# arangesh/TrackMPNN

Measured on AMD Instinct MI355X. Metric: graph_edges_per_sec_fwd_bwd, higher is better.
Workload: dtype f32; 1 GPU; C2 KITTI Car/RRC-shaped rolling windows: 7 frames, D_t~clip(Poisson(6),1,20), F=8 (2d), H=64, K=0, diff; 1 fwd per frame + 1 bwd per window; 16384 windows/GPU batched block-diagonally (64 distinct seeds tiled); windows_per_gpu=16384, rows_final=6762496, parallelism=sequence-dp1

## Files before the change

include/tmpnn.h:

```cpp
#ifndef TMPNN_H
#define TMPNN_H

#include <stddef.h>
#include <stdint.h>

#ifdef __cplusplus
extern "C" {
#endif

#define TMPNN_ABI_VERSION 13

#define TMPNN_OK 0
#define TMPNN_EINVAL (-1)
#define TMPNN_ELAUNCH (-2)
#define TMPNN_EWORKSPACE (-3)

typedef void* tmpnn_stream;
typedef void* tmpnn_event;

typedef struct tmpnn_seg_plan {
    int32_t T;
    int32_t I;
    int32_t nsplit;
    const int32_t* t_row;
// ... 37 lines not shown
    const int32_t* t_loc;
    const int32_t* t_dptr;
    const int32_t* t_dets;
} tmpnn_edge_tiles;

int tmpnn_abi_version(void);
const char* tmpnn_last_error(void);

int tmpnn_gather_diff_fwd(const tmpnn_graph* g, const float* in, int ld_in, float* out, int ld_out,
                          int H, int accumulate, tmpnn_stream stream);
int tmpnn_gather_concat_fwd(const tmpnn_graph* g, const float* in, int ld_in, float* out, int ld_out,
                            int H, int accumulate, tmpnn_stream stream);
int tmpnn_gather_diff_bwd(const tmpnn_graph* g, const float* d_out, int ld_dout, float* d_in, int ld_din,
                          int H, int accumulate, tmpnn_stream stream);
int tmpnn_gather_concat_bwd(const tmpnn_graph* g, const float* d_out, int ld_dout, float* d_in, int ld_din,
                            int H, int accumulate, tmpnn_stream stream);

int tmpnn_segsum_fwd(const tmpnn_graph* g, const float* in, int ld_in, float* out, int ld_out,
                     int H, int accumulate, int compact_out ,
                     tmpnn_stream stream);
int tmpnn_segsum_fwd_live(const tmpnn_graph* g, const float* in, int ld_in, float* out, int ld_out,
                          int H, int compact_out, int row_limit, tmpnn_stream stream);
int tmpnn_segsum_bwd(const tmpnn_graph* g, const float* d_out, int ld_dout, float* d_in, int ld_din,
                     int H, int accumulate, tmpnn_stream stream);

int tmpnn_att_fwd(const tmpnn_graph* g, const int32_t* erec, const float* h, int ld_h, int H, int K,
                  const float* W_cat, const float* a, const uint8_t* keep, float p_drop,
                  float* ha, float* score, float* stats, float* esk, float* alpha, float* out, int ld_out,
                  tmpnn_stream stream);
size_t tmpnn_att_bwd_ws(int E, int Dn, int H, int K);
int tmpnn_att_index(const tmpnn_graph* g, const int32_t* pos, const int32_t* src_pos, const int32_t* dst_pos,
                    int32_t* erec, int32_t* inc_other, tmpnn_stream stream);
int tmpnn_att_bwd(const tmpnn_graph* g, const int32_t* erec, const int32_t* inc_other,
                  const float* h, int ld_h, int H, int K,
                  const float* W_cat, const float* a, const uint8_t* keep, float p_drop,
                  const float* ha, const float* score, const float* stats, const float* esk,
                  const float* d_out, int ld_dout, float* ws, size_t ws_floats,
                  float* d_h, int ld_dh, float* dW_att, float* da, tmpnn_stream stream);
int tmpnn_att_bwd_heads(const tmpnn_graph* g, const int32_t* erec, const int32_t* inc_other,
                        const float* h, int ld_h, int H, int K,
                        const float* W_cat, const float* a, const uint8_t* keep, float p_drop,
                        const float* ha, const float* score, const float* stats, const float* esk,
                        const float* d_out, int ld_dout, float* ws, size_t ws_floats,
                        float* d_h, int ld_dh, float* const* dW_heads, float* const* da_heads, tmpnn_stream stream);

int tmpnn_gru_fwd_head_parts(int H, int IN, int xmode);
int tmpnn_gru_fwd(const int32_t* rows, int R, int xmode, const int32_t* src, const int32_t* dst,
                  const float* msg, int ld_msg, int msg_compact, int IN, const float* h, int ld_h, int H,
                  const float* wih_t, const float* whh_t, const float* b_ih, const float* b_hh,
                  float* h_out, int ld_out, float* gates, size_t gate_plane,
                  const float* w_head, float* logit_part, size_t part_stride, tmpnn_stream stream);
int tmpnn_gru_bwd_data(const int32_t* rows, int R, int IN, const float* h, int ld_h, int H,
                       const float* w_ih, const float* w_hh,
                       const float* gates, size_t gate_plane, const float* d_hout, int ld_dhout,
                       const float* dy, const float* w_head,
                       float* d_msg, int ld_dmsg, float* d_h, int ld_dh,
                       const int32_t* add_src, const int32_t* add_dst, const float* add_msg, int ld_add,
                       tmpnn_stream stream);
size_t tmpnn_gru_bwd_weights_ws(int R, int IN, int H);
int tmpnn_gru_bwd_weights(const int32_t* rows, int R, int xmode, const int32_t* src, const int32_t* dst,
                          const float* msg, int ld_msg, int msg_compact, int IN,
                          const float* h, int ld_h, int H,
                          const float* gates, size_t gate_plane, const float* d_hout, int ld_dhout,
                          const float* dy, const float* w_head,
                          float* dW_ih, float* dW_hh, float* db_ih, float* db_hh,
                          void* ws, size_t ws_bytes, tmpnn_stream stream);

int tmpnn_gru_bwd_fused_available(int H, int IN, int xmode);
size_t tmpnn_gru_bwd_fused_ws(int R, int IN, int H);
int tmpnn_gru_bwd_fused(const int32_t* rows, int R, int xmode, const int32_t* src, const int32_t* dst,
                        const float* msg, int ld_msg, int msg_compact, int IN,
                        const float* h, int ld_h, int H, const float* w_ih, const float* w_hh,
                        const float* gates, size_t gate_plane, const float* d_hout, int ld_dhout,
                        const float* dy, const float* w_head,
                        float* d_msg, int ld_dmsg, float* d_h, int ld_dh,
                        const int32_t* add_src, const int32_t* add_dst, const float* add_msg, int ld_add,
                        float* dW_ih, float* dW_hh, float* db_ih, float* db_hh,
                        void* ws, size_t ws_bytes, tmpnn_stream stream);
typedef struct tmpnn_zs_gate_src {
    const float* proj;
    int32_t ld_proj;
    const int32_t* src_pos;
    const int32_t* dst_pos;
    const float* b_ih;
    const float* b_hh;
} tmpnn_zs_gate_src;
int tmpnn_gru_bwd_fused_zero_state_available(int H, int IN, int xmode);
int tmpnn_gru_bwd_fused_zero_state(const int32_t* rows, int R, const int32_t* src, const int32_t* dst, int IN,
                                   const float* h, int ld_h, int H, const float* w_ih, const float* b_hn,
                                   const float* gates, size_t gate_plane, const float* d_hout, int ld_dhout,
                                   const float* dy, const float* w_head, float* d_msg, int ld_dmsg,
                                   float* dW_ih, float* db_ih, float* db_hh,
                                   void* ws, size_t ws_bytes, tmpnn_stream stream);

int tmpnn_gru_fwd_tiles(const tmpnn_edge_tiles* tiles, int R, const float* proj, int ld_proj, const float* h, int ld_h, int H,
                        const float* whh_t, const float* b_ih, const float* b_hh, float* h_out, int ld_out, float* gates,
                        size_t gate_plane, const float* w_head, float* logit_part, size_t part_stride, tmpnn_stream stream);
int tmpnn_gru_fwd_tiles_zero_state_available(int H, int xmode);
int tmpnn_gru_fwd_tiles_zero_state(const tmpnn_edge_tiles* tiles, int R, const float* proj, int ld_proj, int H,
                                   const float* b_ih, const float* b_hh, float* h_out, int ld_out, float* gates,
                                   size_t gate_plane, int write_hn, const float* w_head, float* logit_part, size_t part_stride,
                                   tmpnn_stream stream);

int tmpnn_rows_linear(const int32_t* rows, int R, const float* in, int ld_in, int H, const float* wt, int NOUT,
                      float* out, int ld_out, tmpnn_stream stream);

int tmpnn_transpose(const float* in, int rows, int cols, float* out, tmpnn_stream stream);

int tmpnn_input_bn_fwd(const float* xdet, int ld_x, int F, int nd, const int32_t* seg_ptr,
                       const int32_t* seg_cnt, const int32_t* seg_of_det ,
                       int S, int H, int training,
                       const float* w1, const float* b1, const float* gamma, const float* beta,
                       float* running_mean, float* running_var,
                       const float* w2, const float* b2,
                       float* y_save, float* mean, float* rstd, float* ws_a ,
                       const int32_t* out_row, float* h_new, int ld_h, tmpnn_stream stream);
size_t tmpnn_input_bn_bwd_ws(int nd, int S, int H, int F);
int tmpnn_input_bn_bwd(const float* xdet, int ld_x, int F, int nd, const int32_t* seg_ptr,
                       const int32_t* seg_cnt, const int32_t* seg_of_det, int S, int H, int training,
                       const float* w1, const float* b1, const float* gamma, const float* beta,
                       const float* w2,
                       const float* y_save, const float* mean, const float* rstd,
                       const int32_t* out_row, const float* d_h, int ld_dh,
                       float* d_xdet, int ld_dx, float* d_xzero,
                       float* dw1, float* db1, float* dgamma, float* dbeta, float* dw2, float* db2,
                       float* ws, size_t ws_floats, tmpnn_stream stream);

int tmpnn_input_tf_supported(int H, int F, int max_seg_rows);
int tmpnn_input_tf_fwd(const float* xdet, const int64_t* x_rows, int ld_x, int F, int nd, const int32_t* seg_ptr, const int32_t* seg_cnt,
                       const int32_t* seg_of_det, int S, int max_seg_rows, int H, int training, const float* w1, const float* b1,
                       const float* gamma, const float* beta, float* running_mean, float* running_var, const float* w2,
                       const float* b2, float* y_save, float* mean, float* rstd, const int32_t* out_row, float* h_new,
                       int ld_h, tmpnn_stream stream);
size_t tmpnn_input_tf_bwd_ws(int nd, int S, int H, int F, int training);
int tmpnn_input_tf_bwd(const float* xdet, const int64_t* x_rows, int ld_x, int F, int nd, const int32_t* seg_ptr, const int32_t* seg_cnt,
                       const int32_t* seg_of_det, int S, int max_seg_rows, int H, int training, const float* w1, const float* b1,
                       const float* gamma, const float* beta, const float* w2, const float* y_save, const float* mean,
                       const float* rstd, const int32_t* out_row, const float* d_h, int ld_dh, float* d_xdet, int ld_dx,
                       float* d_xzero, float* dw1, float* db1, float* dgamma, float* dbeta, float* dw2, float* db2, void* ws,
                       size_t ws_bytes, tmpnn_stream stream);

int tmpnn_heads_fwd(const float* h, int ld_h, int C, int N, const uint8_t* is_edge,
                    const float* w_node, const float* b_node, const float* w_edge, const float* b_edge,
                    float* logits, float* scores, tmpnn_stream stream);
int tmpnn_heads_finish(const float* parts, size_t part_stride, int nparts, int N, const uint8_t* is_edge,
                       const float* b_node, const float* b_edge, float* logits, float* scores, tmpnn_stream stream);
size_t tmpnn_heads_bwd_ws(int N, int C);
int tmpnn_heads_bwd(const float* h, int ld_h, int C, int N, const uint8_t* is_edge,
                    const float* w_node, const float* w_edge, const float* scores,
                    const float* d_logits, const float* d_scores, float* dy_out,
                    float* d_h, int ld_dh, int accumulate,
                    float* dw_node, float* db_node, float* dw_edge, float* db_edge,
                    void* ws, size_t ws_bytes, tmpnn_stream stream);

int tmpnn_targets(const tmpnn_graph* g, const uint8_t* labels, uint8_t* targets, tmpnn_stream stream);
size_t tmpnn_ce_loss_ws(int Dn);
int tmpnn_ce_loss_fwd(const tmpnn_graph* g, const float* logits, const uint8_t* targets, float* stats, float* loss,
                      float* ws, size_t ws_floats, tmpnn_stream stream);
int tmpnn_ce_loss_bwd(const tmpnn_graph* g, const int32_t* src_pos, const int32_t* dst_pos, const float* logits,
                      const float* stats, const float* d_loss, float* d_logits, tmpnn_stream stream);
size_t tmpnn_focal_loss_ws(int R);
int tmpnn_focal_loss_fwd(const int32_t* rows, int R, const float* scores, const uint8_t* targets, float gamma,
                         int use_alpha, float alpha0, float alpha1, float* loss_sum, float* ws, size_t ws_floats,
                         tmpnn_stream stream);
int tmpnn_focal_loss_bwd(const int32_t* rows, int R, const float* scores, const uint8_t* targets, float gamma,
                         int use_alpha, float alpha0, float alpha1, const float* d_loss, float scale, float* d_scores,
                         tmpnn_stream stream);
size_t tmpnn_bce_logits_ws(long n);
int tmpnn_bce_logits_sum_fwd(const float* logits, const float* targets, long n, float* loss_sum, float* ws, size_t ws_floats,
                             tmpnn_stream stream);
int tmpnn_bce_logits_sum_bwd(const float* logits, const float* targets, long n, const float* d_loss, float* d_logits,
                             tmpnn_stream stream);
int tmpnn_train_losses_supported(int E, int Dn);
size_t tmpnn_train_losses_ws(int E, int Dn);
int tmpnn_train_losses_fwd(const tmpnn_graph* g, const float* logits, const float* scores, const uint8_t* labels,
                           int tp_classifier, uint8_t* targets, float* stats, float* out, float* ws, size_t ws_floats,
                           tmpnn_stream stream);
int tmpnn_train_losses_bwd(const tmpnn_graph* g, const int32_t* src_pos, const int32_t* dst_pos, const float* logits,
                           const float* scores, const uint8_t* targets, const float* stats, const float* d_c, const float* d_f,
                           int tp_classifier, float* d_logits, float* d_scores, tmpnn_stream stream);
typedef struct tmpnn_loss_windows {
    int32_t W;
    int32_t n_det;
    int32_t n_edge;
    const int32_t* det_ptr;
    const int32_t* det_idx;
    const int32_t* edge_ptr;
    const int32_t* edge_idx;
    const int32_t* det_win;
    const int32_t* edge_win;
} tmpnn_loss_windows;
size_t tmpnn_train_losses_win_ws(const tmpnn_loss_windows* w);
int tmpnn_train_losses_win_fwd(const tmpnn_graph* g, const tmpnn_loss_windows* w, const float* logits, const float* scores,
                               const uint8_t* labels, int tp_classifier, uint8_t* targets, float* stats, float* out, float* ws,
                               size_t ws_floats, tmpnn_stream stream);
int tmpnn_train_losses_win_bwd(const tmpnn_graph* g, const tmpnn_loss_windows* w, const int32_t* src_pos, const int32_t* dst_pos,
                               const float* logits, const float* scores, const uint8_t* targets, const float* stats,
                               const float* d_c, const float* d_f, int tp_classifier, float* d_logits, float* d_scores,
                               tmpnn_stream stream);

typedef struct tmpnn_train_record {
    double sum_f1;
    int64_t forwards;
    double sum_loss_c;
    double sum_loss_f;
    double sum_loss;
    int64_t chunks;
} tmpnn_train_record;
int tmpnn_cls_counts(const tmpnn_graph* g, const float* scores, const uint8_t* targets, int tp_classifier, int32_t* counts,
                     tmpnn_stream stream);
int tmpnn_cls_counts_win(const tmpnn_graph* g, const tmpnn_loss_windows* w, const float* scores, const uint8_t* targets,
                         int tp_classifier, int32_t* counts, tmpnn_stream stream);
int tmpnn_train_record_fold(const int32_t* counts, int C, int W, const float* loss_c, const float* loss_f, int B,
                            tmpnn_train_record* rec, tmpnn_stream stream);

typedef struct tmpnn_optim_seg {
    float* p;
    int64_t start;
    int64_t count;
} tmpnn_optim_seg;
typedef struct tmpnn_adam_state {
    double lr;
    float step;
    int32_t ticket;
} tmpnn_adam_state;
int tmpnn_optim_chunk(void);
int tmpnn_adam_step(const tmpnn_optim_seg* segs, int P, const int32_t* work, int nwork, float* grad, float* exp_avg,
                    float* exp_avg_sq, int64_t n_flat, tmpnn_adam_state* state, double beta1, double beta2, double eps,
                    double weight_decay, float grad_scale, int zero_grads, tmpnn_stream stream);
int tmpnn_grad_flow(const tmpnn_optim_seg* segs, int P, const float* grad, int64_t n_flat, double* stats, tmpnn_stream stream);

#define TMPNN_TB_MAX_DETS 4096
#define TMPNN_TB_MAX_CALLS 1024
#define TMPNN_TB_NONINT INT64_MIN
#define TMPNN_TB_ST_NONINT 1
#define TMPNN_TB_ST_NEGTS 2
#define TMPNN_TB_ST_RANGE 4
#define TMPNN_TB_ST_DETS 8
#define TMPNN_TB_ST_CALLS 16
#define TMPNN_TB_ST_OFFSETS 32
#define TMPNN_TB_ST_LDS 64
typedef struct tmpnn_train_build {
    int32_t n;
    int32_t B;
    int32_t C;
    int32_t max_dets;
    int32_t max_slots;
    int64_t n_feat;
    const int64_t* y;
    const int64_t* offsets;
    int64_t* info;
    const int32_t* kept;
    const int32_t* cptr;
    int32_t* counts;
    const int32_t* blk;
    const int64_t* call_tab;
    const int32_t* cb_tab;
    int32_t* src; int32_t* dst; int32_t* edge_row; int32_t* src_pos; int32_t* dst_pos;
    int32_t* det_row; int32_t* seg_of_det; int64_t* new_det_local; int64_t* det_group;
    uint8_t* is_edge; int32_t* pos; uint8_t* labels; int64_t* feat_src; int64_t* seg_of_new;
    int32_t* rowptr; int32_t* inc; int32_t* det_order; int32_t* det_win; int32_t* edge_win; int32_t* det_idx; int32_t* edge_idx;
} tmpnn_train_build;
int tmpnn_train_build_count(const tmpnn_train_build* d, tmpnn_stream stream);
int tmpnn_train_build_calls(const tmpnn_train_build* d, tmpnn_stream stream);
int tmpnn_train_build_fill(const tmpnn_train_build* d, int phase, tmpnn_stream stream);

#define TMPNN_CD_MAX_FRAMES 256
#define TMPNN_CD_FLAG_REVERSED 1
#define TMPNN_CD_FLAG_FLIPPED 2
#define TMPNN_CD_FLAG_BAD 128
typedef struct tmpnn_chunk_draw {
    int32_t B;
    int32_t nchunks;
    int32_t L;
    int32_t nseq;
    int32_t F;
    int32_t Fs;
    int32_t fr_range;
    int32_t transforms;
    int64_t ndets;
    int64_t nframes;
    int64_t n_max;
    uint64_t seed;
    uint64_t step;
    float p_drop;
    float p_reverse;
    float p_flip;
    float reserved;
    const int32_t* indices;
    const int32_t* chunks;
    const int32_t* seq_base;
    const int32_t* first;
    const int32_t* track;
    const float* stat;
    const float* table;
    int32_t* count;
    uint8_t* flags;
    int64_t* offsets;
    float* X;
    int64_t* y;
} tmpnn_chunk_draw;
int tmpnn_chunk_draw_count(const tmpnn_chunk_draw* d, tmpnn_stream stream);
int tmpnn_chunk_draw_fill(const tmpnn_chunk_draw* d, tmpnn_stream stream);

#define TMPNN_DG_MAX_ROWS 4096
#define TMPNN_DG_BIG_ROWS 65535
// ... 320 lines not shown
```

trackmpnn_amd/_lib.py:

```python
from __future__ import annotations

import ctypes as C

import torch
import os
import re
from typing import Dict, List, Optional

_HERE = os.path.dirname(os.path.abspath(__file__))
LIB_PATH = os.environ.get('TMPNN_LIB_PATH') or os.path.join(_HERE, 'lib', 'libtmpnn.so')
HEADER_PATH = os.path.join(os.path.dirname(_HERE), 'include', 'tmpnn.h')

ABI_VERSION = 13

c_int = C.c_int
c_void_p = C.c_void_p
c_size_t = C.c_size_t
c_float = C.c_float


class CSegPlan(C.Structure):
    _fields_ = [('T', C.c_int32), ('I', C.c_int32), ('nsplit', C.c_int32), ('t_row', c_void_p), ('items', c_void_p),
                ('rowptr2', c_void_p), ('inc2', c_void_p), ('ws', c_void_p), ('ws_floats', c_size_t)]

# ... 45 lines not shown


class CTrackRows(C.Structure):
    _fields_ = [('ts', c_void_p), ('det_id', c_void_p), ('assoc', c_void_p), ('is_edge', c_void_p), ('src', c_void_p),
                ('dst', c_void_p), ('labels', c_void_p)]


class CLossWindows(C.Structure):
    _fields_ = [('W', C.c_int32), ('n_det', C.c_int32), ('n_edge', C.c_int32), ('det_ptr', c_void_p), ('det_idx', c_void_p),
                ('edge_ptr', c_void_p), ('edge_idx', c_void_p), ('det_win', c_void_p), ('edge_win', c_void_p)]


class CTrainBuild(C.Structure):
    _fields_ = [('n', C.c_int32), ('B', C.c_int32), ('C', C.c_int32), ('max_dets', C.c_int32), ('max_slots', C.c_int32),
                ('n_feat', C.c_int64)] + [(f, c_void_p) for f in (
                    'y', 'offsets', 'info', 'kept', 'cptr', 'counts', 'blk', 'call_tab', 'cb_tab',
                    'src', 'dst', 'edge_row', 'src_pos', 'dst_pos', 'det_row', 'seg_of_det', 'new_det_local', 'det_group',
                    'is_edge', 'pos', 'labels', 'feat_src', 'seg_of_new',
                    'rowptr', 'inc', 'det_order', 'det_win', 'edge_win', 'det_idx', 'edge_idx')]


class CChunkDraw(C.Structure):
    _fields_ = ([(f, C.c_int32) for f in ('B', 'nchunks', 'L', 'nseq', 'F', 'Fs', 'fr_range', 'transforms')]
                + [(f, C.c_int64) for f in ('ndets', 'nframes', 'n_max')] + [('seed', C.c_uint64), ('step', C.c_uint64)]
                + [(f, c_float) for f in ('p_drop', 'p_reverse', 'p_flip', 'reserved')]
                + [(f, c_void_p) for f in ('indices', 'chunks', 'seq_base', 'first', 'track', 'stat', 'table',
                                           'count', 'flags', 'offsets', 'X', 'y')])


class CMotStore(C.Structure):
    _fields_ = ([('S', C.c_int32), ('reserved', C.c_int32)] + [(f, C.c_int64) for f in ('n_gt', 'n_det', 'n_off', 'n_obj')]
                + [(f, c_void_p) for f in ('seq', 'gt_off', 'det_off', 'gt_id', 'gt_box', 'det_box', 'det_perm')])


class CMapStore(C.Structure):
    _fields_ = ([('S', C.c_int32), ('C', C.c_int32)] + [(f, C.c_int64) for f in ('n_gt', 'n_det', 'n_grp', 'n_live', 'n_claim')]
                + [(f, c_void_p) for f in ('gt_box', 'gt_seq', 'cls_gt_off', 'grp_off', 'det_box', 'det_grp', 'det_best', 'cls_off',
                                           'order', 'claim_off', 'claim_det')])


class CLabelStore(C.Structure):
    _fields_ = ([('S', C.c_int32), ('reserved', C.c_int32)] + [(f, C.c_int64) for f in ('n_frames', 'n_det', 'n_gt')]
                + [('iom_ignore_cat', C.c_int32), ('iou_ignore_cat', C.c_int32), ('iou_thresh', c_float), ('iom_thresh', c_float)]
                + [(f, C.c_int64) for f in ('n_small', 'n_big')]
                + [(f, c_void_p) for f in ('seq_base', 'det_first', 'gt_first', 'small_frames', 'big_frames', 'det_frame', 'det_cat',
                                           'det_box', 'det_score', 'gt_frame', 'gt_track', 'gt_cat', 'gt_box')])


class CLabelOut(C.Structure):
    _fields_ = [(f, c_void_p) for f in ('record', 'track', 'keep', 'gt_keep', 'det_cnt', 'gt_cnt', 'fflag', 'det_off', 'gt_off',
                                        'seq_det_off', 'seq_gt_off', 'o_det_frame', 'o_det_track', 'o_det_cat', 'o_det_box',
                                        'o_det_score', 'o_gt_frame', 'o_gt_track', 'o_gt_cat', 'o_gt_box')]


class CVisHead(C.Structure):
    _fields_ = ([(f, C.c_int32) for f in ('T', 'Hm', 'Wm', 'B')] + [('D', C.c_int64)]
                + [(f, c_float) for f in ('input_h', 'input_w', 'down_ratio', 'im_h', 'im_w')]
                + [(f, C.c_int32) for f in ('ld_rows', 'col', 'reserved')]
                + [(f, c_void_p) for f in ('maps', 'box', 'map_of', 'im_hw', 'track', 'offsets', 'mean', 'std', 'rows', 'logits',
                                           'stat', 'nll', 'pix', 'flag', 'chunk_of', 'key', 'loss', 'count')])


_DGP = C.POINTER(CDGraph)
_MPP = C.POINTER(CMpParams)
_TRP = C.POINTER(CTrackRows)
_LWP = C.POINTER(CLossWindows)
_TBP = C.POINTER(CTrainBuild)
_CDP = C.POINTER(CChunkDraw)
_MSP = C.POINTER(CMotStore)
_MAP = C.POINTER(CMapStore)
_LSP = C.POINTER(CLabelStore)
_LOP = C.POINTER(CLabelOut)
_VHP = C.POINTER(CVisHead)

_SIGNATURES = {
    'tmpnn_abi_version': (c_int, []),
    'tmpnn_last_error': (C.c_char_p, []),
    'tmpnn_gather_diff_fwd': (c_int, [_GP, c_void_p, c_int, c_void_p, c_int, c_int, c_int, c_void_p]),
    'tmpnn_gather_concat_fwd': (c_int, [_GP, c_void_p, c_int, c_void_p, c_int, c_int, c_int, c_void_p]),
    'tmpnn_gather_diff_bwd': (c_int, [_GP, c_void_p, c_int, c_void_p, c_int, c_int, c_int, c_void_p]),
    'tmpnn_gather_concat_bwd': (c_int, [_GP, c_void_p, c_int, c_void_p, c_int, c_int, c_int, c_void_p]),
    'tmpnn_segsum_fwd': (c_int, [_GP, c_void_p, c_int, c_void_p, c_int, c_int, c_int, c_int, c_void_p]),
    'tmpnn_segsum_fwd_live': (c_int, [_GP, c_void_p, c_int, c_void_p, c_int, c_int, c_int, c_int, c_void_p]),
    'tmpnn_segsum_bwd': (c_int, [_GP, c_void_p, c_int, c_void_p, c_int, c_int, c_int, c_void_p]),
    'tmpnn_att_fwd': (c_int, [_GP, c_void_p, c_void_p, c_int, c_int, c_int, c_void_p, c_void_p, c_void_p, c_float,
                              c_void_p, c_void_p, c_void_p, c_void_p, c_void_p, c_void_p, c_int, c_void_p]),
    'tmpnn_att_bwd_ws': (c_size_t, [c_int, c_int, c_int, c_int]),
    'tmpnn_att_index': (c_int, [_GP, c_void_p, c_void_p, c_void_p, c_void_p, c_void_p, c_void_p]),
    'tmpnn_att_bwd': (c_int, [_GP, c_void_p, c_void_p, c_void_p, c_int, c_int, c_int, c_void_p, c_void_p, c_void_p,
                              c_float, c_void_p, c_void_p, c_void_p, c_void_p, c_void_p, c_int, c_void_p, c_size_t,
                              c_void_p, c_int, c_void_p, c_void_p, c_void_p]),
    'tmpnn_att_bwd_heads': (c_int, [_GP, c_void_p, c_void_p, c_void_p, c_int, c_int, c_int, c_void_p, c_void_p,
                                    c_void_p, c_float, c_void_p, c_void_p, c_void_p, c_void_p, c_void_p, c_int, c_void_p,
                                    c_size_t, c_void_p, c_int, c_void_p, c_void_p, c_void_p]),
    'tmpnn_gru_fwd': (c_int, [c_void_p, c_int, c_int, c_void_p, c_void_p, c_void_p, c_int, c_int, c_int,
                              c_void_p, c_int, c_int, c_void_p, c_void_p, c_void_p, c_void_p,
                              c_void_p, c_int, c_void_p, c_size_t, c_void_p, c_void_p, c_size_t, c_void_p]),
    'tmpnn_gru_fwd_head_parts': (c_int, [c_int, c_int, c_int]),
    'tmpnn_gru_fwd_tiles': (c_int, [_TP, c_int, c_void_p, c_int, c_void_p, c_int, c_int, c_void_p, c_void_p, c_void_p,
                                    c_void_p, c_int, c_void_p, c_size_t, c_void_p, c_void_p, c_size_t, c_void_p]),
    'tmpnn_gru_fwd_tiles_zero_state_available': (c_int, [c_int, c_int]),
    'tmpnn_gru_fwd_tiles_zero_state': (c_int, [_TP, c_int, c_void_p, c_int, c_int, c_void_p, c_void_p, c_void_p, c_int,
                                               c_void_p, c_size_t, c_int, c_void_p, c_void_p, c_size_t, c_void_p]),
    'tmpnn_heads_finish': (c_int, [c_void_p, c_size_t, c_int, c_int, c_void_p, c_void_p, c_void_p, c_void_p, c_void_p, c_void_p]),
    'tmpnn_gru_bwd_data': (c_int, [c_void_p, c_int, c_int, c_void_p, c_int, c_int, c_void_p, c_void_p,
                                   c_void_p, c_size_t, c_void_p, c_int, c_void_p, c_void_p,
                                   c_void_p, c_int, c_void_p, c_int,
                                   c_void_p, c_void_p, c_void_p, c_int, c_void_p]),
    'tmpnn_gru_bwd_weights_ws': (c_size_t, [c_int, c_int, c_int]),
    'tmpnn_gru_bwd_weights': (c_int, [c_void_p, c_int, c_int, c_void_p, c_void_p, c_void_p, c_int, c_int, c_int,
                                      c_void_p, c_int, c_int, c_void_p, c_size_t, c_void_p, c_int, c_void_p, c_void_p,
                                      c_void_p, c_void_p, c_void_p, c_void_p, c_void_p, c_size_t, c_void_p]),
    'tmpnn_gru_bwd_fused_available': (c_int, [c_int, c_int, c_int]),
    'tmpnn_gru_bwd_fused_ws': (c_size_t, [c_int, c_int, c_int]),
    'tmpnn_gru_bwd_fused': (c_int, [c_void_p, c_int, c_int, c_void_p, c_void_p, c_void_p, c_int, c_int, c_int,
                                    c_void_p, c_int, c_int, c_void_p, c_void_p, c_void_p, c_size_t, c_void_p, c_int,
                                    c_void_p, c_void_p, c_void_p, c_int, c_void_p, c_int,
                                    c_void_p, c_void_p, c_void_p, c_int, c_void_p, c_void_p, c_void_p, c_void_p,
                                    c_void_p, c_size_t, c_void_p]),
    'tmpnn_gru_bwd_fused_zero_state_available': (c_int, [c_int, c_int, c_int]),
    'tmpnn_gru_bwd_fused_zero_state': (c_int, [c_void_p, c_int, c_void_p, c_void_p, c_int, c_void_p, c_int, c_int,
                                               c_void_p, c_void_p, c_void_p, c_size_t, c_void_p, c_int, c_void_p,
                                               c_void_p, c_void_p, c_int, c_void_p, c_void_p, c_void_p, c_void_p,
                                               c_size_t, c_void_p]),
    'tmpnn_rows_linear': (c_int, [c_void_p, c_int, c_void_p, c_int, c_int, c_void_p, c_int, c_void_p, c_int, c_void_p]),
    'tmpnn_transpose': (c_int, [c_void_p, c_int, c_int, c_void_p, c_void_p]),
    'tmpnn_input_bn_fwd': (c_int, [c_void_p, c_int, c_int, c_int, c_void_p, c_void_p, c_void_p, c_int, c_int, c_int,
                                   c_void_p, c_void_p, c_void_p, c_void_p, c_void_p, c_void_p, c_void_p, c_void_p,
                                   c_void_p, c_void_p, c_void_p, c_void_p, c_void_p, c_void_p, c_int, c_void_p]),
    'tmpnn_input_bn_bwd_ws': (c_size_t, [c_int, c_int, c_int, c_int]),
    'tmpnn_input_bn_bwd': (c_int, [c_void_p, c_int, c_int, c_int, c_void_p, c_void_p, c_void_p, c_int, c_int, c_int,
                                   c_void_p, c_void_p, c_void_p, c_void_p, c_void_p,
                                   c_void_p, c_void_p, c_void_p, c_void_p, c_void_p, c_int,
                                   c_void_p, c_int, c_void_p,
                                   c_void_p, c_void_p, c_void_p, c_void_p, c_void_p, c_void_p,
                                   c_void_p, c_size_t, c_void_p]),
    'tmpnn_input_tf_supported': (c_int, [c_int, c_int, c_int]),
    'tmpnn_input_tf_fwd': (c_int, [c_void_p, c_void_p, c_int, c_int, c_int, c_void_p, c_void_p, c_void_p, c_int, c_int, c_int, c_int,
                                   c_void_p, c_void_p, c_void_p, c_void_p, c_void_p, c_void_p, c_void_p, c_void_p,
                                   c_void_p, c_void_p, c_void_p, c_void_p, c_void_p, c_int, c_void_p]),
    'tmpnn_input_tf_bwd_ws': (c_size_t, [c_int, c_int, c_int, c_int, c_int]),
    'tmpnn_input_tf_bwd': (c_int, [c_void_p, c_void_p, c_int, c_int, c_int, c_void_p, c_void_p, c_void_p, c_int, c_int, c_int, c_int,
                                   c_void_p, c_void_p, c_void_p, c_void_p, c_void_p,
                                   c_void_p, c_void_p, c_void_p, c_void_p, c_void_p, c_int,
                                   c_void_p, c_int, c_void_p,
                                   c_void_p, c_void_p, c_void_p, c_void_p, c_void_p, c_void_p,
                                   c_void_p, c_size_t, c_void_p]),
    'tmpnn_heads_fwd': (c_int, [c_void_p, c_int, c_int, c_int, c_void_p, c_void_p, c_void_p, c_void_p, c_void_p,
                                c_void_p, c_void_p, c_void_p]),
    'tmpnn_heads_bwd_ws': (c_size_t, [c_int, c_int]),
    'tmpnn_heads_bwd': (c_int, [c_void_p, c_int, c_int, c_int, c_void_p, c_void_p, c_void_p, c_void_p, c_void_p,
                                c_void_p, c_void_p, c_void_p, c_int, c_int, c_void_p, c_void_p, c_void_p, c_void_p,
                                c_void_p, c_size_t, c_void_p]),
    'tmpnn_targets': (c_int, [_GP, c_void_p, c_void_p, c_void_p]),
    'tmpnn_ce_loss_ws': (c_size_t, [c_int]),
    'tmpnn_ce_loss_fwd': (c_int, [_GP, c_void_p, c_void_p, c_void_p, c_void_p, c_void_p, c_size_t, c_void_p]),
    'tmpnn_ce_loss_bwd': (c_int, [_GP, c_void_p, c_void_p, c_void_p, c_void_p, c_void_p, c_void_p, c_void_p]),
    'tmpnn_focal_loss_ws': (c_size_t, [c_int]),
    'tmpnn_focal_loss_fwd': (c_int, [c_void_p, c_int, c_void_p, c_void_p, c_float, c_int, c_float, c_float, c_void_p,
                                     c_void_p, c_size_t, c_void_p]),
    'tmpnn_focal_loss_bwd': (c_int, [c_void_p, c_int, c_void_p, c_void_p, c_float, c_int, c_float, c_float, c_void_p,
                                     c_float, c_void_p, c_void_p]),
    'tmpnn_bce_logits_ws': (c_size_t, [C.c_long]),
    'tmpnn_bce_logits_sum_fwd': (c_int, [c_void_p, c_void_p, C.c_long, c_void_p, c_void_p, c_size_t, c_void_p]),
    'tmpnn_bce_logits_sum_bwd': (c_int, [c_void_p, c_void_p, C.c_long, c_void_p, c_void_p, c_void_p]),
    'tmpnn_train_losses_supported': (c_int, [c_int, c_int]),
    'tmpnn_train_losses_ws': (c_size_t, [c_int, c_int]),
    'tmpnn_train_losses_fwd': (c_int, [_GP, c_void_p, c_void_p, c_void_p, c_int, c_void_p, c_void_p, c_void_p, c_void_p,
                                       c_size_t, c_void_p]),
    'tmpnn_train_losses_bwd': (c_int, [_GP, c_void_p, c_void_p, c_void_p, c_void_p, c_void_p, c_void_p, c_void_p, c_void_p,
                                       c_int, c_void_p, c_void_p, c_void_p]),
    'tmpnn_train_losses_win_ws': (c_size_t, [_LWP]),
    'tmpnn_train_losses_win_fwd': (c_int, [_GP, _LWP, c_void_p, c_void_p, c_void_p, c_int, c_void_p, c_void_p, c_void_p,
                                           c_void_p, c_size_t, c_void_p]),
    'tmpnn_train_losses_win_bwd': (c_int, [_GP, _LWP, c_void_p, c_void_p, c_void_p, c_void_p, c_void_p, c_void_p, c_void_p,
                                           c_void_p, c_int, c_void_p, c_void_p, c_void_p]),
    'tmpnn_cls_counts': (c_int, [_GP, c_void_p, c_void_p, c_int, c_void_p, c_void_p]),
    'tmpnn_cls_counts_win': (c_int, [_GP, _LWP, c_void_p, c_void_p, c_int, c_void_p, c_void_p]),
    'tmpnn_train_record_fold': (c_int, [c_void_p, c_int, c_int, c_void_p, c_void_p, c_int, c_void_p, c_void_p]),
    'tmpnn_optim_chunk': (c_int, []),
    'tmpnn_adam_step': (c_int, [c_void_p, c_int, c_void_p, c_int, c_void_p, c_void_p, c_void_p, C.c_int64, c_void_p,
                                C.c_double, C.c_double, C.c_double, C.c_double, c_float, c_int, c_void_p]),
    'tmpnn_grad_flow': (c_int, [c_void_p, c_int, c_void_p, C.c_int64, c_void_p, c_void_p]),
    'tmpnn_train_build_count': (c_int, [_TBP, c_void_p]),
    'tmpnn_train_build_calls': (c_int, [_TBP, c_void_p]),
    'tmpnn_train_build_fill': (c_int, [_TBP, c_int, c_void_p]),
    'tmpnn_chunk_draw_count': (c_int, [_CDP, c_void_p]),
    'tmpnn_chunk_draw_fill': (c_int, [_CDP, c_void_p]),
    'tmpnn_online_features': (c_int, [c_int] * 8 + [c_void_p, c_void_p, c_int, c_void_p, c_void_p, c_void_p, c_void_p, c_int,
                                      c_void_p, c_void_p, c_void_p]),
    'tmpnn_mot_max_per_frame': (c_int, []),
    'tmpnn_mot_events_ws': (c_size_t, [c_int, C.c_int64, C.c_int64]),
    'tmpnn_mot_events': (c_int, [_MSP, c_void_p, c_void_p, c_void_p, c_size_t, c_void_p, c_void_p]),
    'tmpnn_mot_dist': (c_int, [c_void_p, c_int, c_void_p, c_int, c_void_p, c_void_p]),
    'tmpnn_mot_summary_limit': (c_int, [c_int]),
    'tmpnn_mot_summary_ws': (c_size_t, [c_int, C.c_int64, C.c_int64, C.c_int64]),
    'tmpnn_mot_summary': (c_int, [_MSP, c_void_p, c_void_p, c_void_p, c_size_t, c_void_p, c_void_p]),
    'tmpnn_map_tile': (c_int, []),
    'tmpnn_map_best': (c_int, [_MAP, c_void_p, c_void_p]),
    'tmpnn_map_eval_ws': (c_size_t, [C.c_int64, C.c_int64, C.c_int64]),
    'tmpnn_map_eval': (c_int, [_MAP, c_void_p, c_void_p, c_void_p, c_size_t, c_void_p, c_void_p]),
    'tmpnn_label_max_per_frame': (c_int, []),
    'tmpnn_label_wave_frame': (c_int, []),
    'tmpnn_label_dets': (c_int, [_LSP, _LOP, c_void_p]),
    'tmpnn_label_compact': (c_int, [_LSP, _LOP, c_void_p]),
    'tmpnn_vis_head_fwd': (c_int, [_VHP, c_void_p]),
    'tmpnn_vis_head_bwd': (c_int, [_VHP, c_void_p, c_void_p, c_void_p]),
    'tmpnn_dgraph_ints': (c_size_t, [c_int]),
    'tmpnn_dgraph_bind': (c_int, [c_void_p, c_int, c_int, _DGP]),
    'tmpnn_graph_from_coo': (c_int, [c_int, c_void_p, c_void_p, C.c_int64, c_void_p, c_void_p, C.c_int64, _DGP, c_void_p]),
    'tmpnn_graph_from_coo_arena': (c_int, [c_int, c_void_p, c_void_p, C.c_int64, c_void_p, c_void_p, C.c_int64, c_void_p, c_int, c_void_p]),
    'tmpnn_graph_from_coo_arena_ws': (c_int, [c_int, c_void_p, c_void_p, C.c_int64, c_void_p, c_void_p, C.c_int64, c_void_p, c_int,
                                              c_void_p, c_size_t, c_void_p]),
    'tmpnn_graph_from_rows_ws': (c_int, [c_int, c_void_p, c_void_p, c_void_p, _DGP, c_void_p, c_size_t, c_void_p]),
    'tmpnn_track_finalize_ws': (c_size_t, [c_int]),
    'tmpnn_track_load': (c_int, [c_int, c_int, c_void_p, _TRP, c_void_p, c_int, c_int, c_void_p, c_int, c_void_p, _DGP, c_void_p,
                                 c_size_t, c_void_p]),
    'tmpnn_track_select': (c_int, [_DGP, _TRP, c_void_p, c_int, c_int, c_int, c_void_p, c_void_p, c_void_p]),
    'tmpnn_track_select_ws': (c_int, [_DGP, _TRP, c_void_p, c_int, c_int, c_int, c_void_p, c_void_p, c_void_p, c_size_t, c_void_p]),
    'tmpnn_track_hungarian_max_dets': (c_int, []),
    'tmpnn_track_extend': (c_int, [c_int, c_int, c_int, c_void_p, c_void_p, c_int, c_void_p, _TRP, c_void_p, c_int, c_int,
                                   c_void_p, c_int, _DGP, c_void_p, c_size_t, c_void_p]),
    'tmpnn_track_extend_tf': (c_int, [c_int, c_int, c_int, c_void_p, c_void_p, c_int, c_void_p, _TRP, c_void_p, c_int, c_void_p,
                                      c_void_p, c_void_p, c_size_t, _DGP, c_void_p, c_void_p, c_int, c_void_p, c_void_p]),
    'tmpnn_track_retire': (c_int, [_DGP, _TRP, c_void_p, c_int, c_int, c_int, c_void_p, c_int, c_void_p, c_void_p, c_size_t,
                                   c_void_p, c_void_p, _TRP, c_void_p, c_int, c_int, c_void_p, c_int, c_void_p, c_int,
                                   c_void_p, c_void_p, c_void_p]),
    'tmpnn_val_f1_count': (c_int, [_DGP, c_void_p, c_void_p, c_int, c_void_p, c_void_p, c_int, c_void_p]),
    'tmpnn_wide_supported': (c_int, [c_int, c_int]),
    'tmpnn_wide_prep_bytes': (c_size_t, [c_int, c_int]),
    'tmpnn_wide_prepare': (c_int, [c_void_p, c_void_p, c_int, c_int, c_void_p, c_void_p]),
    'tmpnn_wide_gru_fwd': (c_int, [c_void_p, c_void_p, c_int, c_void_p, c_int, c_void_p, c_void_p, c_void_p, c_int, c_int,
                                   c_void_p, c_void_p, c_void_p, c_void_p, c_int, c_void_p, c_size_t, c_void_p]),
    'tmpnn_wide_gru_fwd_tiled': (c_int, [c_void_p, c_void_p, c_int, _TP, c_int, c_void_p, c_int, c_int, c_void_p, c_void_p,
                                         c_void_p, c_void_p, c_int, c_void_p, c_size_t, c_void_p]),
    'tmpnn_wide_gru_bwd_diff_ws': (c_size_t, [c_int, c_int, c_int, c_int]),
    'tmpnn_wide_gru_bwd_diff': (c_int, [c_void_p, _GP, c_void_p, c_int, c_int, c_void_p, c_size_t, c_void_p, c_int,
                                        c_void_p, c_void_p, c_void_p, c_int, c_void_p, c_void_p, c_void_p, c_void_p,
                                        c_void_p, c_size_t, c_void_p]),
    'tmpnn_wide_gru_bwd_diff_fused': (c_int, [c_void_p, _GP, c_void_p, c_int, c_int, c_void_p, c_size_t, c_void_p, c_int,
                                              c_void_p, c_void_p, c_void_p, c_int, c_void_p, c_void_p, c_void_p, c_void_p,
                                              c_void_p, c_size_t, c_void_p, c_int, c_void_p, c_void_p, c_void_p, c_void_p]),
    'tmpnn_mp_iter_prep_floats': (c_size_t, [c_int, c_int, c_int]),
    'tmpnn_mp_iter_prepare': (c_int, [_MPP, c_void_p, c_void_p]),
    'tmpnn_mp_iter_save_floats': (c_size_t, [c_int, c_int, c_int, c_int]),
    'tmpnn_mp_iter_fwd': (c_int, [_MPP, c_void_p, _DGP, c_int, c_void_p, c_int, c_void_p, c_int,
                                  c_void_p, c_void_p, c_void_p, c_void_p, c_size_t, c_void_p]),
    'tmpnn_mp_iter_save_es_offset': (c_size_t, [c_int, c_int, c_int, c_int]),
    'tmpnn_mp_iter_fwd_parts': (c_int, [_MPP, c_void_p, _DGP, c_int, c_void_p, c_int, c_void_p, c_int,
                                        c_void_p, c_void_p, c_void_p, c_void_p, c_size_t, c_int, c_void_p]),
    'tmpnn_mp_iter_bwd_parts': (c_int, [_MPP, c_void_p, _DGP, c_int, c_void_p, c_int, c_void_p, c_void_p, c_void_p, c_void_p,
                                        c_int, c_void_p, c_int, c_void_p, c_int, c_void_p, c_void_p, c_void_p, _MPP, c_void_p,
                                        c_size_t, c_int, c_void_p]),
    'tmpnn_mp_iter_bwd_ws': (c_size_t, [c_int, c_int, c_int, c_int, c_int]),
    'tmpnn_mp_iter_bwd': (c_int, [_MPP, c_void_p, _DGP, c_int, c_void_p, c_int, c_void_p, c_void_p, c_void_p, c_void_p,
                                  c_int, c_void_p, c_int, c_void_p, c_int, c_void_p, c_void_p, c_void_p, _MPP, c_void_p,
                                  c_size_t, c_void_p]),
}

_lib: Optional[C.CDLL] = None


_VARIANT_SIGNATURES = {
    'tmpnn_track_append': (c_int, [c_int, c_int, c_int, c_void_p, c_void_p, c_int, c_void_p, c_void_p, c_void_p, c_void_p,
                                   c_void_p, c_void_p, c_void_p, c_void_p, c_void_p]),
    'tmpnn_gru_bwd_weights_variant': (c_int, [c_void_p, c_int, c_int, c_void_p, c_void_p, c_void_p, c_int, c_int, c_int,
                                              c_void_p, c_int, c_int, c_void_p, c_size_t, c_void_p, c_int, c_void_p, c_void_p,
                                              c_void_p, c_void_p, c_void_p, c_void_p, c_void_p, c_size_t, c_int, c_void_p]),
    'tmpnn_gru_bwd_weights_choice': (c_int, []),
    'tmpnn_wide_gru_bwd_diff_aux': (c_int, [c_void_p, _GP, c_void_p, c_int, c_int, c_void_p, c_size_t, c_void_p, c_int,
                                            c_void_p, c_void_p, c_void_p, c_int, c_void_p, c_void_p, c_void_p, c_void_p,
                                            c_void_p, c_size_t, c_void_p, c_void_p, c_void_p, c_void_p]),
    'tmpnn_wide_gru_bwd_data_ws': (c_size_t, [c_int, c_int]),
    'tmpnn_wide_gru_bwd_data': (c_int, [c_void_p, c_void_p, c_int, c_void_p, c_int, c_int, c_void_p, c_size_t, c_void_p, c_int,
                                        c_void_p, c_void_p, c_void_p, c_int, c_void_p, c_int, c_void_p, c_size_t, c_void_p]),
    'tmpnn_wide_gru_bwd_weights_ws': (c_size_t, [c_int, c_int]),
    'tmpnn_wide_gru_bwd_weights': (c_int, [c_void_p, c_void_p, c_int, c_void_p, c_void_p, c_void_p, c_int, c_int, c_void_p,
                                           c_void_p, c_void_p, c_void_p, c_void_p, c_size_t, c_void_p]),
}


def header_symbols(variants: bool = False) -> List[str]:
    with open(HEADER_PATH) as f:
        txt = f.read()
    if not variants:
        txt = re.sub(r'#ifdef TMPNN_KEEP_VARIANTS.*?#endif', '', txt, flags=re.S)
    txt = re.sub(r'/\*.*?\*/', '', txt, flags=re.S)
    return sorted(set(re.findall(r'\b(tmpnn_[a-z0-9_]+)\s*\(', txt)))


def load() -> C.CDLL:
    global _lib
    if _lib is not None:
        return _lib
    if not os.path.exists(LIB_PATH):
        raise RuntimeError(
            f'{LIB_PATH} is missing: build it with `python -c "import __graft_entry__ as g; g.build()"` '
            '(hipcc --offload-arch=gfx950).  trackmpnn_amd has no CPU or torch fallback.')
    lib = C.CDLL(LIB_PATH)
    for name, (res, args) in _SIGNATURES.items():
        try:
            fn = getattr(lib, name)
        except AttributeError as e:
            raise RuntimeError(f'libtmpnn.so does not export {name}; rebuild it') from e
        fn.restype = res
        fn.argtypes = args
# ... 37 lines not shown
```

trackmpnn_amd/csrc/agg.hip:

```cpp
#include "common.h"
#include <stdlib.h>

namespace tmpnn {

static thread_local char g_err[512] = "";

int set_error(int code, const char* fmt, ...) {
    va_list ap;
    va_start(ap, fmt);
    vsnprintf(g_err, sizeof(g_err), fmt, ap);
    va_end(ap);
    return code;
}

#ifdef TMPNN_KEEP_VARIANTS
template <bool CONCAT, bool ACC>
__global__ __launch_bounds__(256) void k_gather(int E, const int32_t* __restrict__ src,
                                                const int32_t* __restrict__ dst,
                                                const int32_t* __restrict__ edge_row,
                                                const float* __restrict__ in, int ld_in,
                                                float* __restrict__ out, int ld_out, int H) {
    const int lpr = H >> 2;
    const int rpb = 256 / lpr;
    const int c4 = (threadIdx.x % lpr) * 4;
    const int slot = threadIdx.x / lpr;
    constexpr int U = 4;
    const long stride = (long)gridDim.x * rpb;
    for (long e0 = (long)blockIdx.x * rpb + slot; e0 < E; e0 += stride * U) {
        int s[U], d[U], r[U];
        bool ok[U];
#pragma unroll
        for (int u = 0; u < U; ++u) {
            const long e = e0 + u * stride;
            ok[u] = e < E;
            const long ec = ok[u] ? e : e0;
            s[u] = src[ec]; d[u] = dst[ec]; r[u] = edge_row[ec];
        }
        float4 a[U], b[U];
#pragma unroll
        for (int u = 0; u < U; ++u) {
            a[u] = *reinterpret_cast<const float4*>(in + (size_t)s[u] * ld_in + c4);
            b[u] = *reinterpret_cast<const float4*>(in + (size_t)d[u] * ld_in + c4);
        }
#pragma unroll
        for (int u = 0; u < U; ++u) {
            if (!ok[u]) continue;
            float* o = out + (size_t)r[u] * ld_out + c4;
            if (!CONCAT) {
                float4 v = make_float4(a[u].x - b[u].x, a[u].y - b[u].y, a[u].z - b[u].z, a[u].w - b[u].w);
                if (ACC) {
                    const float4 p = *reinterpret_cast<const float4*>(o);
                    v.x += p.x; v.y += p.y; v.z += p.z; v.w += p.w;
                }
                *reinterpret_cast<float4*>(o) = v;
            } else {
                float4 va = a[u], vb = b[u];
                if (ACC) {
                    const float4 p = *reinterpret_cast<const float4*>(o);
                    const float4 q = *reinterpret_cast<const float4*>(o + H);
                    va.x += p.x; va.y += p.y; va.z += p.z; va.w += p.w;
                    vb.x += q.x; vb.y += q.y; vb.z += q.z; vb.w += q.w;
                }
                *reinterpret_cast<float4*>(o) = va;
                *reinterpret_cast<float4*>(o + H) = vb;
            }
        }
    }
}

template <bool ACC>
__global__ __launch_bounds__(256) void k_segsum(int Dn, const int32_t* __restrict__ det_row,
                                                const int32_t* __restrict__ rowptr,
                                                const int32_t* __restrict__ inc,
                                                const int32_t* __restrict__ det_order,
                                                const float* __restrict__ in, int ld_in,
                                                float* __restrict__ out, int ld_out, int H,
                                                float wneg, int cneg, int compact_out) {
    const int lane = threadIdx.x & 63;
    const int lpr = H >> 2;
    const int ngrp = 64 / lpr;
    const int grp = lane / lpr;
    const int c4 = (lane % lpr) * 4;
    constexpr int U = 4;
    constexpr int SEG_CHUNK = 64;
    const int wv = threadIdx.x >> 6;
    for (long base = (long)blockIdx.x * SEG_CHUNK; base < Dn; base += (long)gridDim.x * SEG_CHUNK) {
        const long hi = base + SEG_CHUNK < Dn ? base + SEG_CHUNK : Dn;
        for (long i = base + wv; i < hi; i += 4) {
            const int d = det_order ? det_order[i] : (int)i;
            const int p0 = rowptr[d], p1 = rowptr[d + 1];
            float4 acc = make_float4(0.f, 0.f, 0.f, 0.f);
            for (int pb = p0 + grp; pb < p1; pb += ngrp * U) {
                int v[U];
#pragma unroll
                for (int u = 0; u < U; ++u) {
                    const int p = pb + u * ngrp;
                    v[u] = p < p1 ? inc[p] : 0x7fffffff;
                }
                float4 x[U];
#pragma unroll
                for (int u = 0; u < U; ++u) {
                    const bool live = v[u] != 0x7fffffff;
                    const int row = live ? (v[u] & 0x7fffffff) : 0;
                    x[u] = *reinterpret_cast<const float4*>(in + (size_t)row * ld_in + (v[u] < 0 ? cneg : 0) + c4);
                    const float w = v[u] < 0 ? wneg : 1.0f;
                    if (live) { x[u].x *= w; x[u].y *= w; x[u].z *= w; x[u].w *= w; }
                    else x[u] = make_float4(0.f, 0.f, 0.f, 0.f);
                }
#pragma unroll
                for (int u = 0; u < U; ++u) { acc.x += x[u].x; acc.y += x[u].y; acc.z += x[u].z; acc.w += x[u].w; }
            }
            for (int off = lpr; off < 64; off <<= 1) {
                acc.x += __shfl_xor(acc.x, off);
                acc.y += __shfl_xor(acc.y, off);
                acc.z += __shfl_xor(acc.z, off);
                acc.w += __shfl_xor(acc.w, off);
            }
            if (grp == 0) {
                float* o = out + (size_t)(compact_out ? d : det_row[d]) * ld_out + c4;
                if (ACC) {
                    const float4 p = *reinterpret_cast<const float4*>(o);
                    acc.x += p.x; acc.y += p.y; acc.z += p.z; acc.w += p.w;
                }
                *reinterpret_cast<float4*>(o) = acc;
            }
        }
    }
}


#endif

template <bool CONCAT, bool ACC, int U = 4>
__global__ __launch_bounds__(256) void k_gather_pipe(int E, const int32_t* __restrict__ src,
                                                     const int32_t* __restrict__ dst,
                                                     const int32_t* __restrict__ edge_row,
                                                     const float* __restrict__ in, int ld_in,
                                                     float* __restrict__ out, int ld_out, int H) {
    const int lpr = H >> 2;
    const int rpb = 256 / lpr;
    const int c4 = (threadIdx.x % lpr) * 4;
    const int slot = threadIdx.x / lpr;
    const long chunk = (long)rpb * U;
    long e0 = (long)blockIdx.x * chunk + slot;
    const long step = (long)gridDim.x * chunk;
    int s[U], d[U], r[U];
    auto load_ids = [&](long base) {
#pragma unroll
        for (int u = 0; u < U; ++u) {
            const long e = base + (long)u * rpb;
            const long ec = e < E ? e : (E - 1);
            s[u] = src[ec]; d[u] = dst[ec]; r[u] = edge_row[ec];
        }
    };
    if (e0 < E) load_ids(e0);
    for (; e0 < E; e0 += step) {
        float4 a[U], b[U];
        int rr[U];
        bool ok[U];
#pragma unroll
        for (int u = 0; u < U; ++u) {
            ok[u] = e0 + (long)u * rpb < E;
            rr[u] = r[u];
            a[u] = *reinterpret_cast<const float4*>(in + (size_t)s[u] * ld_in + c4);
            b[u] = *reinterpret_cast<const float4*>(in + (size_t)d[u] * ld_in + c4);
        }
        if (e0 + step < E) load_ids(e0 + step);
#pragma unroll
        for (int u = 0; u < U; ++u) {
            if (!ok[u]) continue;
            float* o = out + (size_t)rr[u] * ld_out + c4;
            if (!CONCAT) {
                float4 v = make_float4(a[u].x - b[u].x, a[u].y - b[u].y, a[u].z - b[u].z, a[u].w - b[u].w);
                if (ACC) {
                    const float4 p = *reinterpret_cast<const float4*>(o);
                    v.x += p.x; v.y += p.y; v.z += p.z; v.w += p.w;
                }
                *reinterpret_cast<float4*>(o) = v;
            } else {
                float4 va = a[u], vb = b[u];
                if (ACC) {
                    const float4 p = *reinterpret_cast<const float4*>(o);
                    const float4 q = *reinterpret_cast<const float4*>(o + H);
                    va.x += p.x; va.y += p.y; va.z += p.z; va.w += p.w;
                    vb.x += q.x; vb.y += q.y; vb.z += q.z; vb.w += q.w;
                }
                *reinterpret_cast<float4*>(o) = va;
                *reinterpret_cast<float4*>(o + H) = vb;
            }
        }
    }
}

template <bool ACC, int U = 4, int SEG_CHUNK = 32, bool DUAL = false, bool LIM = false>
__global__ __launch_bounds__(256) void k_segsum_pipe(int Dn, const int32_t* __restrict__ det_row,
                                                     const int32_t* __restrict__ rowptr,
                                                     const int32_t* __restrict__ inc,
                                                     const int32_t* __restrict__ det_order,
                                                     const float* __restrict__ in, int ld_in,
                                                     float* __restrict__ out, int ld_out, int H,
                                                     float wneg, int cneg, int compact_out,
                                                     const float* __restrict__ part = nullptr, int nsplit = 0,
                                                     int row_limit = 0x7fffffff) {
    const int lane = threadIdx.x & 63;
    const int lpr = H >> 2;
    const int ngrp = 64 / lpr;
    const int grp = lane / lpr;
    const int c4 = (lane % lpr) * 4;
    const int wv = threadIdx.x >> 6;
    const long nchunk = (Dn + SEG_CHUNK - 1) / SEG_CHUNK;
    auto item_pos = [&](long k) -> long {
        const long per = SEG_CHUNK / 4;
        const long ch = (long)blockIdx.x + (k / per) * gridDim.x;
        if (ch >= nchunk) return -1;
        const long i = ch * SEG_CHUNK + wv + (k % per) * 4;
        return i < Dn ? i : -2;
    };
    long kA = 0;
    int dA = -1, dB = -1, p0B = 0, p1B = 0, dC = -1, p0C = 0, p1C = 0, vC[U];
    auto fetchA = [&]() {
        long pos;
        do { pos = item_pos(kA++); } while (pos == -2);
        dA = pos < 0 ? -1 : (det_order ? det_order[pos] : (int)pos);
    };
    auto advanceB = [&]() {
        dB = dA;
        if (dB >= 0) { p0B = rowptr[dB]; p1B = rowptr[dB + 1]; }
    };
    auto advanceC = [&]() {
        dC = dB; p0C = p0B; p1C = p1B;
        if (dC >= 0) {
#pragma unroll
            for (int u = 0; u < U; ++u) {
                const int p = p0C + grp + u * ngrp;
                vC[u] = p < p1C ? inc[p] : 0x7fffffff;
            }
        }
    };
    fetchA(); advanceB(); fetchA(); advanceC(); advanceB(); fetchA();
    int pbC = p0C + grp;
    float4 acc = make_float4(0.f, 0.f, 0.f, 0.f);
    while (dC >= 0) {
        const int d = dC;
        float4 x[U];
        bool live[U];
        float w[U];
#pragma unroll
        for (int u = 0; u < U; ++u) {
            live[u] = vC[u] != 0x7fffffff;
            const int row = live[u] ? (vC[u] & 0x7fffffff) : 0;
            w[u] = vC[u] < 0 ? wneg : 1.0f;
            if (LIM) {
                live[u] = live[u] && row < row_limit;
                x[u] = make_float4(0.f, 0.f, 0.f, 0.f);
                if (live[u]) x[u] = *reinterpret_cast<const float4*>(in + (size_t)row * ld_in + (vC[u] < 0 ? cneg : 0) + c4);
            } else if (DUAL && row >= nsplit)
                x[u] = *reinterpret_cast<const float4*>(part + (size_t)(row - nsplit) * H + c4);
            else
                x[u] = *reinterpret_cast<const float4*>(in + (size_t)row * ld_in + (vC[u] < 0 ? cneg : 0) + c4);
        }
        const bool last = (pbC - grp) + ngrp * U >= p1C;
        if (!last) {
            pbC += ngrp * U;
#pragma unroll
            for (int u = 0; u < U; ++u) {
                const int p = pbC + u * ngrp;
                vC[u] = p < p1C ? inc[p] : 0x7fffffff;
            }
        } else {
            advanceC(); advanceB(); fetchA();
            pbC = p0C + grp;
        }
#pragma unroll
        for (int u = 0; u < U; ++u) {
            if (live[u]) { x[u].x *= w[u]; x[u].y *= w[u]; x[u].z *= w[u]; x[u].w *= w[u]; }
            else x[u] = make_float4(0.f, 0.f, 0.f, 0.f);
        }
#pragma unroll
        for (int u = 0; u < U; ++u) { acc.x += x[u].x; acc.y += x[u].y; acc.z += x[u].z; acc.w += x[u].w; }
        if (!last) continue;
        for (int off = lpr; off < 64; off <<= 1) {
            acc.x += __shfl_xor(acc.x, off);
            acc.y += __shfl_xor(acc.y, off);
            acc.z += __shfl_xor(acc.z, off);
            acc.w += __shfl_xor(acc.w, off);
        }
        if (grp == 0) {
            float* o = out + (size_t)(compact_out ? d : det_row[d]) * ld_out + c4;
            if (ACC) {
                const float4 p = *reinterpret_cast<const float4*>(o);
                acc.x += p.x; acc.y += p.y; acc.z += p.z; acc.w += p.w;
            }
            *reinterpret_cast<float4*>(o) = acc;
        }
        acc = make_float4(0.f, 0.f, 0.f, 0.f);
    }
}

#ifdef TMPNN_KEEP_VARIANTS
static int agg_variant() {
    static const int v = [] { const char* e = getenv("TMPNN_AGG"); return (e && e[0] == '0') ? 0 : 1; }();
    return v;
}
#else
static constexpr int agg_variant() { return 1; }
#endif

__global__ void k_transpose(const float* __restrict__ in, int rows, int cols, float* __restrict__ out) {
    __shared__ float tile[32][33];
    const int bx = blockIdx.x * 32, by = blockIdx.y * 32;
    for (int j = threadIdx.y; j < 32; j += blockDim.y) {
        const int r = by + j, c = bx + threadIdx.x;
        if (r < rows && c < cols) tile[j][threadIdx.x] = in[(size_t)r * cols + c];
    }
    __syncthreads();
    for (int j = threadIdx.y; j < 32; j += blockDim.y) {
        const int c = bx + j, r = by + threadIdx.x;
        if (r < rows && c < cols) out[(size_t)c * rows + r] = tile[threadIdx.x][j];
    }
}

__global__ void k_reduce_slabs(const float* __restrict__ slabs, size_t stride, int nslab,
                               float* __restrict__ dst, size_t n, int accumulate) {
    const size_t i = (size_t)blockIdx.x * blockDim.x + threadIdx.x;
    if (i >= n) return;
    float s = 0.f;
#pragma unroll 8
    for (int k = 0; k < nslab; ++k) s += slabs[(size_t)k * stride + i];
    dst[i] = accumulate ? dst[i] + s : s;
}

__global__ void k_fold_slabs(const float* __restrict__ slabs, size_t stride, int nslab, float* __restrict__ out,
                             size_t n) {
    const size_t i = (size_t)blockIdx.x * blockDim.x + threadIdx.x;
    if (i >= n) return;
    const int k0 = blockIdx.y * 32, k1 = min(nslab, k0 + 32);
    float s = 0.f;
#pragma unroll 8
    for (int k = k0; k < k1; ++k) s += slabs[(size_t)k * stride + i];
    out[(size_t)blockIdx.y * n + i] = s;
}

size_t reduce_slabs_ws_floats(int nslab, size_t n) { return nslab > 64 ? (size_t)ceil_div(nslab, 32) * n : 0; }

int launch_reduce_slabs(const float* slabs, size_t stride, int nslab, float* dst, size_t n, int accumulate,
                        hipStream_t st, float* ws2) {
    if (n == 0) return TMPNN_OK;
    if (nslab > 64 && ws2 != nullptr) {
        const int ng = ceil_div(nslab, 32);
        hipLaunchKernelGGL(k_fold_slabs, dim3(ceil_div((long)n, 256), ng), dim3(256), 0, st, slabs, stride, nslab, ws2, n);
        int rc = check_launch("fold_slabs");
        if (rc) return rc;
        slabs = ws2;
        stride = n;
        nslab = ng;
    }
    hipLaunchKernelGGL(k_reduce_slabs, dim3(ceil_div((long)n, 256)), dim3(256), 0, st, slabs, stride, nslab, dst,
                       n, accumulate);
    return check_launch("reduce_slabs");
}

static int check_graph(const tmpnn_graph* g) {
    TM_REQUIRE(g != nullptr, "graph is null");
    TM_REQUIRE(g->N >= 0 && g->E >= 0 && g->Dn >= 0 && (long)g->E + g->Dn == g->N,
               "graph sizes inconsistent: N=%d E=%d Dn=%d", g->N, g->E, g->Dn);
    if (g->E > 0)
        TM_REQUIRE(g->src && g->dst && g->edge_row && g->inc, "graph edge arrays are null (E=%d)", g->E);
    if (g->Dn > 0) TM_REQUIRE(g->det_row && g->rowptr, "graph det arrays are null (Dn=%d)", g->Dn);
    return TMPNN_OK;
}

static int check_rows(const float* in, int ld_in, const float* out, int ld_out, int H, int w_in, int w_out) {
    TM_REQUIRE(supported_H(H), "unsupported hidden width H=%d (need 32/64/128/256)", H);
    TM_REQUIRE(in && out, "null feature pointer");
    TM_REQUIRE(ld_in >= w_in && ld_out >= w_out, "leading dimension too small (ld_in=%d ld_out=%d)", ld_in, ld_out);
    TM_REQUIRE((ld_in & 3) == 0 && (ld_out & 3) == 0 && aligned16(in) && aligned16(out),
               "feature rows must be 16-byte aligned (ld multiple of 4 floats)");
    return TMPNN_OK;
}

static int grid_for(long items, int per_block) {
    long b = (items + per_block - 1) / per_block;
    if (b > 256L * 64) b = 256L * 64;
    if (b < 1) b = 1;
    return (int)b;
}

static int gather(const tmpnn_graph* g, const float* in, int ld_in, float* out, int ld_out, int H, int accumulate,
                  bool concat, tmpnn_stream stream) {
    int rc = check_graph(g);
    if (rc) return rc;
    rc = check_rows(in, ld_in, out, ld_out, H, H, concat ? 2 * H : H);
    if (rc) return rc;
    if (g->E == 0) return TMPNN_OK;
    const int rpb = 256 / (H >> 2);
    dim3 grid(grid_for(g->E, rpb)), block(256);
    hipStream_t st = as_stream(stream);
#define L(K, C, A) hipLaunchKernelGGL((K<C, A>), grid, block, 0, st, g->E, g->src, g->dst, g->edge_row, in, ld_in, out, ld_out, H)
    if (agg_variant() && !concat) {
        grid = dim3(grid_for(g->E, rpb * 8));
        if (accumulate) hipLaunchKernelGGL((k_gather_pipe<false, true, 8>), grid, block, 0, st, g->E, g->src, g->dst, g->edge_row, in, ld_in, out, ld_out, H);
        else hipLaunchKernelGGL((k_gather_pipe<false, false, 8>), grid, block, 0, st, g->E, g->src, g->dst, g->edge_row, in, ld_in, out, ld_out, H);
    } else
    if (agg_variant()) {
        grid = dim3(grid_for(g->E, rpb * 4));
        if (concat) { if (accumulate) L(k_gather_pipe, true, true); else L(k_gather_pipe, true, false); }
        else        { if (accumulate) L(k_gather_pipe, false, true); else L(k_gather_pipe, false, false); }
    }
#ifdef TMPNN_KEEP_VARIANTS
    else {
        if (concat) { if (accumulate) L(k_gather, true, true); else L(k_gather, true, false); }
        else        { if (accumulate) L(k_gather, false, true); else L(k_gather, false, false); }
    }
#endif
#undef L
    return check_launch("gather");
}


__global__ __launch_bounds__(256) void k_segsum_tiles(int I, int T, const int32_t* __restrict__ items,
                                                      const int32_t* __restrict__ t_row, const float* __restrict__ in,
                                                      int ld_in, float* __restrict__ part) {
    __shared__ float4 S[4][8][64];
    const int tid = threadIdx.x, lane = tid & 63;
    const int w = __builtin_amdgcn_readfirstlane(tid >> 6);
    auto add4 = [](float4 a, const float4& b) { a.x += b.x; a.y += b.y; a.z += b.z; a.w += b.w; return a; };
    for (int k = blockIdx.x; k < I; k += gridDim.x) {
        const int t0 = items[2 * k], nt = items[2 * k + 1];
        float4 ad[4];
#pragma unroll
        for (int j = 0; j < 4; ++j) ad[j] = make_float4(0.f, 0.f, 0.f, 0.f);
        for (int t = t0; t < t0 + nt; ++t) {
            const int32_t* tr = t_row + (size_t)t * 128 + 4 * w;
            float4 ps[8];
#pragma unroll
            for (int half = 0; half < 2; ++half) {
                float4 x[4][4];
#pragma unroll
                for (int i = 0; i < 4; ++i)
#pragma unroll
                    for (int j = 0; j < 4; ++j) {
                        const int row = tr[(half * 4 + i) * 16 + j];
                        x[i][j] = *reinterpret_cast<const float4*>(in + (size_t)(row < 0 ? 0 : row) * ld_in + 4 * lane);
                        if (row < 0) x[i][j] = make_float4(0.f, 0.f, 0.f, 0.f);
                    }
#pragma unroll
                for (int i = 0; i < 4; ++i) {
                    ps[half * 4 + i] = add4(add4(add4(x[i][0], x[i][1]), x[i][2]), x[i][3]);
#pragma unroll
                    for (int j = 0; j < 4; ++j) ad[j] = add4(ad[j], x[i][j]);
                }
            }
#pragma unroll
            for (int i = 0; i < 8; ++i) S[w][i][lane] = ps[i];
            __syncthreads();
#pragma unroll
            for (int r = 0; r < 2; ++r) {
                const int i = w + 4 * r;
                const float4 v = add4(add4(add4(S[0][i][lane], S[1][i][lane]), S[2][i][lane]), S[3][i][lane]);
                *reinterpret_cast<float4*>(part + ((size_t)t * 8 + i) * 256 + 4 * lane) = v;
            }
            __syncthreads();
        }
#pragma unroll
        for (int j = 0; j < 4; ++j)
            *reinterpret_cast<float4*>(part + ((size_t)8 * T + (size_t)16 * k + 4 * w + j) * 256 + 4 * lane) = ad[j];
    }
}

static int segsum_dense(const tmpnn_graph* g, const tmpnn_seg_plan* pl, const float* in, int ld_in, float* out, int ld_out,
                        int accumulate, int compact_out, hipStream_t st) {
    TM_REQUIRE(pl->T >= 0 && pl->I >= 0 && pl->nsplit == g->N && pl->rowptr2 && pl->inc2 && (pl->T == 0 || (pl->t_row && pl->items)),
               "segsum (dense form): inconsistent plan (T=%d I=%d nsplit=%d N=%d)", pl->T, pl->I, pl->nsplit, g->N);
    const size_t need = ((size_t)8 * pl->T + (size_t)16 * pl->I) * 256;
    if (need > 0 && (pl->ws == nullptr || pl->ws_floats < need))
        return set_error(TMPNN_EWORKSPACE, "segsum (dense form): the plan's partial buffer holds %zu floats, %zu needed", pl->ws_floats, need);
    if (pl->I > 0) {
        const int grid = pl->I < 256 * 4 ? pl->I : 256 * 4;
        hipLaunchKernelGGL(k_segsum_tiles, dim3(grid), dim3(256), 0, st, pl->I, pl->T, pl->items, pl->t_row, in, ld_in, pl->ws);
        int rc = check_launch("segsum_tiles");
        if (rc) return rc;
    }
    dim3 grid(grid_for(g->Dn, 16)), block(256);
    if (accumulate)
        hipLaunchKernelGGL((k_segsum_pipe<true, 8, 16, true>), grid, block, 0, st, g->Dn, g->det_row, pl->rowptr2, pl->inc2,
                           (const int32_t*)nullptr, in, ld_in, out, ld_out, 256, -1.0f, 0, compact_out, pl->ws, pl->nsplit);
    else
        hipLaunchKernelGGL((k_segsum_pipe<false, 8, 16, true>), grid, block, 0, st, g->Dn, g->det_row, pl->rowptr2, pl->inc2,
                           (const int32_t*)nullptr, in, ld_in, out, ld_out, 256, -1.0f, 0, compact_out, pl->ws, pl->nsplit);
    return check_launch("segsum (dense form, second pass)");
}

#ifdef TMPNN_KEEP_VARIANTS
static constexpr int SW_CH = 160;
static constexpr int SW_MAXCH = 24, SW_MAXD = 160, SW_LCAP = 15;
static constexpr int SW_NW = 8, SW_NHG = 128;
static constexpr int SW_ROWS = SW_CH * 128, SW_RECS = 4096, SW_ACCS = 4 * SW_MAXD * 128, SW_IDS = 768, SW_OROW = 768;
static constexpr int SW_OFF_RECS = 3 * SW_ROWS, SW_OFF_ACCS = SW_OFF_RECS + 3 * SW_RECS, SW_OFF_IDS = SW_OFF_ACCS + SW_ACCS,
                     SW_OFF_OROW = SW_OFF_IDS + 3 * SW_IDS;
static constexpr size_t SW_SHM = SW_OFF_OROW + 2 * SW_OROW;
static_assert(SW_SHM <= 160 * 1024, "k_segsum_win: three chunks and a window's streams must fit the LDS");
static_assert(SW_MAXD <= SW_CH && SW_LCAP * 2 * SW_NHG <= SW_RECS && 4 * SW_CH <= SW_IDS && 4 * SW_MAXD <= SW_OROW &&
                  4 * SW_MAXD <= 5 * SW_NHG && SW_CH / 8 <= 3 * SW_NW && SW_MAXD <= 3 * 8 * SW_NW, "k_segsum_win: capacities");

__device__ __forceinline__ uint32_t sw_lds_addr(const void* p) {
    return (uint32_t)(uintptr_t)(const __attribute__((address_space(3))) char*)(const char*)p;
}
template <int DW>
__device__ __forceinline__ void sw_glds(const void* gsrc, uint32_t lds_wave_base) {
    unsigned keep;
    lds_wave_base = __builtin_amdgcn_readfirstlane(lds_wave_base);
    if constexpr (DW == 4)
        asm volatile("s_mov_b32 %0, m0\n\ts_mov_b32 m0, %2\n\ts_nop 0\n\tglobal_load_lds_dwordx4 %1, off\n\ts_mov_b32 m0, %0"
                     : "=&s"(keep) : "v"(gsrc), "s"(lds_wave_base) : "memory");
    else
        asm volatile("s_mov_b32 %0, m0\n\ts_mov_b32 m0, %2\n\ts_nop 0\n\tglobal_load_lds_dword %1, off\n\ts_mov_b32 m0, %0"
                     : "=&s"(keep) : "v"(gsrc), "s"(lds_wave_base) : "memory");
}
__device__ __forceinline__ void sw_wait(int n) {
    if (n == 0) asm volatile("s_waitcnt vmcnt(0)" ::: "memory");
    else if (n == 1) asm volatile("s_waitcnt vmcnt(1)" ::: "memory");
    else if (n == 2) asm volatile("s_waitcnt vmcnt(2)" ::: "memory");
    else if (n == 3) asm volatile("s_waitcnt vmcnt(3)" ::: "memory");
    else if (n == 4) asm volatile("s_waitcnt vmcnt(4)" ::: "memory");
    else if (n == 5) asm volatile("s_waitcnt vmcnt(5)" ::: "memory");
    else if (n == 6) asm volatile("s_waitcnt vmcnt(6)" ::: "memory");
    else if (n == 7) asm volatile("s_waitcnt vmcnt(7)" ::: "memory");
    else if (n == 8) asm volatile("s_waitcnt vmcnt(8)" ::: "memory");
    else asm volatile("s_waitcnt vmcnt(0)" ::: "memory");
}

struct SwJob {
    int j, e0, ne, q0, nd, r0, lm2, mb, nit;
    unsigned long long lm01;
    __device__ __forceinline__ int hf() const { return j & 1; }
    __device__ __forceinline__ int nch() const { return (ne + SW_CH - 1) / SW_CH; }
};
struct SwItem { SwJob jb; int c, L, roff; };
__device__ __forceinline__ void sw_copy(SwItem& d, const SwItem& s) {
// ... 106 lines not shown
    sw_copy(B, A);
    next_item(B);
    sw_copy(Cn, B);
    next_item(Cn);
    sw_copy(D, Cn);
    next_item(D);
    sw_copy(En, D);
    next_item(En);
    for (int x = tid; x < SW_ACCS / 16; x += 512) reinterpret_cast<float4*>(accs)[x] = make_float4(0.f, 0.f, 0.f, 0.f);
    stage_ids(A, 0);
    stage_ids(B, 1);
    stage_ids(Cn, 2);
    sw_wait(0);
    __syncthreads();
    stage_rows(A, 0);
    sw_wait(0);
    __syncthreads();
    fly = 0;
    stage_rows(B, 1);
    stage_ids(D, 0);
    int fly_prev = fly;
    int W_nd = 0, W_hf = 0, W_mb = 0;
    bool wr = false;
    int rb = 0;
    for (;;) {
        sw_wait(fly_prev);
        __syncthreads();
        fly = 0;
        if (wr) {
            const int* orow = orow_of(W_mb);
            const float* prevr = rows_of(rb == 0 ? 2 : rb - 1);
#pragma unroll
            for (int p = 0; p < 3; ++p) {
                if (64 * p + 8 * wv >= W_nd) continue;
                const int q = 64 * p + hgl, qc = min(q, W_nd - 1);
                float* as = accs + qc * 4 * 32 + c4;
                const float4 a0 = *reinterpret_cast<const float4*>(as), a1 = *reinterpret_cast<const float4*>(as + 32);
                const float4 a2 = *reinterpret_cast<const float4*>(as + 64), a3 = *reinterpret_cast<const float4*>(as + 96);
                const int orw = orow[qc];
                float4 t;
                t.x = (a0.x + a1.x) + (a2.x + a3.x);
                t.y = (a0.y + a1.y) + (a2.y + a3.y);
                t.z = (a0.z + a1.z) + (a2.z + a3.z);
                t.w = (a0.w + a1.w) + (a2.w + a3.w);
                if (ACC) {
                    const float4 pv = *reinterpret_cast<const float4*>(prevr + qc * 32 + c4);
                    t.x += pv.x; t.y += pv.y; t.z += pv.z; t.w += pv.w;
                }
                if (q < W_nd) {
                    *reinterpret_cast<float4*>(out + (size_t)orw * ld_out + 32 * W_hf + c4) = t;
                    const float4 z = make_float4(0.f, 0.f, 0.f, 0.f);
                    *reinterpret_cast<float4*>(as) = z;
                    *reinterpret_cast<float4*>(as + 32) = z;
                    *reinterpret_cast<float4*>(as + 64) = z;
                    *reinterpret_cast<float4*>(as + 96) = z;
                }
                ++fly;
            }
            __syncthreads();
            wr = false;
        }
        if (A.jb.nit == 0) break;
        stage_rows(Cn, rb == 0 ? 2 : rb - 1);
        stage_ids(En, rb == 2 ? 0 : rb + 1);
        if (A.L > 0) {
            const uint16_t* rc = recs_of(rb) + hgl;
            const float* rows = rows_of(rb) + c4;
            float* ab = accs + hgl * 32 + c4;
            unsigned r0 = rc[0], r1 = rc[64];
            for (int s = 0; s < A.L; ++s) {
                const int sn = min(s + 1, A.L - 1) * SW_NHG;
                const unsigned n0 = rc[sn], n1 = rc[sn + 64];
                const float4 x0 = *reinterpret_cast<const float4*>(rows + (r0 & 255u) * 32);
                const float4 x1 = *reinterpret_cast<const float4*>(rows + (r1 & 255u) * 32);
                float* ap0 = ab + ((r0 >> 9) & 7u) * (SW_NHG * 32);
                float* ap1 = ab + ((r1 >> 9) & 7u) * (SW_NHG * 32) + 64 * 32;
                float4 a0 = *reinterpret_cast<const float4*>(ap0), a1 = *reinterpret_cast<const float4*>(ap1);
                const float w0 = (r0 & 0x100u) ? -1.0f : 1.0f, w1 = (r1 & 0x100u) ? -1.0f : 1.0f;
                a0.x += x0.x * w0; a0.y += x0.y * w0; a0.z += x0.z * w0; a0.w += x0.w * w0;
                a1.x += x1.x * w1; a1.y += x1.y * w1; a1.z += x1.z * w1; a1.w += x1.w * w1;
                if (!(r0 & 0x8000u)) *reinterpret_cast<float4*>(ap0) = a0;
                if (!(r1 & 0x8000u)) *reinterpret_cast<float4*>(ap1) = a1;
                r0 = n0; r1 = n1;
            }
        }
        if (A.c == A.jb.nit - 1) { wr = true; W_nd = A.jb.nd; W_hf = A.jb.hf(); W_mb = A.jb.mb; }
        sw_copy(A, B); sw_copy(B, Cn); sw_copy(Cn, D); sw_copy(D, En);
        next_item(En);
        rb = rb == 2 ? 0 : rb + 1;
        fly_prev = fly;
    }
    sw_wait(0);
}

static int cu_count() {
    static const int v = [] {
        int dev = 0, cus = 256;
        if (hipGetDevice(&dev) == hipSuccess) (void)hipDeviceGetAttribute(&cus, hipDeviceAttributeMultiprocessorCount, dev);
        return cus > 0 ? cus : 256;
    }();
    return v;
}

static int segsum_win(const tmpnn_graph* g, const tmpnn_win_plan* pl, const float* in, int ld_in, float* out, int ld_out,
                      int accumulate, int compact_out, hipStream_t st) {
    TM_REQUIRE(pl->W > 0 && pl->wrec && pl->erow && pl->recs && pl->det && pl->drow &&
                   (pl->nbig == 0 || pl->big_order), "segsum: incomplete window plan");
    const int njob = 2 * pl->W, cus = cu_count();
    dim3 grid(njob < cus ? njob : cus), block(512);
    if (accumulate) {
        TM_SHM_ONCE((k_segsum_win<true>), SW_SHM);
        hipLaunchKernelGGL((k_segsum_win<true>), grid, block, SW_SHM, st, *pl, in, ld_in, out, ld_out, compact_out);
    } else {
        TM_SHM_ONCE((k_segsum_win<false>), SW_SHM);
        hipLaunchKernelGGL((k_segsum_win<false>), grid, block, SW_SHM, st, *pl, in, ld_in, out, ld_out, compact_out);
    }
    int rc = check_launch("segsum (window-owned form)");
    if (rc || pl->nbig == 0) return rc;
    dim3 g2(grid_for(pl->nbig, 32));
    if (accumulate)
        hipLaunchKernelGGL((k_segsum_pipe<true, 4, 32>), g2, dim3(256), 0, st, pl->nbig, g->det_row, g->rowptr, g->inc, pl->big_order,
                           in, ld_in, out, ld_out, 64, -1.0f, 0, compact_out);
    else
        hipLaunchKernelGGL((k_segsum_pipe<false, 4, 32>), g2, dim3(256), 0, st, pl->nbig, g->det_row, g->rowptr, g->inc, pl->big_order,
                           in, ld_in, out, ld_out, 64, -1.0f, 0, compact_out);
    return check_launch("segsum (windows beyond the LDS capacity)");
}

#endif

static int segsum(const tmpnn_graph* g, const float* in, int ld_in, float* out, int ld_out, int H, int accumulate,
                  float wneg, int cneg, int compact_out, tmpnn_stream stream, int row_limit = 0x7fffffff) {
    int rc = check_graph(g);
    if (rc) return rc;
    rc = check_rows(in, ld_in, out, ld_out, H, H + cneg, H);
    if (rc) return rc;
    if (g->Dn == 0) return TMPNN_OK;
    hipStream_t st = as_stream(stream);
    if (g->seg_plan && H == 256 && wneg == -1.0f && cneg == 0)
        return segsum_dense(g, g->seg_plan, in, ld_in, out, ld_out, accumulate, compact_out, st);
#ifdef TMPNN_KEEP_VARIANTS
    if (g->win_plan && H == 64 && wneg == -1.0f && cneg == 0 && 2 * g->win_plan->W >= cu_count() &&
        ld_in % 4 == 0 && ld_out % 4 == 0 && (((uintptr_t)in | (uintptr_t)out) & 15) == 0)
        return segsum_win(g, g->win_plan, in, ld_in, out, ld_out, accumulate, compact_out, st);
#endif
    dim3 grid(grid_for(g->Dn, 64)), block(256);
#define LS(K, A) hipLaunchKernelGGL((K<A>), grid, block, 0, st, g->Dn, g->det_row, g->rowptr, g->inc, g->det_order, in, ld_in, out, ld_out, H, wneg, cneg, compact_out)
#define LSP(A, UU, CH)                                                                                       \
    do {                                                                                                     \
        grid = dim3(grid_for(g->Dn, CH));                                                                    \
        hipLaunchKernelGGL((k_segsum_pipe<A, UU, CH>), grid, block, 0, st, g->Dn, g->det_row, g->rowptr, g->inc, \
                           g->det_order, in, ld_in, out, ld_out, H, wneg, cneg, compact_out);                \
    } while (0)
    const bool deep = (long)2 * g->E > (long)24 * g->Dn;
    if (row_limit < g->N && !accumulate) {
        grid = dim3(grid_for(g->Dn, deep ? 16 : 32));
        if (deep)
            hipLaunchKernelGGL((k_segsum_pipe<false, 8, 16, false, true>), grid, block, 0, st, g->Dn, g->det_row, g->rowptr, g->inc,
                               g->det_order, in, ld_in, out, ld_out, H, wneg, cneg, compact_out, (const float*)nullptr, 0, row_limit);
        else
            hipLaunchKernelGGL((k_segsum_pipe<false, 4, 32, false, true>), grid, block, 0, st, g->Dn, g->det_row, g->rowptr, g->inc,
                               g->det_order, in, ld_in, out, ld_out, H, wneg, cneg, compact_out, (const float*)nullptr, 0, row_limit);
        return check_launch("segsum (live rows)");
    }
    if (agg_variant()) {
        if (deep) { if (accumulate) LSP(true, 8, 16); else LSP(false, 8, 16); }
        else      { if (accumulate) LSP(true, 4, 32); else LSP(false, 4, 32); }
    }
#ifdef TMPNN_KEEP_VARIANTS
    else               { if (accumulate) LS(k_segsum, true); else LS(k_segsum, false); }
#endif
#undef LSP
#undef LS
    return check_launch("segsum");
}

}

using namespace tmpnn;

extern "C" {

int tmpnn_abi_version(void) { return TMPNN_ABI_VERSION; }
const char* tmpnn_last_error(void) { return tmpnn::g_err; }

#define TM_SLICED(H_, call_)                                                              \
    do {                                                                                  \
        if (supported_H_big(H_)) {                                                        \
            for (int c0 = 0; c0 < (H_); c0 += 256) {                                      \
                const int w = (H_) - c0 < 256 ? (H_) - c0 : 256;                          \
                const int rc_ = call_;                                                    \
                if (rc_) return rc_;                                                      \
            }                                                                             \
            return TMPNN_OK;                                                              \
        }                                                                                 \
    } while (0)

int tmpnn_gather_diff_fwd(const tmpnn_graph* g, const float* in, int ld_in, float* out, int ld_out, int H,
                          int accumulate, tmpnn_stream stream) {
    TM_SLICED(H, gather(g, in + c0, ld_in, out + c0, ld_out, w, accumulate, false, stream));
    return gather(g, in, ld_in, out, ld_out, H, accumulate, false, stream);
}
int tmpnn_gather_concat_fwd(const tmpnn_graph* g, const float* in, int ld_in, float* out, int ld_out, int H,
                            int accumulate, tmpnn_stream stream) {
    return gather(g, in, ld_in, out, ld_out, H, accumulate, true, stream);
}
int tmpnn_gather_diff_bwd(const tmpnn_graph* g, const float* d_out, int ld_dout, float* d_in, int ld_din, int H,
                          int accumulate, tmpnn_stream stream) {
    TM_SLICED(H, segsum(g, d_out + c0, ld_dout, d_in + c0, ld_din, w, accumulate, -1.0f, 0, 0, stream));
    return segsum(g, d_out, ld_dout, d_in, ld_din, H, accumulate, -1.0f, 0, 0, stream);
}
int tmpnn_gather_concat_bwd(const tmpnn_graph* g, const float* d_out, int ld_dout, float* d_in, int ld_din, int H,
                            int accumulate, tmpnn_stream stream) {
    TM_SLICED(H, segsum(g, d_out + c0, ld_dout, d_in + c0, ld_din, w, accumulate, 1.0f, H, 0, stream));
    return segsum(g, d_out, ld_dout, d_in, ld_din, H, accumulate, 1.0f, H, 0, stream);
}
int tmpnn_segsum_fwd(const tmpnn_graph* g, const float* in, int ld_in, float* out, int ld_out, int H, int accumulate,
                     int compact_out, tmpnn_stream stream) {
    TM_SLICED(H, segsum(g, in + c0, ld_in, out + c0, ld_out, w, accumulate, -1.0f, 0, compact_out, stream));
    return segsum(g, in, ld_in, out, ld_out, H, accumulate, -1.0f, 0, compact_out, stream);
}
int tmpnn_segsum_fwd_live(const tmpnn_graph* g, const float* in, int ld_in, float* out, int ld_out, int H, int compact_out,
                          int row_limit, tmpnn_stream stream) {
    TM_REQUIRE(row_limit >= 0, "segsum_fwd_live: row_limit %d", row_limit);
    TM_SLICED(H, segsum(g, in + c0, ld_in, out + c0, ld_out, w, 0, -1.0f, 0, compact_out, stream, row_limit));
    return segsum(g, in, ld_in, out, ld_out, H, 0, -1.0f, 0, compact_out, stream, row_limit);
}
int tmpnn_segsum_bwd(const tmpnn_graph* g, const float* d_out, int ld_dout, float* d_in, int ld_din, int H,
                     int accumulate, tmpnn_stream stream) {
    TM_SLICED(H, gather(g, d_out + c0, ld_dout, d_in + c0, ld_din, w, accumulate, false, stream));
    return gather(g, d_out, ld_dout, d_in, ld_din, H, accumulate, false, stream);
}

int tmpnn_transpose(const float* in, int rows, int cols, float* out, tmpnn_stream stream) {
    TM_REQUIRE(in && out && rows > 0 && cols > 0, "transpose: bad arguments");
    dim3 grid(ceil_div(cols, 32), ceil_div(rows, 32)), block(32, 8);
    hipLaunchKernelGGL(k_transpose, grid, block, 0, as_stream(stream), in, rows, cols, out);
    return check_launch("transpose");
}

}
```

trackmpnn_amd/csrc/dense.hip:

```cpp
#include "common.h"

namespace tmpnn {

static constexpr float BN_EPS = 1e-5f;
static constexpr float BN_MOMENTUM = 0.1f;

__global__ __launch_bounds__(256) void k_gemm(GemmArgs g, int kper, float* slab) {
    __shared__ float As[16][68];
    __shared__ float Bs[16][68];
    const int tid = threadIdx.x;
    const int tx = tid & 15, ty = tid >> 4;
    const int m0 = blockIdx.y * 64, n0 = blockIdx.x * 64;
    const int kbeg = blockIdx.z * kper;
    const int kend = min(g.K, kbeg + kper);
    float acc[4][4] = {};
    const bool va = (reinterpret_cast<uintptr_t>(g.A) & 15) == 0 && ((g.sak == 1 ? g.sam : g.sak) & 3) == 0;
    const bool vb = (reinterpret_cast<uintptr_t>(g.B) & 15) == 0 && ((g.sbn == 1 ? g.sbk : g.sbn) & 3) == 0;
    for (int k0 = kbeg; k0 < kend; k0 += 16) {
        const bool fullk = k0 + 16 <= kend;
        if (fullk && m0 + 64 <= g.M && !g.a_krows && g.sak == 1 && va) {
            const int m = tid >> 2, kq = (tid & 3) * 4;
            const long ar = g.a_rows ? g.a_rows[m0 + m] : (m0 + m);
            const float4 v = *reinterpret_cast<const float4*>(g.A + ar * g.sam + k0 + kq);
            As[kq][m] = v.x; As[kq + 1][m] = v.y; As[kq + 2][m] = v.z; As[kq + 3][m] = v.w;
        } else if (fullk && m0 + 64 <= g.M && !g.a_rows && g.sam == 1 && va) {
            const int k = tid >> 4, mq = (tid & 15) * 4;
            const long ak = g.a_krows ? g.a_krows[k0 + k] : (k0 + k);
            *reinterpret_cast<float4*>(&As[k][mq]) = *reinterpret_cast<const float4*>(g.A + ak * g.sak + m0 + mq);
        } else {
#pragma unroll
            for (int i = 0; i < 4; ++i) {
                const int idx = tid + i * 256;
                int m, k;
                if (g.sak == 1) { k = idx & 15; m = idx >> 4; } else { m = idx & 63; k = idx >> 6; }
                float v = 0.f;
                if (m0 + m < g.M && k0 + k < kend) {
                    const long ar = g.a_rows ? g.a_rows[m0 + m] : (m0 + m);
                    const long ak = g.a_krows ? g.a_krows[k0 + k] : (k0 + k);
                    v = g.A[ar * g.sam + ak * g.sak];
                }
                As[k][m] = v;
            }
        }
        if (fullk && n0 + 64 <= g.N && g.sbn == 1 && vb) {
            const int k = tid >> 4, nq = (tid & 15) * 4;
            *reinterpret_cast<float4*>(&Bs[k][nq]) = *reinterpret_cast<const float4*>(g.B + (long)(k0 + k) * g.sbk + n0 + nq);
        } else if (fullk && n0 + 64 <= g.N && g.sbk == 1 && vb) {
            const int n = tid >> 2, kq = (tid & 3) * 4;
            const float4 v = *reinterpret_cast<const float4*>(g.B + (long)(n0 + n) * g.sbn + k0 + kq);
            Bs[kq][n] = v.x; Bs[kq + 1][n] = v.y; Bs[kq + 2][n] = v.z; Bs[kq + 3][n] = v.w;
        } else {
#pragma unroll
            for (int i = 0; i < 4; ++i) {
                const int idx = tid + i * 256;
                int n, k;
                if (g.sbn == 1) { n = idx & 63; k = idx >> 6; } else { k = idx & 15; n = idx >> 4; }
                float v = 0.f;
                if (n0 + n < g.N && k0 + k < kend) v = g.B[(long)(k0 + k) * g.sbk + (long)(n0 + n) * g.sbn];
                Bs[k][n] = v;
            }
        }
        __syncthreads();
#pragma unroll
        for (int k = 0; k < 16; ++k) {
            float a[4], b[4];
#pragma unroll
            for (int i = 0; i < 4; ++i) { a[i] = As[k][ty * 4 + i]; b[i] = Bs[k][tx * 4 + i]; }
#pragma unroll
            for (int i = 0; i < 4; ++i)
#pragma unroll
                for (int j = 0; j < 4; ++j) acc[i][j] += a[i] * b[j];
        }
        __syncthreads();
    }
    const bool vc = n0 + tx * 4 + 3 < g.N &&
                    (slab ? (g.N & 3) == 0 && (reinterpret_cast<uintptr_t>(slab) & 15) == 0
                          : (g.ldc & 3) == 0 && (reinterpret_cast<uintptr_t>(g.C) & 15) == 0 &&
                                (!g.bias || (reinterpret_cast<uintptr_t>(g.bias) & 15) == 0));
#pragma unroll
    for (int i = 0; i < 4; ++i) {
        const int m = m0 + ty * 4 + i;
        if (m >= g.M) continue;
        if (vc) {
            const int n = n0 + tx * 4;
            float4 v = make_float4(acc[i][0], acc[i][1], acc[i][2], acc[i][3]);
            if (slab) {
                *reinterpret_cast<float4*>(slab + (size_t)blockIdx.z * g.M * g.N + (size_t)m * g.N + n) = v;
            } else {
                if (g.bias) {
                    const float4 b = *reinterpret_cast<const float4*>(g.bias + n);
                    v.x += b.x; v.y += b.y; v.z += b.z; v.w += b.w;
                }
                const long cr = g.c_rows ? g.c_rows[m] : m;
                float4* p = reinterpret_cast<float4*>(g.C + cr * g.ldc + n);
                if (g.accumulate) { const float4 o = *p; v.x = o.x + v.x; v.y = o.y + v.y; v.z = o.z + v.z; v.w = o.w + v.w; }
                *p = v;
            }
            continue;
        }
#pragma unroll
        for (int j = 0; j < 4; ++j) {
            const int n = n0 + tx * 4 + j;
            if (n >= g.N) continue;
            if (slab) {
                slab[(size_t)blockIdx.z * g.M * g.N + (size_t)m * g.N + n] = acc[i][j];
            } else {
                const long cr = g.c_rows ? g.c_rows[m] : m;
                float v = acc[i][j] + (g.bias ? g.bias[n] : 0.f);
                float* p = g.C + cr * g.ldc + n;
                *p = g.accumulate ? *p + v : v;
            }
        }
    }
}

int launch_gemm(const GemmArgs& g, hipStream_t st) {
    if (g.M <= 0 || g.N <= 0) return TMPNN_OK;
    dim3 grid(ceil_div(g.N, 64), ceil_div(g.M, 64), 1), block(256);
    hipLaunchKernelGGL(k_gemm, grid, block, 0, st, g, g.K > 0 ? g.K : 1, (float*)nullptr);
    return check_launch("gemm");
}

static int splitk_plan(int K, int* kper) {
    int nsplit = (K + 127) / 128;
    if (nsplit > 1024) nsplit = 1024;
    if (nsplit < 1) nsplit = 1;
    int kp = (K + nsplit - 1) / nsplit;
    kp = (kp + 15) & ~15;
    if (kp < 16) kp = 16;
    nsplit = (K + kp - 1) / kp;
    if (nsplit < 1) nsplit = 1;
    *kper = kp;
    return nsplit;
}

size_t gemm_splitk_ws_floats(int M, int N, int K) {
    int kper;
    const int ns = splitk_plan(K, &kper);
    return (size_t)ns * M * N + reduce_slabs_ws_floats(ns, (size_t)M * N);
}

int launch_gemm_splitk(const GemmArgs& g, float* ws, size_t ws_floats, hipStream_t st) {
    if (g.M <= 0 || g.N <= 0) return TMPNN_OK;
    if (g.K <= 0) return TMPNN_OK;
    int kper;
    const int ns = splitk_plan(g.K, &kper);
    if (ws_floats < gemm_splitk_ws_floats(g.M, g.N, g.K))
        return set_error(TMPNN_EWORKSPACE, "gemm_splitk: workspace too small");
    if (ns == 1) return launch_gemm(g, st);
    float* ws2 = ws + (size_t)ns * g.M * g.N;
    dim3 grid(ceil_div(g.N, 64), ceil_div(g.M, 64), ns), block(256);
    hipLaunchKernelGGL(k_gemm, grid, block, 0, st, g, kper, ws);
    int rc = check_launch("gemm_splitk");
// ... 292 lines not shown
        const float4 g = *reinterpret_cast<const float4*>(gamma + j), b = *reinterpret_cast<const float4*>(beta + j);
        *reinterpret_cast<float4*>(a_out + idx) = make_float4(fmaxf(yh.x * g.x + b.x, 0.f), fmaxf(yh.y * g.y + b.y, 0.f),
                                                              fmaxf(yh.z * g.z + b.z, 0.f), fmaxf(yh.w * g.w + b.w, 0.f));
    }
}

__global__ void k_running_to_stats(const float* __restrict__ rm, const float* __restrict__ rv, int H,
                                   float* __restrict__ mean, float* __restrict__ rstd) {
    const int j = blockIdx.x * blockDim.x + threadIdx.x;
    if (j >= H) return;
    mean[j] = rm[j];
    rstd[j] = rsqrtf(rv[j] + BN_EPS);
}

__global__ void k_bn_bwd_act(float* __restrict__ da, const float* __restrict__ yhat, int nd, int H,
                             const float* __restrict__ gamma, const float* __restrict__ beta,
                             float* __restrict__ dz_out) {
    const size_t idx = ((size_t)blockIdx.x * blockDim.x + threadIdx.x) * 4;
    if (idx >= (size_t)nd * H) return;
    const int j = (int)(idx % H);
    const float4 yh = *reinterpret_cast<const float4*>(yhat + idx), d = *reinterpret_cast<const float4*>(da + idx);
    const float4 g = *reinterpret_cast<const float4*>(gamma + j), b = *reinterpret_cast<const float4*>(beta + j);
    const float4 dz = make_float4(yh.x * g.x + b.x > 0.f ? d.x : 0.f, yh.y * g.y + b.y > 0.f ? d.y : 0.f,
                                  yh.z * g.z + b.z > 0.f ? d.z : 0.f, yh.w * g.w + b.w > 0.f ? d.w : 0.f);
    *reinterpret_cast<float4*>(dz_out + idx) = dz;
    *reinterpret_cast<float4*>(da + idx) = make_float4(dz.x * g.x, dz.y * g.y, dz.z * g.z, dz.w * g.w);
}

__global__ void k_bn_bwd_seg(const float* __restrict__ dyhat, const float* __restrict__ yhat,
                             const int32_t* __restrict__ seg_ptr, const int32_t* __restrict__ seg_cnt, int H,
                             const float* __restrict__ b1, const float* __restrict__ mean,
                             const float* __restrict__ rstd, float* __restrict__ s1, float* __restrict__ s2) {
    __shared__ float red[2048];
    const int s = blockIdx.x, j = threadIdx.x, g = threadIdx.y, G = blockDim.y;
    const int p0 = seg_ptr[s], p1 = seg_ptr[s + 1];
    float a = 0.f, b = 0.f;
#pragma unroll 4
    for (int i = p0 + g; i < p1; i += G) {
        const float d = dyhat[(size_t)i * H + j];
        a += d;
        b += d * yhat[(size_t)i * H + j];
    }
    if (G > 1) {
        red[g * H + j] = a;
        red[1024 + g * H + j] = b;
        __syncthreads();
        a = 0.f; b = 0.f;
        for (int k = 0; k < G; ++k) { a += red[k * H + j]; b += red[1024 + k * H + j]; }
    }
    if (g == 0) {
        s1[(size_t)s * H + j] = a;
        s2[(size_t)s * H + j] = b;
    }
}

__global__ void k_bn_bwd_dy(float* __restrict__ dyhat, const float* __restrict__ yhat, int nd, int H,
                            const int32_t* __restrict__ seg_ptr, const int32_t* __restrict__ seg_cnt, int S,
                            const int32_t* __restrict__ seg_of_det,
                            const float* __restrict__ rstd, const float* __restrict__ s1,
                            const float* __restrict__ s2, int training) {
    const size_t idx = ((size_t)blockIdx.x * blockDim.x + threadIdx.x) * 4;
    if (idx >= (size_t)nd * H) return;
    const int i = (int)(idx / H), j = (int)(idx % H);
    float4 d = *reinterpret_cast<const float4*>(dyhat + idx);
    if (!training) {
        const float4 r = *reinterpret_cast<const float4*>(rstd + j);
        *reinterpret_cast<float4*>(dyhat + idx) = make_float4(d.x * r.x, d.y * r.y, d.z * r.z, d.w * r.w);
        return;
    }
    const int s = seg_of_det ? seg_of_det[i] : seg_of(seg_ptr, S, i);
    const float cnt = (float)seg_cnt[s];
    const size_t sj = (size_t)s * H + j;
    const float4 r = *reinterpret_cast<const float4*>(rstd + sj), a1 = *reinterpret_cast<const float4*>(s1 + sj);
    const float4 a2 = *reinterpret_cast<const float4*>(s2 + sj), yh = *reinterpret_cast<const float4*>(yhat + idx);
    d.x = r.x / cnt * (cnt * d.x - a1.x - yh.x * a2.x);
    d.y = r.y / cnt * (cnt * d.y - a1.y - yh.y * a2.y);
    d.z = r.z / cnt * (cnt * d.z - a1.z - yh.z * a2.z);
    d.w = r.w / cnt * (cnt * d.w - a1.w - yh.w * a2.w);
    *reinterpret_cast<float4*>(dyhat + idx) = d;
}

__global__ void k_bn_bwd_dy0(float* __restrict__ s1, float* __restrict__ s2, const int32_t* __restrict__ seg_ptr,
                             const int32_t* __restrict__ seg_cnt, int S, int H, const float* __restrict__ b1,
                             const float* __restrict__ mean, const float* __restrict__ rstd) {
    const size_t idx = (size_t)blockIdx.x * blockDim.x + threadIdx.x;
    if (idx >= (size_t)S * H) return;
    const int s = (int)(idx / H), j = (int)(idx % H);
    const float cnt = (float)seg_cnt[s];
    const float nz = cnt - (float)(seg_ptr[s + 1] - seg_ptr[s]);
    const float yh0 = (b1[j] - mean[idx]) * rstd[idx];
    const float dy0 = rstd[idx] / cnt * (-s1[idx] - yh0 * s2[idx]);
    s1[idx] = dy0;
    s2[idx] = nz * dy0;
}

__global__ void k_gather_rows(const float* __restrict__ src, long ld, const int32_t* __restrict__ rows, int n, int H,
                              float* __restrict__ dst) {
    const size_t idx = ((size_t)blockIdx.x * blockDim.x + threadIdx.x) * 4;
    if (idx >= (size_t)n * H) return;
    const int i = (int)(idx / H), j = (int)(idx % H);
    *reinterpret_cast<float4*>(dst + idx) = *reinterpret_cast<const float4*>(src + (size_t)rows[i] * ld + j);
}

__global__ __launch_bounds__(256) void k_heads_fwd(const float* __restrict__ h, int ld_h, int C, int N,
                                                   const uint8_t* __restrict__ is_edge,
                                                   const float* __restrict__ w_node, const float* __restrict__ b_node,
                                                   const float* __restrict__ w_edge, const float* __restrict__ b_edge,
                                                   float* __restrict__ logits, float* __restrict__ scores) {
    const int sub = threadIdx.x & 15;
    const long rows_per_pass = (long)gridDim.x * 16;
    for (long i = (long)blockIdx.x * 16 + (threadIdx.x >> 4); i < N; i += rows_per_pass) {
        const bool e = is_edge[i] != 0;
        const float* w = e ? w_edge : w_node;
        const float* hr = h + (size_t)i * ld_h;
        float s = 0.f;
        for (int c4 = sub * 4; c4 < C; c4 += 64) {
            const float4 x = *reinterpret_cast<const float4*>(hr + c4);
            const float4 ww = *reinterpret_cast<const float4*>(w + c4);
            s += x.x * ww.x + x.y * ww.y + x.z * ww.z + x.w * ww.w;
        }
        s += __shfl_xor(s, 8);
        s += __shfl_xor(s, 4);
        s += __shfl_xor(s, 2);
        s += __shfl_xor(s, 1);
        if (sub == 0) {
            const float y = s + (e ? b_edge[0] : b_node[0]);
            logits[i] = y;
            scores[i] = 1.0f / (1.0f + expf(-y));
        }
    }
}

__global__ void k_heads_finish(const float* __restrict__ parts, size_t stride, int nparts, int N,
                               const uint8_t* __restrict__ is_edge, const float* __restrict__ b_node,
                               const float* __restrict__ b_edge, float* __restrict__ logits,
                               float* __restrict__ scores) {
    const int i = blockIdx.x * blockDim.x + threadIdx.x;
    if (i >= N) return;
    float y = is_edge[i] ? b_edge[0] : b_node[0];
    for (int p = 0; p < nparts; ++p) y += parts[(size_t)p * stride + i];
    logits[i] = y;
    scores[i] = 1.0f / (1.0f + expf(-y));
}

__global__ __launch_bounds__(256) void k_heads_bwd(const float* __restrict__ h, int ld_h, int C, int N,
                                                   const uint8_t* __restrict__ is_edge,
                                                   const float* __restrict__ w_node, const float* __restrict__ w_edge,
                                                   const float* __restrict__ scores, const float* __restrict__ d_logits,
                                                   const float* __restrict__ d_scores, float* __restrict__ dy_out,
                                                   float* __restrict__ d_h,
                                                   int ld_dh, int accumulate, int rows_per_block,
                                                   float* __restrict__ part) {
    extern __shared__ float sm[];
    const int cpt = C >> 2;
    const int slots = 256 / cpt;
    const int slot = threadIdx.x / cpt;
    const int c4 = (threadIdx.x % cpt) * 4;
    const bool active = slot < slots;
    float4 an = make_float4(0.f, 0.f, 0.f, 0.f), ae = an;
    float bn = 0.f, be = 0.f;
    const long r0 = (long)blockIdx.x * rows_per_block;
    const long r1 = min((long)N, r0 + rows_per_block);
    if (active) {
        constexpr int UR = 4;
        for (long i0 = r0 + slot; i0 < r1; i0 += (long)slots * UR) {
            float dyv[UR];
            bool ev[UR], live[UR];
            float4 xv[UR];
#pragma unroll
            for (int u = 0; u < UR; ++u) {
                const long i = i0 + (long)u * slots;
                live[u] = i < r1;
                const long ic = live[u] ? i : r1 - 1;
                float dy = d_logits ? d_logits[ic] : 0.f;
                if (d_scores) {
                    const float sc = scores[ic];
                    dy += d_scores[ic] * sc * (1.0f - sc);
                }
                dyv[u] = live[u] ? dy : 0.f;
                ev[u] = is_edge[ic] != 0;
                xv[u] = *reinterpret_cast<const float4*>(h + (size_t)ic * ld_h + c4);
            }
#pragma unroll
            for (int u = 0; u < UR; ++u) {
                if (!live[u]) continue;
                const long i = i0 + (long)u * slots;
                const float dy = dyv[u];
                const bool e = ev[u];
                const float4 x = xv[u];
                if (dy_out && c4 == 0) dy_out[i] = dy;
                if (d_h) {
                    const float4 w = *reinterpret_cast<const float4*>((e ? w_edge : w_node) + c4);
                    float* dp = d_h + (size_t)i * ld_dh + c4;
                    float4 o = make_float4(dy * w.x, dy * w.y, dy * w.z, dy * w.w);
                    if (accumulate) {
                        const float4 p = *reinterpret_cast<const float4*>(dp);
                        o.x += p.x; o.y += p.y; o.z += p.z; o.w += p.w;
                    }
                    *reinterpret_cast<float4*>(dp) = o;
                }
                if (e) { ae.x += dy * x.x; ae.y += dy * x.y; ae.z += dy * x.z; ae.w += dy * x.w; if (c4 == 0) be += dy; }
                else   { an.x += dy * x.x; an.y += dy * x.y; an.z += dy * x.z; an.w += dy * x.w; if (c4 == 0) bn += dy; }
            }
        }
        float* my = sm + (size_t)slot * 2 * C;
        *reinterpret_cast<float4*>(my + c4) = an;
        *reinterpret_cast<float4*>(my + C + c4) = ae;
        if (c4 == 0) {
            sm[(size_t)slots * 2 * C + slot * 2 + 0] = bn;
            sm[(size_t)slots * 2 * C + slot * 2 + 1] = be;
        }
    }
    __syncthreads();
    float* out = part + (size_t)blockIdx.x * (2 * C + 2);
    for (int j = threadIdx.x; j < 2 * C + 2; j += 256) {
        float s = 0.f;
        if (j < 2 * C) for (int k = 0; k < slots; ++k) s += sm[(size_t)k * 2 * C + j];
        else for (int k = 0; k < slots; ++k) s += sm[(size_t)slots * 2 * C + k * 2 + (j - 2 * C)];
        out[j] = s;
    }
}

__global__ void k_heads_bwd_final(const float* __restrict__ red, int C, float* __restrict__ dw_node,
                                  float* __restrict__ db_node, float* __restrict__ dw_edge,
                                  float* __restrict__ db_edge) {
    const int j = blockIdx.x * blockDim.x + threadIdx.x;
    if (j >= 2 * C + 2) return;
    const float s = red[j];
    if (j < C) dw_node[j] += s;
    else if (j < 2 * C) dw_edge[j - C] += s;
    else if (j == 2 * C) db_node[0] += s;
    else db_edge[0] += s;
}

static int heads_rows_per_block(int N) {
    long rpb = ((long)N + 2047) / 2048;
    if (rpb < 64) rpb = 64;
    return (int)rpb;
}

}

using namespace tmpnn;

extern "C" {

int tmpnn_input_bn_fwd(const float* xdet, int ld_x, int F, int nd, const int32_t* seg_ptr, const int32_t* seg_cnt,
                       const int32_t* seg_of_det, int S, int H, int training, const float* w1, const float* b1, const float* gamma,
                       const float* beta, float* running_mean, float* running_var, const float* w2, const float* b2,
                       float* y_save, float* mean, float* rstd, float* ws_a, const int32_t* out_row, float* h_new,
                       int ld_h, tmpnn_stream stream) {
    TM_REQUIRE(supported_H_cell(H), "input_bn_fwd: unsupported H=%d", H);
    TM_REQUIRE(F > 0 && nd >= 0 && S >= 0, "input_bn_fwd: F=%d nd=%d S=%d", F, nd, S);
    TM_REQUIRE(w1 && b1 && gamma && beta && running_mean && running_var && w2 && b2 && mean && rstd,
               "input_bn_fwd: null parameter pointer");
    TM_REQUIRE(!training || (seg_ptr && seg_cnt && S > 0), "input_bn_fwd: training needs segments");
    hipStream_t st = as_stream(stream);
    int rc;
    if (nd > 0) {
        TM_REQUIRE(xdet && y_save && ws_a && out_row && h_new && ld_x >= F && ld_h >= H, "input_bn_fwd: null/short buffers");
        TM_REQUIRE(aligned16(y_save) && aligned16(ws_a) && aligned16(mean) && aligned16(rstd) && aligned16(gamma) && aligned16(beta),
                   "input_bn_fwd: y_save / ws_a / mean / rstd / gamma / beta must be 16-byte aligned");
        GemmArgs g{xdet, ld_x, 1, nullptr, nullptr, w1, 1, F, b1, y_save, H, nullptr, nd, H, F, 0};
        if ((rc = launch_gemm(g, st))) return rc;
    }
    if (training) {
        hipLaunchKernelGGL(k_bn_stats, dim3(S), dim3(H, bn_row_groups(nd, S, H)), 0, st, y_save, seg_ptr, seg_cnt, H, b1, mean, rstd);
        if ((rc = check_launch("bn_stats"))) return rc;
        hipLaunchKernelGGL(k_bn_running, dim3(H), dim3(64), 0, st, mean, rstd, seg_cnt, S, H, running_mean,
                           running_var);
        if ((rc = check_launch("bn_running"))) return rc;
    } else {
        hipLaunchKernelGGL(k_running_to_stats, dim3(ceil_div(H, 64)), dim3(64), 0, st, running_mean, running_var, H,
                           mean, rstd);
        if ((rc = check_launch("running_to_stats"))) return rc;
    }
    if (nd == 0) return TMPNN_OK;
    hipLaunchKernelGGL(k_bn_apply, dim3(ceil_div((long)nd * H / 4, 256)), dim3(256), 0, st, y_save, nd, H,
                       training ? seg_ptr : nullptr, S, seg_of_det, mean, rstd, gamma, beta, (float*)nullptr, ws_a);
    if ((rc = check_launch("bn_apply"))) return rc;
    GemmArgs g2{ws_a, H, 1, nullptr, nullptr, w2, 1, H, b2, h_new, ld_h, out_row, nd, H, H, 0};
    return launch_gemm(g2, st);
}

int tmpnn_input_bn_bwd(const float* xdet, int ld_x, int F, int nd, const int32_t* seg_ptr, const int32_t* seg_cnt,
                       const int32_t* seg_of_det, int S, int H, int training, const float* w1, const float* b1, const float* gamma,
                       const float* beta, const float* w2, const float* y_save, const float* mean, const float* rstd,
                       const int32_t* out_row, const float* d_h, int ld_dh, float* d_xdet, int ld_dx, float* d_xzero,
                       float* dw1, float* db1, float* dgamma, float* dbeta, float* dw2, float* db2, float* ws,
                       size_t ws_floats, tmpnn_stream stream) {
    TM_REQUIRE(supported_H_cell(H), "input_bn_bwd: unsupported H=%d", H);
    TM_REQUIRE(F > 0 && nd >= 0 && S >= 0, "input_bn_bwd: F=%d nd=%d S=%d", F, nd, S);
    TM_REQUIRE(w1 && b1 && gamma && beta && w2 && mean && rstd && dw1 && db1 && dgamma && dbeta && dw2 && db2,
               "input_bn_bwd: null parameter pointer");
    hipStream_t st = as_stream(stream);
    if (nd == 0) {
        if (d_xzero && S > 0) (void)hipMemsetAsync(d_xzero, 0, sizeof(float) * (size_t)S * F, st);
        return TMPNN_OK;
    }
    TM_REQUIRE(xdet && y_save && out_row && d_h && ws, "input_bn_bwd: null buffers");
    const size_t ndH = (size_t)nd * H, SH = (size_t)(S > 0 ? S : 1) * H;
    const size_t need = tmpnn_input_bn_bwd_ws(nd, S, H, F);
    if (ws_floats < need) return set_error(TMPNN_EWORKSPACE, "input_bn_bwd: workspace %zu < %zu floats", ws_floats, need);
    TM_REQUIRE(aligned16(y_save) && aligned16(mean) && aligned16(rstd) && aligned16(gamma) && aligned16(beta) && aligned16(ws) &&
                   aligned16(d_h) && (ld_dh & 3) == 0,
               "input_bn_bwd: y_save / mean / rstd / gamma / beta / ws / d_h must be 16-byte aligned (ld_dh a multiple of 4)");
    float* B0 = ws;
    float* B1 = B0 + ndH;
    float* B2 = B1 + ndH;
    float* s1 = B2 + ndH;
    float* s2 = s1 + SH;
    float* scratch = s2 + SH;
    const size_t scratch_n = ws_floats - (3 * ndH + 2 * SH);
    const int gridE = ceil_div((long)ndH / 4, 256);
    int rc;
    hipLaunchKernelGGL(k_gather_rows, dim3(gridE), dim3(256), 0, st, d_h, (long)ld_dh, out_row, nd, H, B0);
    if ((rc = check_launch("gather_rows"))) return rc;
    hipLaunchKernelGGL(k_bn_apply, dim3(gridE), dim3(256), 0, st, y_save, nd, H, training ? seg_ptr : nullptr, S,
                       seg_of_det, mean, rstd, gamma, beta, B1, B2);
    if ((rc = check_launch("bn_apply"))) return rc;
    {
        GemmArgs g{B0, 1, H, nullptr, nullptr, B2, H, 1, nullptr, dw2, H, nullptr, H, H, nd, 1};
        if ((rc = launch_gemm_splitk(g, scratch, scratch_n, st))) return rc;
        if ((rc = launch_colsum(B0, H, nullptr, 0, nd, H, db2, 1, scratch, scratch_n, st))) return rc;
    }
    {
        GemmArgs g{B0, H, 1, nullptr, nullptr, w2, H, 1, nullptr, B2, H, nullptr, nd, H, H, 0};
        if ((rc = launch_gemm(g, st))) return rc;
    }
    hipLaunchKernelGGL(k_bn_bwd_act, dim3(gridE), dim3(256), 0, st, B2, B1, nd, H, gamma, beta, B0);
    if ((rc = check_launch("bn_bwd_act"))) return rc;
    if ((rc = launch_colsum(B0, H, B1, H, nd, H, dgamma, 1, scratch, scratch_n, st))) return rc;
    if ((rc = launch_colsum(B0, H, nullptr, 0, nd, H, dbeta, 1, scratch, scratch_n, st))) return rc;
    if (training) {
        hipLaunchKernelGGL(k_bn_bwd_seg, dim3(S), dim3(H, bn_row_groups(nd, S, H)), 0, st, B2, B1, seg_ptr, seg_cnt, H, b1, mean, rstd, s1, s2);
        if ((rc = check_launch("bn_bwd_seg"))) return rc;
    }
    hipLaunchKernelGGL(k_bn_bwd_dy, dim3(gridE), dim3(256), 0, st, B2, B1, nd, H, seg_ptr, seg_cnt, S, seg_of_det, rstd,
                       s1, s2, training);
    if ((rc = check_launch("bn_bwd_dy"))) return rc;
    {
        GemmArgs g{B2, 1, H, nullptr, nullptr, xdet, ld_x, 1, nullptr, dw1, F, nullptr, H, F, nd, 1};
        if ((rc = launch_gemm_splitk(g, scratch, scratch_n, st))) return rc;
        if ((rc = launch_colsum(B2, H, nullptr, 0, nd, H, db1, 1, scratch, scratch_n, st))) return rc;
        if (d_xdet) {
            GemmArgs gx{B2, H, 1, nullptr, nullptr, w1, F, 1, nullptr, d_xdet, ld_dx, nullptr, nd, F, H, 0};
            if ((rc = launch_gemm(gx, st))) return rc;
        }
    }
    if (training) {
        hipLaunchKernelGGL(k_bn_bwd_dy0, dim3(ceil_div((long)S * H, 256)), dim3(256), 0, st, s1, s2, seg_ptr, seg_cnt,
                           S, H, b1, mean, rstd);
        if ((rc = check_launch("bn_bwd_dy0"))) return rc;
        const size_t cs2 = colsum_ws_floats(S, H);
        if (scratch_n < cs2) return set_error(TMPNN_EWORKSPACE, "input_bn_bwd: workspace too small for segments");
        if ((rc = launch_colsum(s2, H, nullptr, 0, S, H, db1, 1, scratch, scratch_n, st))) return rc;
        if (d_xzero) {
            GemmArgs gz{s1, H, 1, nullptr, nullptr, w1, F, 1, nullptr, d_xzero, F, nullptr, S, F, H, 0};
            if ((rc = launch_gemm(gz, st))) return rc;
        }
    } else if (d_xzero && S > 0) {
        (void)hipMemsetAsync(d_xzero, 0, sizeof(float) * (size_t)S * F, st);
    }
    return TMPNN_OK;
}

size_t tmpnn_input_bn_bwd_ws(int nd, int S, int H, int F) {
    if (nd <= 0) return 0;
    const size_t ndH = (size_t)nd * H, SH = (size_t)(S > 0 ? S : 1) * H;
    size_t x = colsum_ws_floats(nd, H);
    const size_t a = gemm_splitk_ws_floats(H, H, nd), b = gemm_splitk_ws_floats(H, F, nd),
                 c = colsum_ws_floats(S > 0 ? S : 1, H);
    if (a > x) x = a;
    if (b > x) x = b;
    if (c > x) x = c;
    return 3 * ndH + 2 * SH + x;
}

int tmpnn_heads_fwd(const float* h, int ld_h, int C, int N, const uint8_t* is_edge, const float* w_node,
                    const float* b_node, const float* w_edge, const float* b_edge, float* logits, float* scores,
                    tmpnn_stream stream) {
    TM_REQUIRE(C > 0 && (C & 3) == 0 && N >= 0, "heads_fwd: C=%d N=%d", C, N);
    if (N == 0) return TMPNN_OK;
    TM_REQUIRE(h && is_edge && w_node && b_node && w_edge && b_edge && logits && scores, "heads_fwd: null pointer");
    TM_REQUIRE(ld_h >= C && (ld_h & 3) == 0 && aligned16(h) && aligned16(w_node) && aligned16(w_edge),
               "heads_fwd: rows must be 16-byte aligned");
    long b = ((long)N + 15) / 16;
    if (b > 4096) b = 4096;
    hipLaunchKernelGGL(k_heads_fwd, dim3((int)b), dim3(256), 0, as_stream(stream), h, ld_h, C, N, is_edge, w_node,
                       b_node, w_edge, b_edge, logits, scores);
    return check_launch("heads_fwd");
}

int tmpnn_heads_finish(const float* parts, size_t part_stride, int nparts, int N, const uint8_t* is_edge,
                       const float* b_node, const float* b_edge, float* logits, float* scores, tmpnn_stream stream) {
    TM_REQUIRE(nparts > 0 && N >= 0, "heads_finish: nparts=%d N=%d", nparts, N);
    if (N == 0) return TMPNN_OK;
    TM_REQUIRE(parts && is_edge && b_node && b_edge && logits && scores && part_stride >= (size_t)N, "heads_finish: null pointer");
    hipLaunchKernelGGL(k_heads_finish, dim3(ceil_div(N, 256)), dim3(256), 0, as_stream(stream), parts, part_stride, nparts, N,
                       is_edge, b_node, b_edge, logits, scores);
    return check_launch("heads_finish");
}

size_t tmpnn_heads_bwd_ws(int N, int C) {
    if (N <= 0) return 0;
    const int rpb = heads_rows_per_block(N);
    const int nblk = ceil_div(N, rpb);
    const size_t n = 2 * (size_t)C + 2;
    return ((size_t)nblk * n + n + reduce_slabs_ws_floats(nblk, n)) * sizeof(float);
}

int tmpnn_heads_bwd(const float* h, int ld_h, int C, int N, const uint8_t* is_edge, const float* w_node,
                    const float* w_edge, const float* scores, const float* d_logits, const float* d_scores,
                    float* dy_out, float* d_h, int ld_dh, int accumulate, float* dw_node, float* db_node,
                    float* dw_edge, float* db_edge, void* ws, size_t ws_bytes, tmpnn_stream stream) {
    TM_REQUIRE(C > 0 && (C & 3) == 0 && C <= 1024 && N >= 0, "heads_bwd: C=%d N=%d", C, N);
    if (N == 0) return TMPNN_OK;
    TM_REQUIRE(h && is_edge && w_node && w_edge && dw_node && db_node && dw_edge && db_edge, "heads_bwd: null pointer");
    TM_REQUIRE(d_scores == nullptr || scores != nullptr, "heads_bwd: d_scores needs scores");
    TM_REQUIRE((ld_h & 3) == 0 && aligned16(h) && aligned16(w_node) && aligned16(w_edge) &&
                   (d_h == nullptr || ((ld_dh & 3) == 0 && aligned16(d_h))),
               "heads_bwd: rows must be 16-byte aligned");
    const size_t need = tmpnn_heads_bwd_ws(N, C);
    if (!ws || ws_bytes < need) return set_error(TMPNN_EWORKSPACE, "heads_bwd: workspace %zu < %zu", ws_bytes, need);
    const int rpb = heads_rows_per_block(N);
    const int nblk = ceil_div(N, rpb);
    const int cpt = C >> 2;
    TM_REQUIRE(cpt <= 256, "heads_bwd: C too wide");
    const int slots = 256 / cpt;
    const size_t shm = ((size_t)slots * 2 * C + (size_t)slots * 2) * sizeof(float);
    hipStream_t st = as_stream(stream);
    hipLaunchKernelGGL(k_heads_bwd, dim3(nblk), dim3(256), shm, st, h, ld_h, C, N, is_edge, w_node, w_edge, scores,
                       d_logits, d_scores, dy_out, d_h, ld_dh, accumulate, rpb, reinterpret_cast<float*>(ws));
    int rc = check_launch("heads_bwd");
    if (rc) return rc;
    const size_t nred = 2 * (size_t)C + 2;
    float* part = reinterpret_cast<float*>(ws);
    float* red = part + (size_t)nblk * nred;
    if ((rc = launch_reduce_slabs(part, nred, nblk, red, nred, 0, st, red + nred))) return rc;
    hipLaunchKernelGGL(k_heads_bwd_final, dim3(ceil_div(2 * C + 2, 256)), dim3(256), 0, st, red, C, dw_node, db_node,
                       dw_edge, db_edge);
    return check_launch("heads_bwd_final");
}

}
```

trackmpnn_amd/functional.py:

```python
from __future__ import annotations

import contextlib
import ctypes
import os
from dataclasses import dataclass
from types import SimpleNamespace
from typing import Dict, List, Optional, Sequence, Tuple

import torch

from . import _lib
from .graph import CallPlan, dense_seg_plan, edge_tiles, win_plan

ATT_DROPOUT_P = 0.5
INPLACE_GRADS = os.environ.get('TMPNN_INPLACE_GRADS', '0') == '1'
FUSED_BWD = os.environ.get('TMPNN_FUSED_BWD', '1') == '1'
ZERO_STATE_BWD = os.environ.get('TMPNN_BWD_ZERO_STATE', '1') != '0'
ZERO_STATE_FWD = os.environ.get('TMPNN_FWD_ZERO_STATE', '1') != '0'
WIDE_OVERLAP = os.environ.get('TMPNN_WIDE_OVERLAP', '0') == '1' and os.environ.get('TMPNN_KEEP_VARIANTS', '0') == '1'
ATT_KMAX = 8
_SPLIT = os.environ.get('TMPNN_SPLIT', '1')[:1] != '0'

_VARIANTS = os.environ.get('TMPNN_KEEP_VARIANTS', '0') == '1'


def _variant(name: str, default: str) -> str:
    return os.environ.get(name, default) if _VARIANTS else default


WIDE_DW = _variant('TMPNN_WIDE_DW', '1') == '1'
WIDE_DET = _variant('TMPNN_WIDE_DET', '1') == '1'
WIDE = _variant('TMPNN_WIDE', '1') != '0' and _SPLIT
WIDE_TILED = _variant('TMPNN_WIDE_TILED', '1') != '0'
FWD_TILED = _variant('TMPNN_FWD_TILED', '1') != '0' and _SPLIT
FWD_TILE_ROWS = 16 if _variant('TMPNN_FWD_TILE_ROWS', '32') == '16' else 32
INPUT_TF = _variant('TMPNN_INPUT_TF', '1') != '0'
RECOMPUTE_GATES = _variant('TMPNN_RECOMPUTE_GATES', '0') == '1'
CONCAT_PROJ = _variant('TMPNN_CONCAT_PROJ', '1') != '0'
ZS_RECOMPUTE = _variant('TMPNN_ZS_RECOMPUTE', '1') != '0'
WIN_SEGSUM = _variant('TMPNN_SEGSUM_WIN', '0') == '1'
WIDE_FUSED_ADJOINT = _variant('TMPNN_WIDE_FUSED_ADJOINT', '1') != '0'
_aux_streams: Dict[torch.device, 'torch.cuda.Stream'] = {}


def _aux_stream(dev) -> Optional[int]:
    if not WIDE_OVERLAP or torch.cuda.is_current_stream_capturing():
        return None
    key = torch.device(dev)
    s = _aux_streams.get(key)
    if s is None:
        s = torch.cuda.Stream(key)
        _aux_streams[key] = s
    if s.cuda_stream == torch.cuda.current_stream(key).cuda_stream:
        return None
    return s.cuda_stream


def _seg_plan_guard(g, dev, on_aux: bool) -> None:
    plan = g.__dict__.get('_seg_plan')
    if plan is None or torch.cuda.is_current_stream_capturing():
        return
    cur = _aux_streams[torch.device(dev)] if on_aux else torch.cuda.current_stream(dev)
    last = plan.__dict__.get('_last_stream')
    if last is not None and last.cuda_stream != cur.cuda_stream:
        ev = torch.cuda.Event()
        ev.record(last)
        cur.wait_event(ev)
    plan._last_stream = cur


_aux_events: Dict[torch.device, tuple] = {}


def _aux_event_pair(dev):
    key = torch.device(dev)
    ev = _aux_events.get(key)
    if ev is None:
        with torch.cuda.device(key):
            ev = (torch.cuda.Event(enable_timing=False), torch.cuda.Event(enable_timing=False))
            for e in ev:
                e.record(torch.cuda.current_stream(key))
        _aux_events[key] = ev
    return ev


_wide_ws: Dict[torch.device, torch.Tensor] = {}


def _wide_workspace(nbytes: int, dev, slot: int = 0) -> torch.Tensor:
    key = (torch.device(dev), slot)
    ws = _wide_ws.get(key)
    if ws is None or ws.numel() * 4 < nbytes + 16:
        _wide_ws.pop(key, None)
        ws = torch.empty((nbytes // 4 + 4,), dtype=torch.float32, device=dev)
        _wide_ws[key] = ws
    return ws


_weight_images = None


@contextlib.contextmanager
def weight_cache():
    global _weight_images
    prev = _weight_images
    _weight_images = {}
    try:
        yield
    finally:
        _weight_images = prev


def _cached(key, sources, build):
    if _weight_images is None:
        return build()
    hit = _weight_images.get(key)
    if hit is None:
        hit = _weight_images[key] = (sources, build())
    return hit[1]


def _wide_prep(w_ih: torch.Tensor, w_hh: torch.Tensor, H: int) -> torch.Tensor:
    def build():
        nb = int(_lib.load().tmpnn_wide_prep_bytes(H, H))
        prep = torch.empty((nb // 4 + 4,), dtype=torch.float32, device=w_ih.device)
        _lib.call('tmpnn_wide_prepare', w_ih.data_ptr(), w_hh.data_ptr(), H, H, prep.data_ptr(), _stream())
        return prep
    return _cached(('wide', w_ih.data_ptr(), w_hh.data_ptr(), H), (w_ih, w_hh), build)


@dataclass(frozen=True)
class ModelSpec:
    groups: Tuple[Tuple[str, int], ...]
    H: int
    K: int
    msg_type: str

    @property
    def G(self) -> int:
        return len(self.groups)

    @property
    def IN_e(self) -> int:
        return 2 * self.H if self.msg_type == 'concat' else self.H

    @property
    def F_total(self) -> int:
        return sum(f for _, f in self.groups)

    def param_names(self) -> List[str]:
        names = []
        for g in range(self.G):
            t = f'input_transforms.{g}.'
            names += [t + '0.weight', t + '0.bias', t + '1.weight', t + '1.bias', t + '3.weight', t + '3.bias']
        for g in range(self.G):
            f = f'factor_grus.{g}.'
            names += [f + 'edge_gru.weight_ih', f + 'edge_gru.weight_hh', f + 'edge_gru.bias_ih', f + 'edge_gru.bias_hh']
            for k in range(self.K):
                names += [f + f'gat.{k}.W_att', f + f'gat.{k}.a']
            names += [f + 'node_gru.weight_ih', f + 'node_gru.weight_hh', f + 'node_gru.bias_ih', f + 'node_gru.bias_hh']
        names += ['output_transform_node.weight', 'output_transform_node.bias',
                  'output_transform_edge.weight', 'output_transform_edge.bias']
        return names


def _stream() -> int:
    return _lib.raw_stream()


def _keep_bits(keep, K: int, n: int, dev) -> torch.Tensor:
    n = max(n, 1)
    if keep is None:
        if ATT_DROPOUT_P == 0.5:
            return torch.empty((n,), dtype=torch.uint8, device=dev).random_(0, 1 << K)
        keep = torch.empty((K, n), dtype=torch.uint8, device=dev).bernoulli_(1.0 - ATT_DROPOUT_P)
    keep = (keep != 0).to(torch.uint8)
    bits = keep[0].clone()
    for k in range(1, K):
        bits |= keep[k] << k
    return bits.contiguous()


def _require_device(t: torch.Tensor, what: str):
    if not t.is_cuda:
        raise RuntimeError(f'{what} is on {t.device}: trackmpnn_amd runs on the MI355X HIP kernels only '
                           '(no CPU or torch fallback exists)')


def _f32c(t: torch.Tensor) -> torch.Tensor:
    if t.dtype != torch.float32:
        t = t.float()
    return t if t.is_contiguous() else t.contiguous()


def _transpose(w: torch.Tensor) -> torch.Tensor:
    def build():
        out = torch.empty((w.shape[1], w.shape[0]), dtype=torch.float32, device=w.device)
        _lib.call('tmpnn_transpose', w.data_ptr(), w.shape[0], w.shape[1], out.data_ptr(), _stream())
        return out
    return _cached(('t', w.data_ptr(), w.shape[0], w.shape[1]), (w,), build)


@dataclass(frozen=True)
class CallRoute:
    n: int
    E_old: int
    save: bool
    edge_fwd: str
    tile_rows: int
    agg: str
    zs_fwd: bool
    zs_bwd: bool
    zs_groups: Tuple[bool, ...]
    zs_rc: bool
    recompute_gates: bool
    cw: int
    tf: Tuple[bool, ...]
    tf_all: bool
    dense_plan: bool
    win_plan: bool
    bwd_fused: bool
    edge_bwd: str
    gather_bwd: bool

    @property
    def wide(self) -> bool:
        return self.edge_fwd in ('wide_tiled', 'wide_rows')

    @property
    def new_rows_unread(self) -> bool:
        return self.zs_fwd and (self.zs_bwd or not self.save)


def _input_tf(plan: CallPlan, H: int, F: int, caps) -> bool:
    return (INPUT_TF and plan.max_seg_nd >= 0 and plan.seg_of_det is not None
            and bool(caps.tmpnn_input_tf_supported(H, F, plan.max_seg_nd)))


def plan_route(spec: ModelSpec, plan: CallPlan, P: Dict[str, torch.Tensor], save: bool, caps=None) -> CallRoute:
    if caps is None:
        caps = _lib.load()
    g = plan.graph
    H, G, K, IN_e = spec.H, spec.G, spec.K, spec.IN_e
    E, Dn, n = g.E, g.Dn, plan.n_new
    diff = spec.msg_type == 'diff'
    xmode = 1 if diff else 2
    has_pos = g.src_pos is not None and Dn > 0
    nd = int(plan.new_det_row.numel()) if n > 0 else 0
    E_old = E - (n - nd) if n > 0 else E
    if WIDE and diff and H >= 128 and bool(caps.tmpnn_wide_supported(H, H)) and has_pos and E > 0:
        edge_fwd = 'wide_tiled' if WIDE_TILED else 'wide_rows'
    elif CONCAT_PROJ and not diff and H <= 64 and FWD_TILED and has_pos and E > 0:
        edge_fwd = 'concat_proj'
    elif diff and H <= 64 and has_pos:
        edge_fwd = 'proj_tiled' if FWD_TILED and E > 0 else 'proj_rows'
    else:
        edge_fwd = 'generic'
    recompute = edge_fwd == 'proj_tiled' and RECOMPUTE_GATES and save
    zs_rows = n > 0 and K == 0 and diff and 0 <= E_old < E
    aligned = (tuple((P[f'factor_grus.{gi}.edge_gru.bias_hh'].data_ptr() + 4 * 2 * H) % 16 == 0 for gi in range(G))
               if zs_rows else (False,) * G)
    zs_fwd = (ZERO_STATE_FWD and zs_rows and edge_fwd == 'proj_tiled' and H == 64 and FWD_TILE_ROWS == 32
              and not RECOMPUTE_GATES and all(aligned) and bool(caps.tmpnn_gru_fwd_tiles_zero_state_available(H, 3)))
    bwd_fused = bool(save and FUSED_BWD and caps.tmpnn_gru_bwd_fused_available(H, H, 0)
                     and caps.tmpnn_gru_bwd_fused_available(H, IN_e, xmode))
    zs_bwd = bool(bwd_fused and ZERO_STATE_BWD and zs_rows and not recompute and any(aligned)
                  and caps.tmpnn_gru_bwd_fused_zero_state_available(H, IN_e, xmode))
    zs_rc = zs_fwd and zs_bwd and ZS_RECOMPUTE
    proj_table = edge_fwd in ('concat_proj', 'proj_tiled', 'proj_rows')
    cw = min(caps.tmpnn_gru_fwd_head_parts(H, H if edge_fwd == 'concat_proj' else IN_e, 3 if proj_table else xmode),
             caps.tmpnn_gru_fwd_head_parts(H, H, 0))
    tf = tuple(_input_tf(plan, H, F, caps) for _, F in spec.groups) if n > 0 else (False,) * G
    wide = edge_fwd in ('wide_tiled', 'wide_rows')
    if not save:
        edge_bwd = ''
    elif bwd_fused:
        edge_bwd = 'fused'
    elif wide and WIDE_DET:
        edge_bwd = 'wide_det_fused' if K == 0 and WIDE_FUSED_ADJOINT else 'wide_det'
    elif wide:
        edge_bwd = 'wide_data_dw' if WIDE_DW else 'wide_data'
    else:
        edge_bwd = 'generic'
    return CallRoute(n=n, E_old=E_old, save=save, edge_fwd=edge_fwd, tile_rows=FWD_TILE_ROWS,
                     agg='attention' if K > 0 else 'segsum', zs_fwd=zs_fwd, zs_bwd=zs_bwd,
                     zs_groups=tuple(zs_bwd and a for a in aligned), zs_rc=zs_rc, recompute_gates=recompute, cw=cw,
                     tf=tf, tf_all=nd > 0 and all(tf), dense_plan=wide and H % 256 == 0 and K == 0,
                     win_plan=WIN_SEGSUM and H == 64 and E > 0, bwd_fused=bwd_fused, edge_bwd=edge_bwd,
                     gather_bwd=edge_bwd not in ('wide_det_fused', 'wide_det'))


@dataclass
class SavedCall:
    route: CallRoute
    h_cat: Optional[torch.Tensor] = None
    gates: Optional[torch.Tensor] = None
    es: Optional[torch.Tensor] = None
    h_out: Optional[torch.Tensor] = None
    scores: Optional[torch.Tensor] = None
    att: Optional[list] = None
    wide: Optional[list] = None
    proj: Optional[dict] = None
    xdet: Optional[torch.Tensor] = None
    xrows: Optional[torch.Tensor] = None
    y_save: Optional[list] = None
    mean: Optional[list] = None
    rstd: Optional[list] = None


def _call_dims(spec: ModelSpec, plan: CallPlan, dev) -> SimpleNamespace:
    g = plan.graph
    return SimpleNamespace(spec=spec, plan=plan, g=g, H=spec.H, G=spec.G, K=spec.K, GH=spec.G * spec.H, IN_e=spec.IN_e,
                           N=g.N, E=g.E, Dn=g.Dn, n=plan.n_new, N_old=g.N - plan.n_new, plane=g.N * spec.H,
                           xmode=2 if spec.msg_type == 'concat' else 1, dev=dev, st=_stream(),
                           opts=dict(dtype=torch.float32, device=dev))


_CELL = ('weight_ih', 'weight_hh', 'bias_ih', 'bias_hh')


def _cell_ptrs(T: Dict[str, torch.Tensor], prefix: str) -> Tuple[int, int, int, int]:
    return tuple(T[prefix + s].data_ptr() for s in _CELL)


def _tf_head(tf: bool, plan: CallPlan, xg: int, xrows, Ft: int, F: int, nd: int, H: int) -> tuple:
    segs = (plan.seg_ptr.data_ptr(), plan.seg_cnt.data_ptr(), _lib.ptr(plan.seg_of_det), plan.S)
    if tf:
        return (xg, _lib.ptr(xrows), Ft, F, nd, *segs, plan.max_seg_nd, H)
    return (xg, Ft, F, nd, *segs, H)



def _fwd_state(c, route: CallRoute, h_in: Optional[torch.Tensor], h_spare: int) -> torch.Tensor:
    N, GH, n, N_old = c.N, c.GH, c.n, c.N_old
    h_cat = None
    if h_in is not None and N_old > 0 and n > 0 and h_in.is_contiguous():
        st_ = h_in.untyped_storage()
        if h_spare >= n and st_.nbytes() >= 4 * (h_in.storage_offset() + N * GH):
            h_cat = torch.empty(0, **c.opts).set_(st_, h_in.storage_offset(), (N, GH), (GH, 1))
    if h_cat is None:
        if h_in is not None and n == 0:
            h_cat = h_in
        else:
            h_cat = torch.empty((N, GH), **c.opts)
            if N_old > 0:
                h_cat[:N_old].copy_(h_in)
    if n > 0 and not route.new_rows_unread:
        h_cat[N_old:].zero_()
    return h_cat


def _fwd_input_transform(c, route: CallRoute, x, h_cat, P, buffers, training: bool, saved: SavedCall) -> None:
    spec, plan, H, GH = c.spec, c.plan, c.H, c.GH
    nd = int(plan.new_det_row.numel())
    S = plan.S
    if training and plan.min_seg_cnt <= 1:
        raise ValueError('Expected more than 1 value per channel when training, got input size '
                         f'[1, {H}]')
    if route.tf_all:
        xsrc, xrows = _f32c(x.detach()), plan.new_det_local
        if xrows.dtype != torch.int64 or not xrows.is_contiguous():
            xrows = xrows.long().contiguous()
    else:
        xsrc = _f32c(x.detach().index_select(0, plan.new_det_local)) if nd > 0 else torch.empty((0, spec.F_total), **c.opts)
        xrows = None
    ws_a = torch.empty((max(nd, 1), H), **c.opts)
    y_saves, means, rstds = [], [], []
    f0 = 0
    for gi, (_, F) in enumerate(spec.groups):
        t = f'input_transforms.{gi}.'
        y_save = torch.empty((max(nd, 1), H), **c.opts)
        SS = S if training else 1
        mean = torch.empty((SS, H), **c.opts)
        rstd = torch.empty((SS, H), **c.opts)
        tf = route.tf[gi]
        args = (*_tf_head(tf, plan, xsrc.data_ptr() + 4 * f0, xrows, spec.F_total, F, nd, H), int(training),
                P[t + '0.weight'].data_ptr(), P[t + '0.bias'].data_ptr(), P[t + '1.weight'].data_ptr(), P[t + '1.bias'].data_ptr(),
                buffers[t + '1.running_mean'].data_ptr(), buffers[t + '1.running_var'].data_ptr(),
                P[t + '3.weight'].data_ptr(), P[t + '3.bias'].data_ptr(), y_save.data_ptr(), mean.data_ptr(), rstd.data_ptr())
        if not tf:
            args += (ws_a.data_ptr(),)
        _lib.call('tmpnn_input_tf_fwd' if tf else 'tmpnn_input_bn_fwd', *args,
                  plan.new_det_row.data_ptr(), h_cat.data_ptr() + 4 * gi * H, GH, c.st)
        if training:
            buffers[t + '1.num_batches_tracked'] += S
        y_saves.append(y_save)
        means.append(mean)
        rstds.append(rstd)
        f0 += F
    if route.save:
        saved.xdet, saved.xrows, saved.y_save, saved.mean, saved.rstd = xsrc, xrows, y_saves, means, rstds


def _fwd_group(c, route: CallRoute, gi: int, P, h_cat, h_out, gates, parts) -> SimpleNamespace:
    f = f'factor_grus.{gi}.'
    H, cw = c.H, route.cw
    e_wih, e_whh = P[f + 'edge_gru.weight_ih'], P[f + 'edge_gru.weight_hh']
    q = SimpleNamespace(gi=gi, f=f, e_wih=e_wih, e_whh=e_whh,
                        hg=h_cat.data_ptr() + 4 * gi * H, og=h_out.data_ptr() + 4 * gi * H,
                        gp=gates[gi].data_ptr() if gates is not None else None,
                        part=(parts.data_ptr() + 4 * gi * cw * c.N) if cw > 0 else None,
                        we=(P['output_transform_edge.weight'].data_ptr() + 4 * gi * H) if cw > 0 else None,
                        wn=(P['output_transform_node.weight'].data_ptr() + 4 * gi * H) if cw > 0 else None,
                        e_bih=P[f + 'edge_gru.bias_ih'].data_ptr(), e_bhh=P[f + 'edge_gru.bias_hh'].data_ptr(),
                        n_bih=P[f + 'node_gru.bias_ih'].data_ptr(), n_bhh=P[f + 'node_gru.bias_hh'].data_ptr())
    q.e_wih_t, q.e_whh_t = _transpose(e_wih), _transpose(e_whh)
    q.n_wih_t, q.n_whh_t = _transpose(P[f + 'node_gru.weight_ih']), _transpose(P[f + 'node_gru.weight_hh'])
    return q


def _fwd_edge_wide(c, route: CallRoute, q, saved: SavedCall):
    g, H, GH, E, Dn = c.g, c.H, c.GH, c.E, c.Dn
    prep = _wide_prep(q.e_wih, q.e_whh, H)
    if route.save:
        saved.wide.append(prep)
    proj = torch.empty((Dn, 3 * H), **c.opts)
    if route.edge_fwd == 'wide_tiled':
        _lib.call('tmpnn_wide_gru_fwd_tiled', prep.data_ptr(), g.det_row.data_ptr(), Dn, edge_tiles(g, 128).cref(), E,
                  q.hg, GH, H, q.e_bih, q.e_bhh, proj.data_ptr(), q.og, GH, q.gp, c.plane, c.st)
    else:
        _lib.call('tmpnn_wide_gru_fwd', prep.data_ptr(), g.det_row.data_ptr(), Dn, g.edge_row.data_ptr(), E,
                  g.src_pos.data_ptr(), g.dst_pos.data_ptr(), q.hg, GH, H, q.e_bih, q.e_bhh,
                  proj.data_ptr(), q.og, GH, q.gp, c.plane, c.st)
    return prep, proj


def _fwd_edge_tiles(c, route: CallRoute, q, proj, saved: SavedCall) -> None:
    g, H, GH, E, E_old = c.g, c.H, c.GH, c.E, route.E_old
    E_full = E_old if route.zs_fwd else E
    if E_full > 0:
        tiles = edge_tiles(g, route.tile_rows, e1=E_full)
        _lib.call('tmpnn_gru_fwd_tiles', tiles.cref(), E_full, proj.data_ptr(), 3 * H, q.hg, GH, H,
                  q.e_whh_t.data_ptr(), q.e_bih, q.e_bhh,
                  q.og, GH, None if route.recompute_gates else q.gp, c.plane, q.we, q.part, c.N, c.st)
    if route.zs_fwd:
        _lib.call('tmpnn_gru_fwd_tiles_zero_state', edge_tiles(g, route.tile_rows, e0=E_old).cref(), E - E_old,
                  proj.data_ptr(), 3 * H, H, q.e_bih,
                  q.e_bhh, q.og, GH, None if route.zs_rc else q.gp, c.plane,
                  int(route.save and not route.zs_bwd), q.we, q.part, c.N, c.st)
    if route.zs_rc or route.recompute_gates:
        saved.proj[q.gi] = (proj, q.e_whh_t if route.recompute_gates else None)

# ... 24 lines not shown
    if arm == 'proj_tiled':
        _fwd_edge_tiles(c, route, q, proj, saved)
    else:
        _lib.call('tmpnn_gru_fwd', g.edge_row.data_ptr(), E, 3, g.src_pos.data_ptr(), g.dst_pos.data_ptr(),
                  proj.data_ptr(), 3 * H, 0, H, q.hg, GH, H, None, q.e_whh_t.data_ptr(), q.e_bih, q.e_bhh,
                  q.og, GH, q.gp, c.plane, q.we, q.part, c.N, st)
    return proj


def _fwd_attention(c, q, es, P, training: bool, keep):
    g, H, GH, E, Dn, K, opts = c.g, c.H, c.GH, c.E, c.Dn, c.K, c.opts
    erec, inc_other = g.att_index() if E > 0 else (None, None)
    groups, al = [], []
    for k0 in range(0, K, ATT_KMAX):
        Kg = min(ATT_KMAX, K - k0)
        Ws = [P[q.f + f'gat.{k}.W_att'] for k in range(k0, k0 + Kg)]
        As = [P[q.f + f'gat.{k}.a'] for k in range(k0, k0 + Kg)]
        W = _cached(('attW', tuple(t.data_ptr() for t in Ws)), tuple(Ws), lambda: torch.cat(Ws, 1).contiguous())
        a = _cached(('atta', tuple(t.data_ptr() for t in As)), tuple(As),
                    lambda: torch.stack([t.reshape(-1) for t in As]).contiguous())
        ws_ha = torch.empty((max(Dn, 1), Kg * H), **opts)
        score = torch.empty((max(2 * E, 1), Kg), **opts)
        stats = torch.empty((max(Dn, 1), Kg, 2), **opts)
        esk = torch.empty((Kg, max(Dn, 1), H), **opts)
        alpha = torch.empty((Kg, max(2 * E, 1)), **opts)
        kp = None
        if training:
            kp = _keep_bits(None if keep is None else keep[q.gi][k0:k0 + Kg], Kg, 2 * E, c.dev)
        out_g = es if Kg == K else torch.empty_like(es)
        _lib.call('tmpnn_att_fwd', g.cref(), _lib.ptr(erec), q.hg, GH, H, Kg, W.data_ptr(),
                  a.data_ptr(), _lib.ptr(kp), ATT_DROPOUT_P, ws_ha.data_ptr(), score.data_ptr(), stats.data_ptr(),
                  esk.data_ptr(), alpha.data_ptr(), out_g.data_ptr(), H, c.st)
        if Kg != K:
            if k0 == 0:
                torch.mul(out_g, Kg / K, out=es)
            else:
                es.add_(out_g, alpha=Kg / K)
        al += [alpha[k, :2 * E] for k in range(Kg)]
        groups.append((k0, Kg, W, a, kp, ws_ha, score, stats, esk))
    return al, groups


def _fwd_aggregate(c, route: CallRoute, q, es, P, training: bool, keep, zero_from: int, st_det, on_aux: bool, saved):
    if route.agg == 'segsum':
        _seg_plan_guard(c.g, c.dev, on_aux)
        _lib.call('tmpnn_segsum_fwd_live', c.g.cref(), q.hg, c.GH, es.data_ptr(), c.H, c.H, 1, zero_from, st_det)
        return None
    al, groups = _fwd_attention(c, q, es, P, training, keep)
    if route.save:
        saved.att.append(groups)
    return al


def _fwd_node_cell(c, q, es, st_det) -> None:
    _lib.call('tmpnn_gru_fwd', c.g.det_row.data_ptr(), c.Dn, 0, None, None,
              es.data_ptr(), c.H, 1, c.H, q.hg, c.GH, c.H,
              q.n_wih_t.data_ptr(), q.n_whh_t.data_ptr(), q.n_bih, q.n_bhh,
              q.og, c.GH, q.gp, c.plane, q.wn, q.part, c.N, st_det)


def _fwd_heads(c, route: CallRoute, P, parts, h_out):
    g, N, GH = c.g, c.N, c.GH
    logits = torch.empty((N, 1), **c.opts)
    scores = torch.empty((N, 1), **c.opts)
    if route.cw > 0:
        _lib.call('tmpnn_heads_finish', parts.data_ptr(), N, c.G * route.cw, N, g.is_edge.data_ptr(),
                  P['output_transform_node.bias'].data_ptr(), P['output_transform_edge.bias'].data_ptr(),
                  logits.data_ptr(), scores.data_ptr(), c.st)
    else:
        _lib.call('tmpnn_heads_fwd', h_out.data_ptr(), GH, GH, N, g.is_edge.data_ptr(),
                  P['output_transform_node.weight'].data_ptr(), P['output_transform_node.bias'].data_ptr(),
                  P['output_transform_edge.weight'].data_ptr(), P['output_transform_edge.bias'].data_ptr(),
                  logits.data_ptr(), scores.data_ptr(), c.st)
    return scores, logits


def _aux_fork(c):
    aux = _aux_stream(c.dev)
    if aux is None:
        return c.st, None
    aux_obj = _aux_streams[torch.device(c.dev)]
    fork, _ = _aux_event_pair(c.dev)
    fork.record(torch.cuda.current_stream(c.dev))
    aux_obj.wait_event(fork)
    return aux, aux_obj


def mp_forward(spec: ModelSpec, plan: CallPlan, x: torch.Tensor, h_in: Optional[torch.Tensor],
               P: Dict[str, torch.Tensor], buffers: Dict[str, torch.Tensor], training: bool, save: bool,
               keep: Optional[Sequence[torch.Tensor]] = None, reserve_rows: int = 0, h_spare: int = 0):
    c = _call_dims(spec, plan, x.device)
    g, H, G, K, GH, N, Dn, n, dev, st, opts = c.g, c.H, c.G, c.K, c.GH, c.N, c.Dn, c.n, c.dev, c.st, c.opts
    if h_in is None:
        if c.N_old != 0:
            raise ValueError(f'h_in is None but the graph has {c.N_old} rows that are not new')
    else:
        if h_in.shape[0] != c.N_old or h_in.shape[1] != GH:
            raise ValueError(f'h_in must be [{c.N_old}, {GH}] (N - n, G*H), got {tuple(h_in.shape)}')
    if x.shape[0] != n or (n > 0 and x.shape[1] != spec.F_total):
        raise ValueError(f'x must be [{n}, {spec.F_total}], got {tuple(x.shape)}')

    route = plan_route(spec, plan, P, save)
    saved = SavedCall(route, att=[], wide=[] if route.wide else None, proj={})
    h_cat = _fwd_state(c, route, h_in, h_spare)
    if n > 0:
        _fwd_input_transform(c, route, x, h_cat, P, buffers, training, saved)

    spare = max(int(reserve_rows), 0)
    if spare > 0:
        buf = torch.empty(((N + spare) * GH,), **opts)
        h_out = torch.empty(0, **opts).set_(buf.untyped_storage(), 0, (N, GH), (GH, 1))
    else:
        h_out = torch.empty((N, GH), **opts)
    gates = torch.empty((G, 4, N, H), **opts) if save else None
    es_all = torch.empty((G, max(Dn, 1), H), **opts)
    alphas: List[Optional[List[torch.Tensor]]] = []
    if route.dense_plan:
        dense_seg_plan(g)
    if route.win_plan:
        win_plan(g)
    zero_from = c.N_old if n > 0 else N
    parts = torch.empty((G * route.cw, N), **opts) if route.cw > 0 else None
    for gi in range(G):
        q = _fwd_group(c, route, gi, P, h_cat, h_out, gates, parts)
        st_det, aux_obj = _aux_fork(c) if route.wide and K == 0 else (st, None)
        held = _fwd_edge_cell(c, route, q, saved)
        es = es_all[gi]
        alphas.append(_fwd_aggregate(c, route, q, es, P, training, keep, zero_from, st_det, aux_obj is not None, saved))
        _fwd_node_cell(c, q, es, st_det)
        if aux_obj is not None:
            _, join = _aux_event_pair(dev)
            join.record(aux_obj)
            torch.cuda.current_stream(dev).wait_event(join)
        del held
    scores, logits = _fwd_heads(c, route, P, parts, h_out)
    if save:
        saved.h_cat, saved.gates, saved.es, saved.h_out, saved.scores = h_cat, gates, es_all, h_out, scores
    return scores, logits, h_out, alphas, saved



def _bwd_grads(spec: ModelSpec, P, opts, grad_out) -> Dict[str, torch.Tensor]:
    if grad_out is not None:
        return dict(grad_out)
    names = spec.param_names()
    sizes = [P[nm].numel() for nm in names]
    offs = [0]
    for sz in sizes:
        offs.append(offs[-1] + ((sz + 63) // 64) * 64)
    flat = torch.zeros((offs[-1],), **opts)
    return {nm: flat[o:o + sz].view(P[nm].shape) for nm, o, sz in zip(names, offs, sizes)}


def _bwd_heads(c, saved: SavedCall, P, grads, d_scores, d_logits, d_hout):
    g, N, GH, opts = c.g, c.N, c.GH, c.opts
    lib = _lib.load()
    dh_up = _f32c(d_hout) if d_hout is not None else None
    dy = None
    if d_scores is not None or d_logits is not None:
        dy = torch.empty((N,), **opts)
        dl = _f32c(d_logits) if d_logits is not None else None
        ds = _f32c(d_scores) if d_scores is not None else None
        for c0 in range(0, GH, 1024):
            cw_ = min(1024, GH - c0)
            ws_b = lib.tmpnn_heads_bwd_ws(N, cw_)
            ws = torch.empty((max(ws_b // 4, 1),), **opts)
            db_n = grads['output_transform_node.bias'] if c0 == 0 else torch.zeros((1,), **opts)
            db_e = grads['output_transform_edge.bias'] if c0 == 0 else torch.zeros((1,), **opts)
            _lib.call('tmpnn_heads_bwd', saved.h_out.data_ptr() + 4 * c0, GH, cw_, N, g.is_edge.data_ptr(),
                      P['output_transform_node.weight'].data_ptr() + 4 * c0, P['output_transform_edge.weight'].data_ptr() + 4 * c0,
                      saved.scores.data_ptr(), _lib.ptr(dl), _lib.ptr(ds), dy.data_ptr(), None, 0, 0,
                      grads['output_transform_node.weight'].data_ptr() + 4 * c0, db_n.data_ptr(),
                      grads['output_transform_edge.weight'].data_ptr() + 4 * c0, db_e.data_ptr(),
                      ws.data_ptr(), ws_b, c.st)
    elif dh_up is None:
        dh_up = torch.zeros((N, GH), **opts)
    return dy, dh_up


def _bwd_group(c, gi: int, saved: SavedCall, P, grads, dy, dh_up, d_hcat, dmsg, ws_w) -> SimpleNamespace:
    f = f'factor_grus.{gi}.'
    H = c.H
    return SimpleNamespace(gi=gi, f=f, hg=saved.h_cat.data_ptr() + 4 * gi * H,
                           dog=(dh_up.data_ptr() + 4 * gi * H) if dh_up is not None else None,
                           dhg=d_hcat.data_ptr() + 4 * gi * H, gp=saved.gates[gi].data_ptr(), es=saved.es[gi],
                           dyp=_lib.ptr(dy), dmsg=dmsg.data_ptr(), ws=ws_w.data_ptr(), ws_bytes=ws_w.numel() * 4,
                           wn=(P['output_transform_node.weight'].data_ptr() + 4 * gi * H) if dy is not None else None,
                           we=(P['output_transform_edge.weight'].data_ptr() + 4 * gi * H) if dy is not None else None,
                           e=_cell_ptrs(P, f + 'edge_gru.'), n=_cell_ptrs(P, f + 'node_gru.'),
                           ge=_cell_ptrs(grads, f + 'edge_gru.'), gn=_cell_ptrs(grads, f + 'node_gru.'))


def _bwd_node_cell(c, route: CallRoute, q) -> None:
    g, H, GH, Dn, IN_e, st = c.g, c.H, c.GH, c.Dn, c.IN_e, c.st
    if route.bwd_fused:
        _lib.call('tmpnn_gru_bwd_fused', g.det_row.data_ptr(), Dn, 0, None, None, q.es.data_ptr(), H, 1, H,
                  q.hg, GH, H, q.n[0], q.n[1],
                  q.gp, c.plane, q.dog, GH, q.dyp, q.wn, q.dmsg, IN_e, q.dhg, GH, None, None, None, 0,
                  *q.gn, q.ws, q.ws_bytes, st)
        return
    _lib.call('tmpnn_gru_bwd_data', g.det_row.data_ptr(), Dn, H, q.hg, GH, H, q.n[0], q.n[1],
              q.gp, c.plane, q.dog, GH, q.dyp, q.wn, q.dmsg, IN_e, q.dhg, GH, None, None, None, 0, st)
    _lib.call('tmpnn_gru_bwd_weights', g.det_row.data_ptr(), Dn, 0, None, None, q.es.data_ptr(), H, 1, H,
              q.hg, GH, H, q.gp, c.plane, q.dog, GH, q.dyp, q.wn, *q.gn, q.ws, q.ws_bytes, st)


def _bwd_edge_fused(c, route: CallRoute, q, saved: SavedCall) -> None:
    g, H, GH, N, E, IN_e, st, E_old = c.g, c.H, c.GH, c.N, c.E, c.IN_e, c.st, route.E_old
    fuse = c.K == 0
    if route.recompute_gates:
        proj_s, whh_t_s = saved.proj[q.gi]
        h_scr = _wide_workspace(4 * N * GH, c.dev, slot=2)
        _lib.call('tmpnn_gru_fwd_tiles', edge_tiles(g, route.tile_rows).cref(), E, proj_s.data_ptr(), 3 * H, q.hg, GH, H,
                  whh_t_s.data_ptr(), q.e[2], q.e[3],
                  h_scr.data_ptr() + 4 * q.gi * H, GH, q.gp, c.plane, None, None, 0, st)
    zs = route.zs_groups[q.gi]
    E_full = E_old if zs else E
    if E_full > 0:
        _lib.call('tmpnn_gru_bwd_fused', g.edge_row.data_ptr(), E_full, c.xmode, g.src.data_ptr(), g.dst.data_ptr(),
                  None, 0, 0, IN_e, q.hg, GH, H, q.e[0], q.e[1],
                  q.gp, c.plane, q.dog, GH, q.dyp, q.we, q.dmsg, IN_e, q.dhg, GH,
                  g.src.data_ptr() if fuse else None, g.dst.data_ptr() if fuse else None,
                  q.dmsg if fuse else None, IN_e, *q.ge, q.ws, q.ws_bytes, st)
    if zs:
        zg, zplane = q.gp, c.plane
        if route.zs_rc:
            src_ = _lib.CZsGateSrc(saved.proj[q.gi][0].data_ptr(), 3 * H, g.src_pos.data_ptr() + 4 * E_old,
                                   g.dst_pos.data_ptr() + 4 * E_old, q.e[2], q.e[3])
            zg, zplane = ctypes.addressof(src_), 0
        _lib.call('tmpnn_gru_bwd_fused_zero_state', g.edge_row.data_ptr() + 4 * E_old, E - E_old,
                  g.src.data_ptr() + 4 * E_old, g.dst.data_ptr() + 4 * E_old, IN_e, q.hg, GH, H,
                  q.e[0], q.e[3] + 4 * 2 * H, zg, zplane, q.dog, GH, q.dyp, q.we,
                  q.dmsg, IN_e, q.ge[0], q.ge[2], q.ge[3], q.ws, q.ws_bytes, st)


def _bwd_edge_weights(c, q) -> None:
    g = c.g
    _lib.call('tmpnn_gru_bwd_weights', g.edge_row.data_ptr(), c.E, c.xmode, g.src.data_ptr(), g.dst.data_ptr(),
              None, 0, 0, c.IN_e, q.hg, c.GH, c.H, q.gp, c.plane, q.dog, c.GH, q.dyp, q.we, *q.ge, q.ws, q.ws_bytes, c.st)


def _bwd_edge_generic(c, q) -> None:
    g, IN_e = c.g, c.IN_e
    fuse = c.K == 0
    _lib.call('tmpnn_gru_bwd_data', g.edge_row.data_ptr(), c.E, IN_e, q.hg, c.GH, c.H, q.e[0], q.e[1],
              q.gp, c.plane, q.dog, c.GH, q.dyp, q.we, q.dmsg, IN_e, q.dhg, c.GH,
              g.src.data_ptr() if fuse else None, g.dst.data_ptr() if fuse else None,
              q.dmsg if fuse else None, IN_e, c.st)
    _bwd_edge_weights(c, q)


def _bwd_edge_wide_det(c, route: CallRoute, q, prep: int) -> None:
    g, H, GH, IN_e, dev, st = c.g, c.H, c.GH, c.IN_e, c.dev, c.st
    fuse = c.K == 0
    wsb = int(_lib.load().tmpnn_wide_gru_bwd_diff_ws(c.N, c.E, c.Dn, H))
    ws_wide = _wide_workspace(wsb, dev)
    aux = _aux_stream(dev)
    args = (prep, g.cref(), q.hg, GH, H, q.gp, c.plane, q.dog, GH, q.dyp, q.we, q.dhg, GH, *q.ge,
            ws_wide.data_ptr(), wsb, st)
    evf = evj = None
    if aux is not None:
        ef, ej = _aux_event_pair(dev)
        evf, evj = ef.cuda_event, ej.cuda_event
        if not evf or not evj:
            aux = evf = evj = None
    _seg_plan_guard(g, dev, aux is not None)
    if route.edge_bwd == 'wide_det_fused':
        _lib.call('tmpnn_wide_gru_bwd_diff_fused', *args[:-1], q.dmsg, IN_e, st, aux, evf, evj)
        return
    if aux is not None:
        _lib.call('tmpnn_wide_gru_bwd_diff_aux', *args, aux, evf, evj)
    else:
        _lib.call('tmpnn_wide_gru_bwd_diff', *args)
    if fuse:
        _lib.call('tmpnn_gather_diff_fwd', g.cref(), q.dmsg, IN_e, q.dhg, GH, H, 1, st)


def _bwd_edge_wide(c, route: CallRoute, q, saved: SavedCall) -> None:
    g, H, GH, E, IN_e, dev, st = c.g, c.H, c.GH, c.E, c.IN_e, c.dev, c.st
    prep = saved.wide[q.gi].data_ptr()
    if route.edge_bwd in ('wide_det_fused', 'wide_det'):
        _bwd_edge_wide_det(c, route, q, prep)
        return
    lib = _lib.load()
    wsb = int(lib.tmpnn_wide_gru_bwd_data_ws(E, H))
    ws_wide = _wide_workspace(wsb, dev)
    _lib.call('tmpnn_wide_gru_bwd_data', prep, g.edge_row.data_ptr(), E, q.hg, GH, H,
              q.gp, c.plane, q.dog, GH, q.dyp, q.we, q.dmsg, IN_e, q.dhg, GH, ws_wide.data_ptr(), wsb, st)
    if c.K == 0:
        _lib.call('tmpnn_gather_diff_fwd', g.cref(), q.dmsg, IN_e, q.dhg, GH, H, 1, st)
    if route.edge_bwd == 'wide_data_dw':
        ws2b = int(lib.tmpnn_wide_gru_bwd_weights_ws(E, H))
        ws2 = _wide_workspace(ws2b, dev, slot=1)
        _lib.call('tmpnn_wide_gru_bwd_weights', ws_wide.data_ptr(), g.edge_row.data_ptr(), E, g.src.data_ptr(),
                  g.dst.data_ptr(), q.hg, GH, H, *q.ge, ws2.data_ptr(), ws2b, st)
    else:
        _bwd_edge_weights(c, q)


def _bwd_attention(c, q, att_groups, grads, grad_out, dmsg: torch.Tensor) -> None:
    g, H, GH, N, E, Dn, K, IN_e, opts = c.g, c.H, c.GH, c.N, c.E, c.Dn, c.K, c.IN_e, c.opts
    f = q.f
    lib = _lib.load()
    erec, inc_other = g.att_index() if E > 0 else (None, None)
    for k0, Kg, W, a, kp, ws_ha, score, stats, esk in att_groups:
        ws_n_att = lib.tmpnn_att_bwd_ws(E, Dn, H, Kg)
        ws_att = torch.empty((max(ws_n_att, 1),), **opts)
        if Kg == K:
            d_out, ld_dout = dmsg.data_ptr(), IN_e
        else:
            d_es_g = torch.zeros((N, H), **opts)
            d_es_g[g.det_row.long()] = dmsg[g.det_row.long(), :H] * (Kg / K)
            d_out, ld_dout = d_es_g.data_ptr(), H
        gW = [grads.get(f + f'gat.{k}.W_att') for k in range(k0, k0 + Kg)] if grad_out is not None else []
        ga = [grads.get(f + f'gat.{k}.a') for k in range(k0, k0 + Kg)] if grad_out is not None else []
        args = (g.cref(), _lib.ptr(erec), _lib.ptr(inc_other), q.hg, GH, H, Kg, W.data_ptr(),
                a.data_ptr(), _lib.ptr(kp), ATT_DROPOUT_P, ws_ha.data_ptr(), score.data_ptr(), stats.data_ptr(),
                esk.data_ptr(), d_out, ld_dout, ws_att.data_ptr(), ws_att.numel(), q.dhg, GH)
        if grad_out is not None and all(t is not None and t.is_contiguous() for t in gW + ga):
            pW = (ctypes.c_void_p * Kg)(*[t.data_ptr() for t in gW])
            pa = (ctypes.c_void_p * Kg)(*[t.data_ptr() for t in ga])
            _lib.call('tmpnn_att_bwd_heads', *args, ctypes.cast(pW, ctypes.c_void_p), ctypes.cast(pa, ctypes.c_void_p), c.st)
        else:
            dW = torch.zeros((Kg, H, H), **opts)
            da = torch.zeros_like(a)
            _lib.call('tmpnn_att_bwd', *args, dW.data_ptr(), da.data_ptr(), c.st)
            for k in range(Kg):
                if grad_out is not None:
                    grads[f + f'gat.{k0 + k}.W_att'].add_(dW[k])
                    grads[f + f'gat.{k0 + k}.a'].add_(da[k].reshape(-1, 1))
                else:
                    grads[f + f'gat.{k0 + k}.W_att'] = dW[k]
                    grads[f + f'gat.{k0 + k}.a'] = da[k].reshape(-1, 1)


def _bwd_input_transform(c, route: CallRoute, saved: SavedCall, P, grads, d_hcat, training: bool, need_x: bool):
    spec, plan, H, GH, n, opts = c.spec, c.plan, c.H, c.GH, c.n, c.opts
    lib = _lib.load()
    nd = int(plan.new_det_row.numel())
    S = plan.S
    Ft = spec.F_total
    d_xdet = torch.empty((max(nd, 1), Ft), **opts) if need_x else None
    d_xzero = torch.empty((max(S, 1), Ft), **opts) if need_x else None
    f0 = 0
    for gi, (_, F) in enumerate(spec.groups):
        t = f'input_transforms.{gi}.'
        dz_g = torch.empty((max(S, 1), F), **opts) if need_x else None
        tf = route.tf[gi]
        if tf:
            wsb = int(lib.tmpnn_input_tf_bwd_ws(nd, S, H, F, int(training)))
            ws = torch.empty((wsb // 4 + 1,), **opts)
        else:
            ws = torch.empty((max(lib.tmpnn_input_bn_bwd_ws(nd, S, H, F), 1),), **opts)
            wsb = ws.numel()
        _lib.call('tmpnn_input_tf_bwd' if tf else 'tmpnn_input_bn_bwd',
                  *_tf_head(tf, plan, saved.xdet.data_ptr() + 4 * f0, saved.xrows, Ft, F, nd, H), int(training),
                  P[t + '0.weight'].data_ptr(), P[t + '0.bias'].data_ptr(),
                  P[t + '1.weight'].data_ptr(), P[t + '1.bias'].data_ptr(), P[t + '3.weight'].data_ptr(),
                  saved.y_save[gi].data_ptr(), saved.mean[gi].data_ptr(), saved.rstd[gi].data_ptr(),
                  plan.new_det_row.data_ptr(), d_hcat.data_ptr() + 4 * gi * H, GH,
                  (d_xdet.data_ptr() + 4 * f0) if need_x else None, Ft, _lib.ptr(dz_g),
                  grads[t + '0.weight'].data_ptr(), grads[t + '0.bias'].data_ptr(),
                  grads[t + '1.weight'].data_ptr(), grads[t + '1.bias'].data_ptr(),
                  grads[t + '3.weight'].data_ptr(), grads[t + '3.bias'].data_ptr(),
                  ws.data_ptr(), wsb, c.st)
        if need_x:
            d_xzero[:, f0:f0 + F] = dz_g
        f0 += F
    if not need_x:
        return None
    d_x = d_xzero[:S].index_select(0, plan.seg_of_new) if S > 0 else torch.zeros((n, Ft), **opts)
    if nd > 0:
        d_x.index_copy_(0, plan.new_det_local, d_xdet[:nd])
    return d_x


def mp_backward(spec: ModelSpec, plan: CallPlan, saved: SavedCall, P: Dict[str, torch.Tensor], training: bool,
                d_scores: Optional[torch.Tensor], d_logits: Optional[torch.Tensor], d_hout: Optional[torch.Tensor],
                need_x: bool, need_h: bool, grad_out=None):
    route = saved.route
    c = _call_dims(spec, plan, saved.h_cat.device)
    g, H, GH, N, E, Dn, IN_e, opts = c.g, c.H, c.GH, c.N, c.E, c.Dn, c.IN_e, c.opts
    lib = _lib.load()
    grads = _bwd_grads(spec, P, opts, grad_out)
    dy, dh_up = _bwd_heads(c, saved, P, grads, d_scores, d_logits, d_hout)

    d_hcat = torch.empty((N, GH), **opts)
    dmsg = torch.empty((N, IN_e), **opts)
    ws_e = lib.tmpnn_gru_bwd_weights_ws(E, IN_e, H)
    ws_n = lib.tmpnn_gru_bwd_weights_ws(Dn, H, H)
    ws_f = max(lib.tmpnn_gru_bwd_fused_ws(E, IN_e, H), lib.tmpnn_gru_bwd_fused_ws(Dn, H, H)) if route.bwd_fused else 0
    ws_w = torch.empty((max(ws_e, ws_n, ws_f) // 4 + 1,), **opts)
    gather = 'tmpnn_gather_concat_bwd' if spec.msg_type == 'concat' else 'tmpnn_gather_diff_bwd'
    for gi in range(c.G):
        q = _bwd_group(c, gi, saved, P, grads, dy, dh_up, d_hcat, dmsg, ws_w)
        _bwd_node_cell(c, route, q)
        if route.edge_bwd == 'fused':
            _bwd_edge_fused(c, route, q, saved)
        elif route.edge_bwd == 'generic':
            _bwd_edge_generic(c, q)
        else:
            _bwd_edge_wide(c, route, q, saved)
        if c.K > 0:
            _bwd_attention(c, q, saved.att[gi], grads, grad_out, dmsg)
        if route.gather_bwd:
            _lib.call(gather, g.cref(), q.dmsg, IN_e, q.dhg, GH, H, 1, c.st)

    d_x = None
    if c.n > 0:
        d_x = _bwd_input_transform(c, route, saved, P, grads, d_hcat, training, need_x)
    elif need_x:
        d_x = torch.zeros((0, spec.F_total), **opts)
    d_h_in = d_hcat[:c.N_old] if (need_h and c.N_old > 0) else None
    return d_x, d_h_in, grads


class MPIteration(torch.autograd.Function):

    @staticmethod
    def forward(ctx, call, x, h_in, *params):
        spec: ModelSpec = call['spec']
        names = spec.param_names()
        P = {nm: _f32c(p.detach()) for nm, p in zip(names, params)}
        for nm, p in P.items():
            _require_device(p, nm)
        need_grad = call['need_grad']
        scores, logits, h_out, alphas, saved = mp_forward(
            spec, call['plan'], x.detach(), None if h_in is None else _f32c(h_in.detach()), P, call['buffers'],
            call['training'], need_grad, call.get('keep'), call.get('reserve', 0), call.get('h_spare', 0))
        call['alphas'] = alphas
        ctx.call = call
        ctx.saved = saved
        ctx.P = P
        ctx.has_h = h_in is not None
        ctx.set_materialize_grads(False)
        return scores, logits, h_out

    @staticmethod
    def backward(ctx, d_scores, d_logits, d_hout):
        call = ctx.call
        spec: ModelSpec = call['spec']
        need = ctx.needs_input_grad
        names = spec.param_names()
        objs = call.get('param_objs')
        grad_out = None
        if (INPLACE_GRADS or call.get('inplace')) and objs is not None and all(need[3:]):
            gs = [p.grad for p in objs]
            if all(g is not None and g.dtype == torch.float32 and g.is_contiguous() and g.device == ctx.P[nm].device
                   and g.shape == ctx.P[nm].shape for g, nm in zip(gs, names)):
                grad_out = dict(zip(names, gs))
        d_x, d_h_in, grads = mp_backward(spec, call['plan'], ctx.saved, ctx.P, call['training'],
                                         d_scores, d_logits, d_hout, need_x=need[1],
                                         need_h=ctx.has_h and need[2], grad_out=grad_out)
        ctx.saved = None
        if grad_out is not None:
            return (None, d_x, d_h_in) + (None,) * len(names)
        return (None, d_x, d_h_in) + tuple(grads[nm] for nm in names)
```

Before: 737.9 million graph-edges/s.

## Co-schedule output-head weight-gradient blocks inside the diff gather-backward kernel

The heads backward pass is split in two. The per-row dy computation stays as its own small kernel, and the output-head weight/bias gradient reduction moves into a combined kernel that also runs the diff gather adjoint segment sum. Blocks are interleaved by a stride so that head blocks and adjoint blocks share the GPU at the same time. This removes a separate heads_bwd launch and lets the memory-bound reduction overlap the gather instead of serialising with it. The cost is more complex role dispatch and shared-memory sizing driven by the heads body, which may lower occupancy for the adjoint blocks.

Result: no change. 741.2 million graph-edges/s, median of 6 (+0.5%).

```diff
diff --git a/include/tmpnn.h b/include/tmpnn.h
--- a/include/tmpnn.h
+++ b/include/tmpnn.h
@@ -213,6 +213,13 @@
                     float* d_h, int ld_dh, int accumulate,
                     float* dw_node, float* db_node, float* dw_edge, float* db_edge,
                     void* ws, size_t ws_bytes, tmpnn_stream stream);
+int tmpnn_heads_dy(int N, const float* scores, const float* d_logits, const float* d_scores, float* dy_out,
+                   tmpnn_stream stream);
+int tmpnn_adjoint_heads_plan(int N, int Dn, int E, int H, int* grid, int* nheads, int* stride);
+int tmpnn_gather_diff_bwd_heads(const tmpnn_graph* g, const float* d_out, int ld_dout, float* d_in, int ld_din, int H,
+                                int accumulate, const float* h, int ld_h, int C, int N, const uint8_t* is_edge,
+                                const float* dy, float* dw_node, float* db_node, float* dw_edge, float* db_edge,
+                                void* ws, size_t ws_bytes, tmpnn_stream stream);
 
 int tmpnn_targets(const tmpnn_graph* g, const uint8_t* labels, uint8_t* targets, tmpnn_stream stream);
 size_t tmpnn_ce_loss_ws(int Dn);
diff --git a/trackmpnn_amd/_lib.py b/trackmpnn_amd/_lib.py
--- a/trackmpnn_amd/_lib.py
+++ b/trackmpnn_amd/_lib.py
@@ -221,6 +221,12 @@
     'tmpnn_heads_bwd': (c_int, [c_void_p, c_int, c_int, c_int, c_void_p, c_void_p, c_void_p, c_void_p, c_void_p,
                                 c_void_p, c_void_p, c_void_p, c_int, c_int, c_void_p, c_void_p, c_void_p, c_void_p,
                                 c_void_p, c_size_t, c_void_p]),
+    'tmpnn_heads_dy': (c_int, [c_int, c_void_p, c_void_p, c_void_p, c_void_p, c_void_p]),
+    'tmpnn_adjoint_heads_plan': (c_int, [c_int, c_int, c_int, c_int, C.POINTER(c_int), C.POINTER(c_int),
+                                         C.POINTER(c_int)]),
+    'tmpnn_gather_diff_bwd_heads': (c_int, [_GP, c_void_p, c_int, c_void_p, c_int, c_int, c_int, c_void_p, c_int, c_int, c_int,
+                                            c_void_p, c_void_p, c_void_p, c_void_p, c_void_p, c_void_p, c_void_p, c_size_t,
+                                            c_void_p]),
     'tmpnn_targets': (c_int, [_GP, c_void_p, c_void_p, c_void_p]),
     'tmpnn_ce_loss_ws': (c_size_t, [c_int]),
     'tmpnn_ce_loss_fwd': (c_int, [_GP, c_void_p, c_void_p, c_void_p, c_void_p, c_void_p, c_size_t, c_void_p]),
diff --git a/trackmpnn_amd/csrc/adjoint_heads.hip b/trackmpnn_amd/csrc/adjoint_heads.hip
--- /dev/null
+++ b/trackmpnn_amd/csrc/adjoint_heads.hip
@@ -0,0 +1,113 @@
+#include "agg_dev.h"
+#include "common.h"
+#include "heads_dev.h"
+#include <stdlib.h>
+
+namespace tmpnn {
+
+static constexpr int AH_STRIDE = 7;
+static_assert(AH_STRIDE >= 3 && AH_STRIDE % 2 == 1, "an even stride leaves XCDs without head blocks");
+
+#ifdef TMPNN_KEEP_VARIANTS
+static int ah_stride() {
+    static const int v = [] {
+        const char* e = getenv("TMPNN_ADJOINT_HEADS_STRIDE");
+        const int s = e ? atoi(e) : 0;
+        return s >= 2 ? s : AH_STRIDE;
+    }();
+    return v;
+}
+#else
+static constexpr int ah_stride() { return AH_STRIDE; }
+#endif
+
+__host__ __device__ inline int ah_role(int id, int nheads, int nadj, int stride, bool* head) {
+    const int qa = nadj / (stride - 1), q = nheads < qa ? nheads : qa;
+    const int L = q * stride;
+    if (id < L) {
+        const int g = id / stride, m = id - g * stride;
+        *head = m == 0;
+        return m == 0 ? g : g * (stride - 1) + m - 1;
+    }
+    const int r = id - L, hl = nheads - q;
+    *head = r < hl;
+    return r < hl ? q + r : q * (stride - 1) + (r - hl);
+}
+
+struct AhSeg {
+    int Dn;
+    const int32_t* det_row; const int32_t* rowptr; const int32_t* inc; const int32_t* det_order;
+    const float* in; int ld_in;
+    float* out; int ld_out;
+    int H;
+};
+struct AhHead {
+    const float* h; int ld_h; int C; int N;
+    const uint8_t* is_edge;
+    const float* dy;
+    int rows_per_block;
+    float* part;
+};
+
+template <bool ACC, int U, int CH>
+__global__ __launch_bounds__(256) void k_adjoint_heads(AhSeg a, AhHead b, int nheads, int nadj, int stride) {
+    extern __shared__ float sm[];
+    bool head;
+    const int blk = ah_role(blockIdx.x, nheads, nadj, stride, &head);
+    if (head)
+        heads_bwd_body<true>(blk, sm, b.h, b.ld_h, b.C, b.N, b.is_edge, nullptr, nullptr, nullptr, nullptr, nullptr, b.dy,
+                             nullptr, nullptr, 0, 0, b.rows_per_block, b.part);
+    else
+        segsum_pipe_body<ACC, U, CH, false, false>(blk, nadj, a.Dn, a.det_row, a.rowptr, a.inc, a.det_order, a.in, a.ld_in,
+                                                    a.out, a.ld_out, a.H, -1.0f, 0, 0, nullptr, 0, 0x7fffffff);
+}
+
+static int ah_nheads(int N) { return N > 0 ? ceil_div(N, heads_rows_per_block(N)) : 0; }
+static int ah_nadj(int Dn, int E) { return Dn > 0 ? segsum_grid_for(Dn, segsum_deep(E, Dn) ? 16 : 32) : 0; }
+
+}
+
+using namespace tmpnn;
+
+extern "C" {
+
+int tmpnn_adjoint_heads_plan(int N, int Dn, int E, int H, int* grid, int* nheads, int* stride) {
+    TM_REQUIRE(N >= 0 && Dn >= 0 && E >= 0 && (long)Dn + E == N, "adjoint_heads_plan: N=%d Dn=%d E=%d", N, Dn, E);
+    TM_REQUIRE(supported_H(H), "adjoint_heads_plan: H=%d is more than one slice", H);
+    TM_REQUIRE(grid && nheads && stride, "adjoint_heads_plan: null pointer");
+    *nheads = ah_nheads(N);
+    *grid = *nheads + ah_nadj(Dn, E);
+    *stride = ah_stride();
+    return TMPNN_OK;
+}
+
+int tmpnn_gather_diff_bwd_heads(const tmpnn_graph* g, const float* d_out, int ld_dout, float* d_in, int ld_din, int H,
+                                int accumulate, const float* h, int ld_h, int C, int N, const uint8_t* is_edge,
+                                const float* dy, float* dw_node, float* db_node, float* dw_edge, float* db_edge, void* ws,
+                                size_t ws_bytes, tmpnn_stream stream) {
+    int rc = check_graph(g);
+    if (rc) return rc;
+    TM_REQUIRE(supported_H(H), "gather_diff_bwd_heads: H=%d is more than one slice", H);
+    TM_REQUIRE(C > 0 && (C & 3) == 0 && C <= 1024, "gather_diff_bwd_heads: C=%d", C);
+    TM_REQUIRE(N == g->N, "gather_diff_bwd_heads: N=%d, the graph has %d rows", N, g->N);
+    TM_REQUIRE(!(g->seg_plan && H == 256), "gather_diff_bwd_heads: the graph's adjoint runs on its dense plan");
+    if (N == 0) return TMPNN_OK;
+    if (g->Dn > 0 && (rc = check_rows(d_out, ld_dout, d_in, ld_din, H, H, H))) return rc;
+    TM_REQUIRE(h && is_edge && dy && dw_node && db_node && dw_edge && db_edge, "gather_diff_bwd_heads: null pointer");
+    TM_REQUIRE(ld_h >= C && (ld_h & 3) == 0 && aligned16(h), "gather_diff_bwd_heads: rows of h must be 16-byte aligned");
+    const size_t need = tmpnn_heads_bwd_ws(N, C);
+    if (!ws || ws_bytes < need) return set_error(TMPNN_EWORKSPACE, "gather_diff_bwd_heads: workspace %zu < %zu", ws_bytes, need);
+    const int nheads = ah_nheads(N), nadj = ah_nadj(g->Dn, g->E);
+    const AhSeg a{g->Dn, g->det_row, g->rowptr, g->inc, g->det_order, d_out, ld_dout, d_in, ld_din, H};
+    const AhHead b{h, ld_h, C, N, is_edge, dy, heads_rows_per_block(N), reinterpret_cast<float*>(ws)};
+    hipStream_t st = as_stream(stream);
+    const dim3 grid(nheads + nadj), block(256);
+#define LAH(A, UU, CH) hipLaunchKernelGGL((k_adjoint_heads<A, UU, CH>), grid, block, heads_bwd_shm(C), st, a, b, nheads, nadj, ah_stride())
+    if (segsum_deep(g->E, g->Dn)) { if (accumulate) LAH(true, 8, 16); else LAH(false, 8, 16); }
+    else                          { if (accumulate) LAH(true, 4, 32); else LAH(false, 4, 32); }
+#undef LAH
+    if ((rc = check_launch("adjoint_heads"))) return rc;
+    return heads_bwd_finish(reinterpret_cast<float*>(ws), nheads, C, dw_node, db_node, dw_edge, db_edge, st);
+}
+
+}
diff --git a/trackmpnn_amd/csrc/agg.hip b/trackmpnn_amd/csrc/agg.hip
--- a/trackmpnn_amd/csrc/agg.hip
+++ b/trackmpnn_amd/csrc/agg.hip
@@ -1,4 +1,5 @@
 #include "common.h"
+#include "agg_dev.h"
 #include <stdlib.h>
 
 namespace tmpnn {
@@ -202,99 +203,8 @@
                                                      float wneg, int cneg, int compact_out,
                                                      const float* __restrict__ part = nullptr, int nsplit = 0,
                                                      int row_limit = 0x7fffffff) {
-    const int lane = threadIdx.x & 63;
-    const int lpr = H >> 2;
-    const int ngrp = 64 / lpr;
-    const int grp = lane / lpr;
-    const int c4 = (lane % lpr) * 4;
-    const int wv = threadIdx.x >> 6;
-    const long nchunk = (Dn + SEG_CHUNK - 1) / SEG_CHUNK;
-    auto item_pos = [&](long k) -> long {
-        const long per = SEG_CHUNK / 4;
-        const long ch = (long)blockIdx.x + (k / per) * gridDim.x;
-        if (ch >= nchunk) return -1;
-        const long i = ch * SEG_CHUNK + wv + (k % per) * 4;
-        return i < Dn ? i : -2;
-    };
-    long kA = 0;
-    int dA = -1, dB = -1, p0B = 0, p1B = 0, dC = -1, p0C = 0, p1C = 0, vC[U];
-    auto fetchA = [&]() {
-        long pos;
-        do { pos = item_pos(kA++); } while (pos == -2);
-        dA = pos < 0 ? -1 : (det_order ? det_order[pos] : (int)pos);
-    };
-    auto advanceB = [&]() {
-        dB = dA;
-        if (dB >= 0) { p0B = rowptr[dB]; p1B = rowptr[dB + 1]; }
-    };
-    auto advanceC = [&]() {
-        dC = dB; p0C = p0B; p1C = p1B;
-        if (dC >= 0) {
-#pragma unroll
-            for (int u = 0; u < U; ++u) {
-                const int p = p0C + grp + u * ngrp;
-                vC[u] = p < p1C ? inc[p] : 0x7fffffff;
-            }
-        }
-    };
-    fetchA(); advanceB(); fetchA(); advanceC(); advanceB(); fetchA();
-    int pbC = p0C + grp;
-    float4 acc = make_float4(0.f, 0.f, 0.f, 0.f);
-    while (dC >= 0) {
-        const int d = dC;
-        float4 x[U];
-        bool live[U];
-        float w[U];
-#pragma unroll
-        for (int u = 0; u < U; ++u) {
-            live[u] = vC[u] != 0x7fffffff;
-            const int row = live[u] ? (vC[u] & 0x7fffffff) : 0;
-            w[u] = vC[u] < 0 ? wneg : 1.0f;
-            if (LIM) {
-                live[u] = live[u] && row < row_limit;
-                x[u] = make_float4(0.f, 0.f, 0.f, 0.f);
-                if (live[u]) x[u] = *reinterpret_cast<const float4*>(in + (size_t)row * ld_in + (vC[u] < 0 ? cneg : 0) + c4);
-            } else if (DUAL && row >= nsplit)
-                x[u] = *reinterpret_cast<const float4*>(part + (size_t)(row - nsplit) * H + c4);
-            else
-                x[u] = *reinterpret_cast<const float4*>(in + (size_t)row * ld_in + (vC[u] < 0 ? cneg : 0) + c4);
-        }
-        const bool last = (pbC - grp) + ngrp * U >= p1C;
-        if (!last) {
-            pbC += ngrp * U;
-#pragma unroll
-            for (int u = 0; u < U; ++u) {
-                const int p = pbC + u * ngrp;
-                vC[u] = p < p1C ? inc[p] : 0x7fffffff;
-            }
-        } else {
-            advanceC(); advanceB(); fetchA();
-            pbC = p0C + grp;
-        }
-#pragma unroll
-        for (int u = 0; u < U; ++u) {
-            if (live[u]) { x[u].x *= w[u]; x[u].y *= w[u]; x[u].z *= w[u]; x[u].w *= w[u]; }
-            else x[u] = make_float4(0.f, 0.f, 0.f, 0.f);
-        }
-#pragma unroll
-        for (int u = 0; u < U; ++u) { acc.x += x[u].x; acc.y += x[u].y; acc.z += x[u].z; acc.w += x[u].w; }
-        if (!last) continue;
-        for (int off = lpr; off < 64; off <<= 1) {
-            acc.x += __shfl_xor(acc.x, off);
-            acc.y += __shfl_xor(acc.y, off);
-            acc.z += __shfl_xor(acc.z, off);
-            acc.w += __shfl_xor(acc.w, off);
-        }
-        if (grp == 0) {
-            float* o = out + (size_t)(compact_out ? d : det_row[d]) * ld_out + c4;
-            if (ACC) {
-                const float4 p = *reinterpret_cast<const float4*>(o);
-                acc.x += p.x; acc.y += p.y; acc.z += p.z; acc.w += p.w;
-            }
-            *reinterpret_cast<float4*>(o) = acc;
-        }
-        acc = make_float4(0.f, 0.f, 0.f, 0.f);
-    }
+    segsum_pipe_body<ACC, U, SEG_CHUNK, DUAL, LIM>(blockIdx.x, gridDim.x, Dn, det_row, rowptr, inc, det_order, in, ld_in, out,
+                                                   ld_out, H, wneg, cneg, compact_out, part, nsplit, row_limit);
 }
 
 #ifdef TMPNN_KEEP_VARIANTS
@@ -360,31 +270,7 @@
     return check_launch("reduce_slabs");
 }
 
-static int check_graph(const tmpnn_graph* g) {
-    TM_REQUIRE(g != nullptr, "graph is null");
-    TM_REQUIRE(g->N >= 0 && g->E >= 0 && g->Dn >= 0 && (long)g->E + g->Dn == g->N,
-               "graph sizes inconsistent: N=%d E=%d Dn=%d", g->N, g->E, g->Dn);
-    if (g->E > 0)
-        TM_REQUIRE(g->src && g->dst && g->edge_row && g->inc, "graph edge arrays are null (E=%d)", g->E);
-    if (g->Dn > 0) TM_REQUIRE(g->det_row && g->rowptr, "graph det arrays are null (Dn=%d)", g->Dn);
-    return TMPNN_OK;
-}
-
-static int check_rows(const float* in, int ld_in, const float* out, int ld_out, int H, int w_in, int w_out) {
-    TM_REQUIRE(supported_H(H), "unsupported hidden width H=%d (need 32/64/128/256)", H);
-    TM_REQUIRE(in && out, "null feature pointer");
-    TM_REQUIRE(ld_in >= w_in && ld_out >= w_out, "leading dimension too small (ld_in=%d ld_out=%d)", ld_in, ld_out);
-    TM_REQUIRE((ld_in & 3) == 0 && (ld_out & 3) == 0 && aligned16(in) && aligned16(out),
-               "feature rows must be 16-byte aligned (ld multiple of 4 floats)");
-    return TMPNN_OK;
-}
-
-static int grid_for(long items, int per_block) {
-    long b = (items + per_block - 1) / per_block;
-    if (b > 256L * 64) b = 256L * 64;
-    if (b < 1) b = 1;
-    return (int)b;
-}
+static int grid_for(long items, int per_block) { return segsum_grid_for(items, per_block); }
 
 static int gather(const tmpnn_graph* g, const float* in, int ld_in, float* out, int ld_out, int H, int accumulate,
                   bool concat, tmpnn_stream stream) {
@@ -797,7 +683,7 @@
         hipLaunchKernelGGL((k_segsum_pipe<A, UU, CH>), grid, block, 0, st, g->Dn, g->det_row, g->rowptr, g->inc, \
                            g->det_order, in, ld_in, out, ld_out, H, wneg, cneg, compact_out);                \
     } while (0)
-    const bool deep = (long)2 * g->E > (long)24 * g->Dn;
+    const bool deep = segsum_deep(g->E, g->Dn);
     if (row_limit < g->N && !accumulate) {
         grid = dim3(grid_for(g->Dn, deep ? 16 : 32));
         if (deep)
diff --git a/trackmpnn_amd/csrc/agg_dev.h b/trackmpnn_amd/csrc/agg_dev.h
--- /dev/null
+++ b/trackmpnn_amd/csrc/agg_dev.h
@@ -0,0 +1,139 @@
+#pragma once
+#include "common.h"
+
+namespace tmpnn {
+
+inline int check_graph(const tmpnn_graph* g) {
+    TM_REQUIRE(g != nullptr, "graph is null");
+    TM_REQUIRE(g->N >= 0 && g->E >= 0 && g->Dn >= 0 && (long)g->E + g->Dn == g->N,
+               "graph sizes inconsistent: N=%d E=%d Dn=%d", g->N, g->E, g->Dn);
+    if (g->E > 0)
+        TM_REQUIRE(g->src && g->dst && g->edge_row && g->inc, "graph edge arrays are null (E=%d)", g->E);
+    if (g->Dn > 0) TM_REQUIRE(g->det_row && g->rowptr, "graph det arrays are null (Dn=%d)", g->Dn);
+    return TMPNN_OK;
+}
+
+inline int check_rows(const float* in, int ld_in, const float* out, int ld_out, int H, int w_in, int w_out) {
+    TM_REQUIRE(supported_H(H), "unsupported hidden width H=%d (need 32/64/128/256)", H);
+    TM_REQUIRE(in && out, "null feature pointer");
+    TM_REQUIRE(ld_in >= w_in && ld_out >= w_out, "leading dimension too small (ld_in=%d ld_out=%d)", ld_in, ld_out);
+    TM_REQUIRE((ld_in & 3) == 0 && (ld_out & 3) == 0 && aligned16(in) && aligned16(out),
+               "feature rows must be 16-byte aligned (ld multiple of 4 floats)");
+    return TMPNN_OK;
+}
+
+__host__ __device__ inline bool segsum_deep(int E, int Dn) { return (long)2 * E > (long)24 * Dn; }
+
+__host__ __device__ inline int segsum_grid_for(long items, int per_block) {
+    long b = (items + per_block - 1) / per_block;
+    if (b > 256L * 64) b = 256L * 64;
+    if (b < 1) b = 1;
+    return (int)b;
+}
+
+template <bool ACC, int U, int SEG_CHUNK, bool DUAL, bool LIM>
+__device__ __forceinline__ void segsum_pipe_body(const unsigned bid, const unsigned nblk, int Dn,
+                                                 const int32_t* __restrict__ det_row,
+                                                 const int32_t* __restrict__ rowptr,
+                                                 const int32_t* __restrict__ inc,
+                                                 const int32_t* __restrict__ det_order,
+                                                 const float* __restrict__ in, int ld_in,
+                                                 float* __restrict__ out, int ld_out, int H,
+                                                 float wneg, int cneg, int compact_out,
+                                                 const float* __restrict__ part, int nsplit, int row_limit) {
+    const int lane = threadIdx.x & 63;
+    const int lpr = H >> 2;
+    const int ngrp = 64 / lpr;
+    const int grp = lane / lpr;
+    const int c4 = (lane % lpr) * 4;
+    const int wv = threadIdx.x >> 6;
+    const long nchunk = (Dn + SEG_CHUNK - 1) / SEG_CHUNK;
+    auto item_pos = [&](long k) -> long {
+        const long per = SEG_CHUNK / 4;
+        const long ch = (long)bid + (k / per) * nblk;
+        if (ch >= nchunk) return -1;
+        const long i = ch * SEG_CHUNK + wv + (k % per) * 4;
+        return i < Dn ? i : -2;
+    };
+    long kA = 0;
+    int dA = -1, dB = -1, p0B = 0, p1B = 0, dC = -1, p0C = 0, p1C = 0, vC[U];
+    auto fetchA = [&]() {
+        long pos;
+        do { pos = item_pos(kA++); } while (pos == -2);
+        dA = pos < 0 ? -1 : (det_order ? det_order[pos] : (int)pos);
+    };
+    auto advanceB = [&]() {
+        dB = dA;
+        if (dB >= 0) { p0B = rowptr[dB]; p1B = rowptr[dB + 1]; }
+    };
+    auto advanceC = [&]() {
+        dC = dB; p0C = p0B; p1C = p1B;
+        if (dC >= 0) {
+#pragma unroll
+            for (int u = 0; u < U; ++u) {
+                const int p = p0C + grp + u * ngrp;
+                vC[u] = p < p1C ? inc[p] : 0x7fffffff;
+            }
+        }
+    };
+    fetchA(); advanceB(); fetchA(); advanceC(); advanceB(); fetchA();
+    int pbC = p0C + grp;
+    float4 acc = make_float4(0.f, 0.f, 0.f, 0.f);
+    while (dC >= 0) {
+        const int d = dC;
+        float4 x[U];
+        bool live[U];
+        float w[U];
+#pragma unroll
+        for (int u = 0; u < U; ++u) {
+            live[u] = vC[u] != 0x7fffffff;
+            const int row = live[u] ? (vC[u] & 0x7fffffff) : 0;
+            w[u] = vC[u] < 0 ? wneg : 1.0f;
+            if (LIM) {
+                live[u] = live[u] && row < row_limit;
+                x[u] = make_float4(0.f, 0.f, 0.f, 0.f);
+                if (live[u]) x[u] = *reinterpret_cast<const float4*>(in + (size_t)row * ld_in + (vC[u] < 0 ? cneg : 0) + c4);
+            } else if (DUAL && row >= nsplit)
+                x[u] = *reinterpret_cast<const float4*>(part + (size_t)(row - nsplit) * H + c4);
+            else
+                x[u] = *reinterpret_cast<const float4*>(in + (size_t)row * ld_in + (vC[u] < 0 ? cneg : 0) + c4);
+        }
+        const bool last = (pbC - grp) + ngrp * U >= p1C;
+        if (!last) {
+            pbC += ngrp * U;
+#pragma unroll
+            for (int u = 0; u < U; ++u) {
+                const int p = pbC + u * ngrp;
+                vC[u] = p < p1C ? inc[p] : 0x7fffffff;
+            }
+        } else {
+            advanceC(); advanceB(); fetchA();
+            pbC = p0C + grp;
+        }
+#pragma unroll
+        for (int u = 0; u < U; ++u) {
+            if (live[u]) { x[u].x *= w[u]; x[u].y *= w[u]; x[u].z *= w[u]; x[u].w *= w[u]; }
+            else x[u] = make_float4(0.f, 0.f, 0.f, 0.f);
+        }
+#pragma unroll
+        for (int u = 0; u < U; ++u) { acc.x += x[u].x; acc.y += x[u].y; acc.z += x[u].z; acc.w += x[u].w; }
+        if (!last) continue;
+        for (int off = lpr; off < 64; off <<= 1) {
+            acc.x += __shfl_xor(acc.x, off);
+            acc.y += __shfl_xor(acc.y, off);
+            acc.z += __shfl_xor(acc.z, off);
+            acc.w += __shfl_xor(acc.w, off);
+        }
+        if (grp == 0) {
+            float* o = out + (size_t)(compact_out ? d : det_row[d]) * ld_out + c4;
+            if (ACC) {
+                const float4 p = *reinterpret_cast<const float4*>(o);
+                acc.x += p.x; acc.y += p.y; acc.z += p.z; acc.w += p.w;
+            }
+            *reinterpret_cast<float4*>(o) = acc;
+        }
+        acc = make_float4(0.f, 0.f, 0.f, 0.f);
+    }
+}
+
+}
diff --git a/trackmpnn_amd/csrc/dense.hip b/trackmpnn_amd/csrc/dense.hip
--- a/trackmpnn_amd/csrc/dense.hip
+++ b/trackmpnn_amd/csrc/dense.hip
@@ -1,4 +1,5 @@
 #include "common.h"
+#include "heads_dev.h"
 
 namespace tmpnn {
 
@@ -597,73 +598,14 @@
                                                    int ld_dh, int accumulate, int rows_per_block,
                                                    float* __restrict__ part) {
     extern __shared__ float sm[];
-    const int cpt = C >> 2;
-    const int slots = 256 / cpt;
-    const int slot = threadIdx.x / cpt;
-    const int c4 = (threadIdx.x % cpt) * 4;
-    const bool active = slot < slots;
-    float4 an = make_float4(0.f, 0.f, 0.f, 0.f), ae = an;
-    float bn = 0.f, be = 0.f;
-    const long r0 = (long)blockIdx.x * rows_per_block;
-    const long r1 = min((long)N, r0 + rows_per_block);
-    if (active) {
-        constexpr int UR = 4;
-        for (long i0 = r0 + slot; i0 < r1; i0 += (long)slots * UR) {
-            float dyv[UR];
-            bool ev[UR], live[UR];
-            float4 xv[UR];
-#pragma unroll
-            for (int u = 0; u < UR; ++u) {
-                const long i = i0 + (long)u * slots;
-                live[u] = i < r1;
-                const long ic = live[u] ? i : r1 - 1;
-                float dy = d_logits ? d_logits[ic] : 0.f;
-                if (d_scores) {
-                    const float sc = scores[ic];
-                    dy += d_scores[ic] * sc * (1.0f - sc);
-                }
-                dyv[u] = live[u] ? dy : 0.f;
-                ev[u] = is_edge[ic] != 0;
-                xv[u] = *reinterpret_cast<const float4*>(h + (size_t)ic * ld_h + c4);
-            }
-#pragma unroll
-            for (int u = 0; u < UR; ++u) {
-                if (!live[u]) continue;
-                const long i = i0 + (long)u * slots;
-                const float dy = dyv[u];
-                const bool e = ev[u];
-                const float4 x = xv[u];
-                if (dy_out && c4 == 0) dy_out[i] = dy;
-                if (d_h) {
-                    const float4 w = *reinterpret_cast<const float4*>((e ? w_edge : w_node) + c4);
-                    float* dp = d_h + (size_t)i * ld_dh + c4;
-                    float4 o = make_float4(dy * w.x, dy * w.y, dy * w.z, dy * w.w);
-                    if (accumulate) {
-                        const float4 p = *reinterpret_cast<const float4*>(dp);
-                        o.x += p.x; o.y += p.y; o.z += p.z; o.w += p.w;
-                    }
-                    *reinterpret_cast<float4*>(dp) = o;
-                }
-                if (e) { ae.x += dy * x.x; ae.y += dy * x.y; ae.z += dy * x.z; ae.w += dy * x.w; if (c4 == 0) be += dy; }
-                else   { an.x += dy * x.x; an.y += dy * x.y; an.z += dy * x.z; an.w += dy * x.w; if (c4 == 0) bn += dy; }
-            }
-        }
-        float* my = sm + (size_t)slot * 2 * C;
-        *reinterpret_cast<float4*>(my + c4) = an;
-        *reinterpret_cast<float4*>(my + C + c4) = ae;
-        if (c4 == 0) {
-            sm[(size_t)slots * 2 * C + slot * 2 + 0] = bn;
-            sm[(size_t)slots * 2 * C + slot * 2 + 1] = be;
-        }
-    }
-    __syncthreads();
-    float* out = part + (size_t)blockIdx.x * (2 * C + 2);
-    for (int j = threadIdx.x; j < 2 * C + 2; j += 256) {
-        float s = 0.f;
-        if (j < 2 * C) for (int k = 0; k < slots; ++k) s += sm[(size_t)k * 2 * C + j];
-        else for (int k = 0; k < slots; ++k) s += sm[(size_t)slots * 2 * C + k * 2 + (j - 2 * C)];
-        out[j] = s;
-    }
+    heads_bwd_body<false>(blockIdx.x, sm, h, ld_h, C, N, is_edge, w_node, w_edge, scores, d_logits, d_scores, nullptr, dy_out,
+                          d_h, ld_dh, accumulate, rows_per_block, part);
+}
+
+__global__ __launch_bounds__(256) void k_heads_dy(int N, const float* __restrict__ scores, const float* __restrict__ d_logits,
+                                                  const float* __restrict__ d_scores, float* __restrict__ dy_out) {
+    const long i = (long)blockIdx.x * 256 + threadIdx.x;
+    if (i < N) dy_out[i] = heads_dy(scores, d_logits, d_scores, i);
 }
 
 __global__ void k_heads_bwd_final(const float* __restrict__ red, int C, float* __restrict__ dw_node,
@@ -678,10 +620,15 @@
     else db_edge[0] += s;
 }
 
-static int heads_rows_per_block(int N) {
-    long rpb = ((long)N + 2047) / 2048;
-    if (rpb < 64) rpb = 64;
-    return (int)rpb;
+int heads_bwd_finish(float* part, int nblk, int C, float* dw_node, float* db_node, float* dw_edge, float* db_edge,
+                     hipStream_t st) {
+    const size_t nred = 2 * (size_t)C + 2;
+    float* red = part + (size_t)nblk * nred;
+    int rc;
+    if ((rc = launch_reduce_slabs(part, nred, nblk, red, nred, 0, st, red + nred))) return rc;
+    hipLaunchKernelGGL(k_heads_bwd_final, dim3(ceil_div(2 * C + 2, 256)), dim3(256), 0, st, red, C, dw_node, db_node,
+                       dw_edge, db_edge);
+    return check_launch("heads_bwd_final");
 }
 
 }
@@ -870,22 +817,24 @@
     if (!ws || ws_bytes < need) return set_error(TMPNN_EWORKSPACE, "heads_bwd: workspace %zu < %zu", ws_bytes, need);
     const int rpb = heads_rows_per_block(N);
     const int nblk = ceil_div(N, rpb);
-    const int cpt = C >> 2;
-    TM_REQUIRE(cpt <= 256, "heads_bwd: C too wide");
-    const int slots = 256 / cpt;
-    const size_t shm = ((size_t)slots * 2 * C + (size_t)slots * 2) * sizeof(float);
+    TM_REQUIRE((C >> 2) <= 256, "heads_bwd: C too wide");
     hipStream_t st = as_stream(stream);
-    hipLaunchKernelGGL(k_heads_bwd, dim3(nblk), dim3(256), shm, st, h, ld_h, C, N, is_edge, w_node, w_edge, scores,
+    hipLaunchKernelGGL(k_heads_bwd, dim3(nblk), dim3(256), heads_bwd_shm(C), st, h, ld_h, C, N, is_edge, w_node, w_edge, scores,
                        d_logits, d_scores, dy_out, d_h, ld_dh, accumulate, rpb, reinterpret_cast<float*>(ws));
     int rc = check_launch("heads_bwd");
     if (rc) return rc;
-    const size_t nred = 2 * (size_t)C + 2;
-    float* part = reinterpret_cast<float*>(ws);
-    float* red = part + (size_t)nblk * nred;
-    if ((rc = launch_reduce_slabs(part, nred, nblk, red, nred, 0, st, red + nred))) return rc;
-    hipLaunchKernelGGL(k_heads_bwd_final, dim3(ceil_div(2 * C + 2, 256)), dim3(256), 0, st, red, C, dw_node, db_node,
-                       dw_edge, db_edge);
-    return check_launch("heads_bwd_final");
-}
-
-}
+    return heads_bwd_finish(reinterpret_cast<float*>(ws), nblk, C, dw_node, db_node, dw_edge, db_edge, st);
+}
+
+int tmpnn_heads_dy(int N, const float* scores, const float* d_logits, const float* d_scores, float* dy_out,
+                   tmpnn_stream stream) {
+    TM_REQUIRE(N >= 0, "heads_dy: N=%d", N);
+    if (N == 0) return TMPNN_OK;
+    TM_REQUIRE(dy_out, "heads_dy: null pointer");
+    TM_REQUIRE(d_scores == nullptr || scores != nullptr, "heads_dy: d_scores needs scores");
+    hipLaunchKernelGGL(k_heads_dy, dim3(ceil_div(N, 256)), dim3(256), 0, as_stream(stream), N, scores, d_logits, d_scores,
+                       dy_out);
+    return check_launch("heads_dy");
+}
+
+}
diff --git a/trackmpnn_amd/csrc/heads_dev.h b/trackmpnn_amd/csrc/heads_dev.h
--- /dev/null
+++ b/trackmpnn_amd/csrc/heads_dev.h
@@ -0,0 +1,102 @@
+#pragma once
+#include "common.h"
+
+namespace tmpnn {
+
+__host__ __device__ inline int heads_rows_per_block(int N) {
+    long rpb = ((long)N + 2047) / 2048;
+    if (rpb < 64) rpb = 64;
+    return (int)rpb;
+}
+
+inline size_t heads_bwd_shm(int C) {
+    const int slots = 256 / (C >> 2);
+    return ((size_t)slots * 2 * C + (size_t)slots * 2) * sizeof(float);
+}
+
+__device__ __forceinline__ float heads_dy(const float* scores, const float* d_logits, const float* d_scores, long i) {
+    float dy = d_logits ? d_logits[i] : 0.f;
+    if (d_scores) {
+        const float sc = scores[i];
+        dy += d_scores[i] * sc * (1.0f - sc);
+    }
+    return dy;
+}
+
+template <bool DY_IN>
+__device__ __forceinline__ void heads_bwd_body(const unsigned bid, float* sm, const float* __restrict__ h, int ld_h,
+                                               int C, int N, const uint8_t* __restrict__ is_edge,
+                                               const float* __restrict__ w_node, const float* __restrict__ w_edge,
+                                               const float* __restrict__ scores, const float* __restrict__ d_logits,
+                                               const float* __restrict__ d_scores, const float* __restrict__ dy_in,
+                                               float* __restrict__ dy_out, float* __restrict__ d_h, int ld_dh,
+                                               int accumulate, int rows_per_block, float* __restrict__ part) {
+    const int cpt = C >> 2;
+    const int slots = 256 / cpt;
+    const int slot = threadIdx.x / cpt;
+    const int c4 = (threadIdx.x % cpt) * 4;
+    const bool active = slot < slots;
+    float4 an = make_float4(0.f, 0.f, 0.f, 0.f), ae = an;
+    float bn = 0.f, be = 0.f;
+    const long r0 = (long)bid * rows_per_block;
+    const long r1 = min((long)N, r0 + rows_per_block);
+    if (active) {
+        constexpr int UR = 4;
+        for (long i0 = r0 + slot; i0 < r1; i0 += (long)slots * UR) {
+            float dyv[UR];
+            bool ev[UR], live[UR];
+            float4 xv[UR];
+#pragma unroll
+            for (int u = 0; u < UR; ++u) {
+                const long i = i0 + (long)u * slots;
+                live[u] = i < r1;
+                const long ic = live[u] ? i : r1 - 1;
+                const float dy = DY_IN ? dy_in[ic] : heads_dy(scores, d_logits, d_scores, ic);
+                dyv[u] = live[u] ? dy : 0.f;
+                ev[u] = is_edge[ic] != 0;
+                xv[u] = *reinterpret_cast<const float4*>(h + (size_t)ic * ld_h + c4);
+            }
+#pragma unroll
+            for (int u = 0; u < UR; ++u) {
+                if (!live[u]) continue;
+                const long i = i0 + (long)u * slots;
+                const float dy = dyv[u];
+                const bool e = ev[u];
+                const float4 x = xv[u];
+                if (dy_out && c4 == 0) dy_out[i] = dy;
+                if (d_h) {
+                    const float4 w = *reinterpret_cast<const float4*>((e ? w_edge : w_node) + c4);
+                    float* dp = d_h + (size_t)i * ld_dh + c4;
+                    float4 o = make_float4(dy * w.x, dy * w.y, dy * w.z, dy * w.w);
+                    if (accumulate) {
+                        const float4 p = *reinterpret_cast<const float4*>(dp);
+                        o.x += p.x; o.y += p.y; o.z += p.z; o.w += p.w;
+                    }
+                    *reinterpret_cast<float4*>(dp) = o;
+                }
+                if (e) { ae.x += dy * x.x; ae.y += dy * x.y; ae.z += dy * x.z; ae.w += dy * x.w; if (c4 == 0) be += dy; }
+                else   { an.x += dy * x.x; an.y += dy * x.y; an.z += dy * x.z; an.w += dy * x.w; if (c4 == 0) bn += dy; }
+            }
+        }
+        float* my = sm + (size_t)slot * 2 * C;
+        *reinterpret_cast<float4*>(my + c4) = an;
+        *reinterpret_cast<float4*>(my + C + c4) = ae;
+        if (c4 == 0) {
+            sm[(size_t)slots * 2 * C + slot * 2 + 0] = bn;
+            sm[(size_t)slots * 2 * C + slot * 2 + 1] = be;
+        }
+    }
+    __syncthreads();
+    float* out = part + (size_t)bid * (2 * C + 2);
+    for (int j = threadIdx.x; j < 2 * C + 2; j += 256) {
+        float s = 0.f;
+        if (j < 2 * C) for (int k = 0; k < slots; ++k) s += sm[(size_t)k * 2 * C + j];
+        else for (int k = 0; k < slots; ++k) s += sm[(size_t)slots * 2 * C + k * 2 + (j - 2 * C)];
+        out[j] = s;
+    }
+}
+
+int heads_bwd_finish(float* ws, int nblk, int C, float* dw_node, float* db_node, float* dw_edge, float* db_edge,
+                     hipStream_t st);
+
+}
diff --git a/trackmpnn_amd/functional.py b/trackmpnn_amd/functional.py
--- a/trackmpnn_amd/functional.py
+++ b/trackmpnn_amd/functional.py
@@ -17,6 +17,7 @@
 FUSED_BWD = os.environ.get('TMPNN_FUSED_BWD', '1') == '1'
 ZERO_STATE_BWD = os.environ.get('TMPNN_BWD_ZERO_STATE', '1') != '0'
 ZERO_STATE_FWD = os.environ.get('TMPNN_FWD_ZERO_STATE', '1') != '0'
+HEADS_UNDER_ADJOINT = os.environ.get('TMPNN_HEADS_UNDER_ADJOINT', '1') != '0'
 WIDE_OVERLAP = os.environ.get('TMPNN_WIDE_OVERLAP', '0') == '1' and os.environ.get('TMPNN_KEEP_VARIANTS', '0') == '1'
 ATT_KMAX = 8
 _SPLIT = os.environ.get('TMPNN_SPLIT', '1')[:1] != '0'
@@ -222,6 +223,7 @@
     bwd_fused: bool
     edge_bwd: str
     gather_bwd: bool
+    heads_under_adjoint: bool = False
 
     @property
     def wide(self) -> bool:
@@ -282,12 +284,16 @@
         edge_bwd = 'wide_data_dw' if WIDE_DW else 'wide_data'
     else:
         edge_bwd = 'generic'
+    gather_bwd = edge_bwd not in ('wide_det_fused', 'wide_det')
+    dense_plan = wide and H % 256 == 0 and K == 0
+    heads_under_adjoint = bool(save and HEADS_UNDER_ADJOINT and gather_bwd and diff and G == 1 and K == 0 and H <= 256
+                               and G * H <= 1024 and not dense_plan)
     return CallRoute(n=n, E_old=E_old, save=save, edge_fwd=edge_fwd, tile_rows=FWD_TILE_ROWS,
                      agg='attention' if K > 0 else 'segsum', zs_fwd=zs_fwd, zs_bwd=zs_bwd,
                      zs_groups=tuple(zs_bwd and a for a in aligned), zs_rc=zs_rc, recompute_gates=recompute, cw=cw,
-                     tf=tf, tf_all=nd > 0 and all(tf), dense_plan=wide and H % 256 == 0 and K == 0,
+                     tf=tf, tf_all=nd > 0 and all(tf), dense_plan=dense_plan,
                      win_plan=WIN_SEGSUM and H == 64 and E > 0, bwd_fused=bwd_fused, edge_bwd=edge_bwd,
-                     gather_bwd=edge_bwd not in ('wide_det_fused', 'wide_det'))
+                     gather_bwd=gather_bwd, heads_under_adjoint=heads_under_adjoint)
 
 
 @dataclass
@@ -618,7 +624,7 @@
     return {nm: flat[o:o + sz].view(P[nm].shape) for nm, o, sz in zip(names, offs, sizes)}
 
 
-def _bwd_heads(c, saved: SavedCall, P, grads, d_scores, d_logits, d_hout):
+def _bwd_heads(c, saved: SavedCall, P, grads, d_scores, d_logits, d_hout, dy_only: bool = False):
     g, N, GH, opts = c.g, c.N, c.GH, c.opts
     lib = _lib.load()
     dh_up = _f32c(d_hout) if d_hout is not None else None
@@ -627,6 +633,9 @@
         dy = torch.empty((N,), **opts)
         dl = _f32c(d_logits) if d_logits is not None else None
         ds = _f32c(d_scores) if d_scores is not None else None
+        if dy_only:
+            _lib.call('tmpnn_heads_dy', N, saved.scores.data_ptr(), _lib.ptr(dl), _lib.ptr(ds), dy.data_ptr(), c.st)
+            return dy, dh_up
         for c0 in range(0, GH, 1024):
             cw_ = min(1024, GH - c0)
             ws_b = lib.tmpnn_heads_bwd_ws(N, cw_)
@@ -642,6 +651,16 @@
     elif dh_up is None:
         dh_up = torch.zeros((N, GH), **opts)
     return dy, dh_up
+
+
+def _bwd_adjoint_heads(c, q, saved: SavedCall, grads, dy) -> None:
+    g, H, GH, N, IN_e = c.g, c.H, c.GH, c.N, c.IN_e
+    ws_b = _lib.load().tmpnn_heads_bwd_ws(N, GH)
+    ws = torch.empty((max(ws_b // 4, 1),), **c.opts)
+    _lib.call('tmpnn_gather_diff_bwd_heads', g.cref(), q.dmsg, IN_e, q.dhg, GH, H, 1, saved.h_out.data_ptr(), GH, GH, N,
+              g.is_edge.data_ptr(), dy.data_ptr(), grads['output_transform_node.weight'].data_ptr(),
+              grads['output_transform_node.bias'].data_ptr(), grads['output_transform_edge.weight'].data_ptr(),
+              grads['output_transform_edge.bias'].data_ptr(), ws.data_ptr(), ws_b, c.st)
 
 
 def _bwd_group(c, gi: int, saved: SavedCall, P, grads, dy, dh_up, d_hcat, dmsg, ws_w) -> SimpleNamespace:
@@ -849,7 +868,9 @@
     g, H, GH, N, E, Dn, IN_e, opts = c.g, c.H, c.GH, c.N, c.E, c.Dn, c.IN_e, c.opts
     lib = _lib.load()
     grads = _bwd_grads(spec, P, opts, grad_out)
-    dy, dh_up = _bwd_heads(c, saved, P, grads, d_scores, d_logits, d_hout)
+    fuse_heads = (route.heads_under_adjoint and (d_scores is not None or d_logits is not None)
+                  and not (H == 256 and g.__dict__.get('_seg_plan') is not None))
+    dy, dh_up = _bwd_heads(c, saved, P, grads, d_scores, d_logits, d_hout, dy_only=fuse_heads)
 
     d_hcat = torch.empty((N, GH), **opts)
     dmsg = torch.empty((N, IN_e), **opts)
@@ -869,7 +890,9 @@
             _bwd_edge_wide(c, route, q, saved)
         if c.K > 0:
             _bwd_attention(c, q, saved.att[gi], grads, grad_out, dmsg)
-        if route.gather_bwd:
+        if fuse_heads:
+            _bwd_adjoint_heads(c, q, saved, grads, dy)
+        elif route.gather_bwd:
             _lib.call(gather, g.cref(), q.dmsg, IN_e, q.dhg, GH, H, 1, c.st)
 
     d_x = None
```
